# Blaizzy/mlx-audio

Measured on NVIDIA H100. Metric: audio-sec/sec Kokoro-82M TTS (128-phoneme utterance, 9.75 s), higher is better.
Workload: dtype bf16x2

## Files before the change

include/b200audio.h:

```cpp
#ifndef B200AUDIO_H
#define B200AUDIO_H

#include <stdint.h>

#ifdef __cplusplus
extern "C" {
#endif

#define B2A_OK 0
#define B2A_E_INVALID (-1)
#define B2A_E_CUDA (-2)
#define B2A_E_UNSUPPORTED (-3)

enum {
  B2A_ACT_NONE = 0,
  B2A_ACT_LRELU = 1,
  B2A_ACT_SNAKE = 2,
  B2A_ACT_ELU = 3,
  B2A_ACT_GELU = 4,
  B2A_ACT_GELU_TANH = 5,
  B2A_ACT_TANH = 6,
  B2A_ACT_SIGMOID = 7,
  B2A_ACT_SILU = 8,
  B2A_ACT_CLIP1 = 9
};

const char* b2a_last_error(void);
int32_t b2a_version(void);
int32_t b2a_device_sm_count(void);

typedef struct {
  const float* x; int64_t x_bs; int64_t x_ld;
  int32_t B, L, Cin;
  const float* w; const float* bias;
  float* y; int64_t y_bs; int64_t y_ld;
  int32_t Lout, Cout;
  int32_t K, stride, dilation, pad_left, groups, pad_mode;
  const float* pre_scale; const float* pre_shift;
  int32_t pre_act; float pre_p0; const float* pre_a; const float* pre_b;
  int32_t post_act; float post_p0;
  const float* post_cscale; int64_t post_cscale_bs;
  const float* res; int64_t res_bs; int64_t res_ld; int32_t res_div;
  float out_scale; int32_t accumulate;
  void* emit_hi; void* emit_lo; int64_t emit_ld;
  int32_t emit_act; float emit_p0; const float* emit_a; const float* emit_b;
} b2a_conv1d_t;

int32_t b2a_conv1d_cl(const b2a_conv1d_t* p, void* stream);
int32_t b2a_convtr1d_cl(const b2a_conv1d_t* p, void* stream);

enum {
  B2A_CONV_PATH_LINEAR_ROWS = 1,
  B2A_CONV_PATH_NARROW = 2,
  B2A_CONV_PATH_DENSE = 3,
  B2A_CONV_PATH_DW_TILED4 = 4,
  B2A_CONV_PATH_DW_TILED = 5,
  B2A_CONV_PATH_DW = 6,
  B2A_CONV_PATH_CONVTR_DENSE = 7,
  B2A_CONV_PATH_CONVTR_DW = 8
};
int32_t b2a_conv1d_cl_last_path(int32_t* out4);

int32_t b2a_kokoro_source_conv(const float* x, int32_t B, int32_t L, const float* w, const float* bias, float* y, int32_t Lout,
                               int32_t Cout, int32_t K, int32_t stride, int32_t pad_left, void* stream);

int32_t b2a_prep_bf16(const float* x, int64_t x_bs, int64_t x_ld, int32_t B, int32_t L, int32_t C, int32_t cpad,
                      const float* scale, const float* shift, int32_t act, float p0, const float* a, const float* b,
                      void* hi, void* lo, int32_t f16, void* stream);
int32_t b2a_conv1d_tc(const void* a_hi, const void* a_lo, int32_t f16, int32_t B, int32_t L, int32_t cin_pad, const void* w_bf16,
                      const void* w_lo,
                      int32_t taps, const int32_t* shifts_host, int32_t Cout, int32_t Lout, const float* bias,
                      int32_t post_act, float post_p0, const float* cscale, int64_t cscale_bs, const float* res,
                      int64_t res_bs, int64_t res_ld, int32_t res_div, float out_scale, int32_t accumulate, float* y,
                      int64_t y_bs, int64_t y_ld, int32_t up_stride, int32_t up_crop, void* emit_hi, void* emit_lo,
                      int64_t emit_ld, void* attn_ws, int32_t attn_heads, float attn_scale, void* stream);

typedef struct {
  int32_t T, layers, heads, hidden, inter, planes;
  const void* w[4];
  const float* bias[4];
  const float* ln_w[2];
  const float* ln_b[2];
  float eps, scale;
  float* h; void* h_hi; void* h_lo;
} b2a_albert_t;
int64_t b2a_albert_ws_bytes(int32_t T, int32_t heads, int32_t hidden, int32_t inter);
int32_t b2a_albert_encoder(const b2a_albert_t* a, void* ws, uint32_t* err, int64_t* timeline, void* stream);

int32_t b2a_conv1d_tc_debug(void* dbg8);

int32_t b2a_conv1d_tc_last_config(int32_t* out5);

int32_t b2a_copy2d(const float* src, int64_t src_ld, float* dst, int64_t dst_ld, int64_t rows, int32_t cols, void* stream);
int32_t b2a_gather_rows(const float* src, int64_t src_ld, const int64_t* idx, float* dst, int64_t dst_ld,
                        int64_t rows, int32_t cols, int64_t n_src_rows, const float* add, int64_t add_ld, int64_t add_period,
                        void* stream);
int32_t b2a_durations_to_index(const float* dur_f, const int64_t* dur_i, int32_t T, float speed, int64_t* pred_dur_out,
                               int64_t* idx_out, int64_t max_frames, int64_t* total_dev, void* stream);

int64_t b2a_adain_ws_bytes(int32_t B, int32_t L, int32_t C);
int32_t b2a_adain_coeffs(const float* x, int64_t x_bs, int64_t x_ld, int32_t B, int32_t L, int32_t C,
                         const float* gb, float eps, float* scale, float* shift, void* ws, void* stream);
int32_t b2a_channel_stats(const float* x, int64_t x_bs, int64_t x_ld, int32_t B, int32_t L, int32_t C, int64_t* const* dst,
                          const int64_t* dst_bs, int32_t n_dst, void* stream);
int32_t b2a_coeffs_from_stats(const int64_t* stats, int32_t B, int32_t L, int32_t C, const float* gb, float eps, float* scale, float* shift,
                              void* stream);
int32_t b2a_layernorm(const float* x, int64_t x_ld, const float* res, int64_t res_ld, float* y, int64_t y_ld,
                      int64_t rows, int32_t C, const float* w, const float* b, const float* ada, float eps,
                      int32_t rms, int32_t post_act, float post_p0, void* emit_hi, void* emit_lo, int64_t emit_ld, void* stream);

typedef struct {
  const float* q; const float* k; const float* v; float* o;
  int64_t q_bs, q_ld, k_bs, k_ld, v_bs, v_ld, o_bs, o_ld;
  int32_t B, Tq, Tk, H, Hkv, D;
  float scale; int32_t causal, q_offset, window;
  const int32_t* k_len;
  void* emit_hi; void* emit_lo; int64_t emit_ld;
  int32_t operands_ready;
} b2a_attn_t;
int32_t b2a_attention(const b2a_attn_t* p, void* stream);
int64_t b2a_attention_tc_ws_bytes(int32_t B, int32_t H, int32_t Tq, int32_t Tk);
int32_t b2a_attention_tc(const b2a_attn_t* p, void* ws, void* stream);
int32_t b2a_rope(float* x, int64_t x_bs, int64_t x_ld, int32_t B, int32_t T, int32_t H, int32_t D,
                 int32_t offset, float base, int32_t traditional, void* stream);

int32_t b2a_lstm_bidir(const float* xproj, const float* wh, float* out, int64_t out_ld, int32_t B, int32_t T, int32_t H, void* stream);

int32_t b2a_stft(const float* x, int64_t x_bs, int32_t B, int64_t n, const float* window, int32_t n_fft, int32_t hop,
                 int32_t pad_mode, int64_t frames, float* out_re, float* out_im, void* stream);
int32_t b2a_whisper_logmel(const float* x, int64_t x_bs, int32_t B, int64_t n, int64_t padding, const float* window,
                           const float* filters, int32_t n_mels, int64_t frames, float* out, float* gmax, void* stream);
int32_t b2a_istft(const float* re, const float* im, int32_t B, int32_t n_fft, int32_t T, int32_t hop, const float* window,
                  int32_t norm_sq, int32_t clamp_mode, int64_t trim, int64_t out_len, float* out, float* ws, void* stream);

int32_t b2a_resample_poly(const float* x, int64_t x_bs, int32_t B, int64_t n_in, const double* h, int32_t n_h, int32_t up,
                          int32_t down, int64_t n_pre_pad, int64_t n_pre_remove, float* out, int64_t n_out, void* stream);

int32_t b2a_kokoro_source(const float* f0, int32_t B, int32_t n_frames, int32_t n_down, const float* noise, const float* lin_w,
                          const float* lin_b, float* har, float* src_ws, double* ph_ws, void* stream);
int32_t b2a_kokoro_istft_head(const float* x, int64_t x_bs, int64_t x_ld, int32_t B, int32_t T, float* audio, void* stream);

#define B2A_CONVF_MAX_PROBLEMS 4
typedef struct {
  const float* x; const float* x1; const float* x2; int64_t x_bs, x_ld; float in_scale;
  int32_t B, L, Cin;
  int32_t pre_mode; const float* pre_scale; const float* pre_shift; const int64_t* pre_stats; const float* pre_gb; int64_t pre_gb_bs; float pre_eps;
  int32_t pre_act; float pre_p0; const float* pre_a; const float* pre_b;
  const void* w_hi; const void* w_lo; int32_t cin_pad, taps, N; int32_t shifts[32];
  int32_t Lout; const float* bias; int32_t post_act; float post_p0; const float* cscale; int64_t cscale_bs;
  const float* res; int64_t res_bs, res_ld; int32_t res_div; float out_scale; int32_t accumulate;
  float* y; int64_t y_bs, y_ld;
  int32_t up_stride, up_crop;
  int64_t* stats_out;
} b2a_convf_t;
int32_t b2a_conv1d_fused_debug(void* stamps );
int32_t b2a_conv1d_fused(const b2a_convf_t* problems, int32_t n_problems, int32_t planes, int32_t f16, void* ws, int64_t ws_bytes, void* stream);
int32_t b2a_conv1d_fused_fits(int32_t span, int32_t N, int32_t C, int32_t wplanes, int32_t planes);
int32_t b2a_conv1d_fused_last_config(int32_t* out10);

int32_t b2a_randn(float* out, int64_t n, uint64_t seed, uint64_t offset, void* stream);
int32_t b2a_randn_dev(float* out, int64_t n, uint64_t* state, void* stream);

int32_t b2a_whisper_greedy_step(const float* logits, int64_t logits_bs, const int64_t* tokens, int64_t tokens_bs,
                                int32_t B, int32_t cur_len, int32_t sample_begin, int32_t V, const float* suppress_mask,
                                const float* blank_mask, int32_t eot, int32_t no_timestamps, int32_t timestamp_begin,
                                int32_t max_initial_ts, int32_t without_timestamps, int64_t* next_out,
                                float* sum_logprobs, int32_t* not_done, float temperature, const float* u, void* stream);

int32_t b2a_sample_token(const float* logits, int64_t logits_bs, int32_t B, int32_t V, const float* suppress_mask,
                         uint8_t* seen, int64_t seen_bs, int32_t mark_seen, float repetition_penalty, float temperature,
                         int32_t top_k, float top_p, float min_p, const float* u, int64_t* out, int64_t out_stride,
                         float* filtered_out, uint8_t* finished, int32_t eos, void* stream);

int32_t b2a_gemv_bf16(const float* x, int64_t x_ld, int32_t M, int32_t K, const void* w_bf16, int64_t w_ld, int32_t N,
                      const float* bias, const float* norm_w, float norm_eps, int32_t mode, const float* res, int64_t res_ld,
                      float* y, int64_t y_ld, const void* prefetch, int64_t prefetch_bytes, void* stream);
int32_t b2a_qknorm_rope_cache(const float* qkv, int64_t qkv_bs, int64_t qkv_ss, int32_t B, int32_t S, int32_t Hq, int32_t Hkv,
                              int32_t D, const float* q_norm_w, const float* k_norm_w, float eps, const int32_t* pos3,
                              const int32_t* base_dev, int32_t base_host, int32_t sec_h, int32_t sec_w, float theta,
                              float* q_out, int64_t qo_bs, int64_t qo_ss, float* k_cache, float* v_cache, int64_t c_bs,
                              int64_t c_ss, int32_t smax, const int32_t* pos_shift, const int32_t* base_rows, const int32_t* slot,
                              void* stream);
int32_t b2a_attn_decode(const float* q, int64_t q_bs, int64_t q_ss, const float* k_cache, const float* v_cache, int64_t c_bs,
                        int64_t c_ss, float* out, int64_t o_bs, int64_t o_ss, int32_t B, int32_t S, int32_t Hq, int32_t Hkv,
                        int32_t D, float scale, const int32_t* base_dev, int32_t base_host, const int32_t* kv_start,
                        int32_t max_k, const int32_t* base_rows, const int32_t* slot, void* stream);
int32_t b2a_attn_prefill(const float* q, int64_t q_bs, int64_t q_ss, const float* k_cache, const float* v_cache, int64_t c_bs,
                         int64_t c_ss, float* out, int64_t o_bs, int64_t o_ss, int32_t B, int32_t S, int32_t Hq, int32_t Hkv,
                         int32_t D, float scale, const int32_t* base_dev, int32_t base_host, const int32_t* kv_start,
                         int32_t max_k, const int32_t* base_rows, const int32_t* slot, void* stream);
int32_t b2a_swiglu(const float* x, int64_t x_ld, int64_t rows, int32_t I, int32_t interleaved, float* y, int64_t y_ld, void* stream);
int32_t b2a_embed_sum(const int64_t* codes, int64_t codes_bs, int32_t B, int32_t G, int32_t dim, const float* const* tables_dev,
                      const int32_t* bins_dev, const float* text, int64_t text_bs, int64_t text_ss, int32_t n_text,
                      const float* pad, const int32_t* step_dev, int32_t step_sub, float* out, int64_t out_bs,
                      int32_t* err_flag_dev, int32_t* tidx, const uint8_t* finished, void* stream);
int32_t b2a_incr_i32(int32_t* p, int32_t v, void* stream);
int32_t b2a_slot_advance(int32_t* lengths, int32_t* frames, uint8_t* finished, const int32_t* cap, const int64_t* codes, int32_t G,
                         int64_t* out, int64_t out_bs, const float* u_tab, int64_t u_bs, float* u, int32_t B, void* stream);

int32_t b2a_rvq_decode(const int64_t* codes, int64_t codes_bs, int64_t codes_qs, int32_t B, int32_t nq, int64_t T,
                       const float* codebooks, int32_t bins, int32_t dim, float* out, int64_t out_ld, int32_t* err_flag_dev, void* stream);
int32_t b2a_rvq_encode(const float* x, int64_t x_ld, int64_t rows, int32_t dim, const float* codebooks, const double* c2, int32_t bins,
                       int32_t nq, int32_t mode, int64_t* codes, int64_t codes_row_stride, int64_t codes_level_stride, void* stream);
int32_t b2a_snac_from_codes(const int64_t* const* codes_host_ptrs, const int32_t* strides_host, int32_t n_levels,
                            const float* const* emb_host_ptrs, const float* const* w_host_ptrs, const float* const* bias_host_ptrs,
                            int32_t B, int64_t T, int32_t bins, int32_t cd, int32_t dim, float* out, int32_t* err_flag_dev, void* stream);

typedef struct {
  const float* w_in; const float* b_in;
  const float* cbn; const double* c2;
  const float* cb;
  const float* w_out; const float* b_out;
  int32_t cd; int32_t lat_off;
} b2a_dac_level_t;
int64_t b2a_dac_rvq_encode_smem_bytes(int32_t dim);
int32_t b2a_dac_rvq_encode(const float* z, int64_t z_ld, int32_t B, int64_t T, int32_t dim, const b2a_dac_level_t* levels_dev, int32_t n_levels,
                           int32_t bins, int32_t latent_channels, int64_t* codes, float* latents, float* z_q, double* loss_part, void* stream);
int32_t b2a_dac_from_codes(const int64_t* codes, int64_t codes_bs, int64_t codes_qs, int32_t B, int32_t n_levels, int64_t T,
                           const b2a_dac_level_t* levels_dev, int32_t bins, int32_t latent_channels, int32_t dim, float* out, float* z_p,
                           int32_t* err_flag_dev, void* stream);

int32_t b2a_aa_snakebeta(const float* x, int64_t x_bs, int64_t x_ld, int32_t B, int32_t L, int32_t C, const float* alpha, const float* inv_beta,
                         const float* f_up, const float* f_down, int32_t ratio, int32_t taps, float* y, int64_t y_bs, int64_t y_ld, void* hi,
                         void* lo, int32_t cpad, void* stream);

#define B2A_ROWOP_COPY 0
#define B2A_ROWOP_ADD 1
#define B2A_ROWOPS_MAX 32
typedef struct {
  const float* src; int64_t src_bs, src_ld;
  float* dst; int64_t dst_bs, dst_ld;
  int32_t B, rows, C, op;
} b2a_rowop_t;
int32_t b2a_stream_rows(const b2a_rowop_t* ops, int32_t n, void* stream);

int32_t b2a_conv1d_stream(const b2a_conv1d_t* p, float* hist, int64_t hist_bs, int32_t H, const int32_t* step_dev, int32_t fresh,
                          void* stream);
int32_t b2a_convtr1d_stream(const b2a_conv1d_t* p, float* tail, int64_t tail_bs, void* stream);
int32_t b2a_ring_rope_kv(float* qkv, int64_t qkv_bs, int64_t qkv_ld, int32_t B, int32_t T, int32_t H, int32_t D, float base,
                         float* k_ring, float* v_ring, int64_t ring_bs, int32_t cap, const int32_t* pos_dev, void* stream);
int32_t b2a_ring_attn(const float* q, int64_t q_bs, int64_t q_ld, const float* k_ring, const float* v_ring, int64_t ring_bs, int32_t cap,
                      float* out, int64_t o_bs, int64_t o_ld, int32_t B, int32_t T, int32_t H, int32_t D, float scale, int32_t window,
                      const int32_t* pos_dev, void* stream);
int32_t b2a_stream_advance(int32_t* ctr, int32_t dpos, void* stream);

int32_t b2a_spk_logmel(const float* x, int64_t x_bs, int32_t B, int64_t n, const float* window, const float* filters, int32_t n_mels,
                       int64_t frames, float* out, void* stream);
int32_t b2a_spk_reflect_pad(const float* x, int64_t x_bs, int64_t x_ld, int32_t B, int32_t T, int32_t C, int32_t pad, float* out_f32,
                            void* hi, void* lo, int32_t cpad, void* stream);
int64_t b2a_spk_res2net_smem_bytes(int32_t C, int32_t scale, int32_t K, int32_t pad, int32_t tile);
int32_t b2a_spk_res2net(const float* y, int64_t y_bs, int64_t y_ld, float* z, int64_t z_bs, int64_t z_ld, const float* w, const float* bias,
                        int32_t B, int32_t T, int32_t C, int32_t scale, int32_t K, int32_t dilation, int32_t tile, void* stream);
int32_t b2a_spk_channel_stats(const float* x, int64_t x_bs, int64_t x_ld, int32_t B, int32_t T, int32_t C, int32_t with_std, float eps,
                              float* out, int64_t o_bs, void* stream);
int32_t b2a_spk_se_gate(const float* mean, int64_t m_bs, int32_t B, int32_t C, int32_t S, const float* w1, const float* b1, const float* w2,
                        const float* b2, float* gate, void* stream);
int32_t b2a_spk_se_apply(const float* y, int64_t y_bs, int64_t y_ld, const float* gate, const float* res, int64_t r_bs, int64_t r_ld,
                         float* out, int64_t o_bs, int64_t o_ld, int32_t B, int32_t T, int32_t C, void* stream);
int32_t b2a_spk_gemv(const float* x, int64_t x_bs, int32_t B, int32_t K, const float* w, int64_t w_ld, int32_t N, const float* bias,
                     int32_t act, float* y, int64_t y_bs, void* stream);
int32_t b2a_spk_asp_act(float* h, int64_t h_bs, int64_t h_ld, const float* cb, int32_t B, int32_t T, int32_t A, void* stream);
int32_t b2a_spk_asp_pool(const float* logits, int64_t l_bs, int64_t l_ld, const float* x, int64_t x_bs, int64_t x_ld, int32_t B, int32_t T,
                         int32_t C, float eps, float* pooled, int64_t p_bs, void* stream);

int32_t b2a_vocos_dwnorm(const float* x, int64_t x_bs, int64_t x_ld, int32_t B, int32_t L, int32_t C, const float* dw_w, const float* dw_b,
                         int32_t K, const float* w, const float* b, const float* ada, int64_t ada_bs, float eps, float* y, int64_t y_bs,
                         int64_t y_ld, void* hi, void* lo, void* stream);
int32_t b2a_vocos_istft_head(const float* h, int64_t h_bs, int64_t h_ld, int32_t B, int32_t T, int32_t n_fft, int32_t hop, const float* window,
                             float* out, int64_t out_bs, void* stream);
int32_t b2a_vocos_logmel(const float* x, int64_t x_bs, int32_t B, int64_t n, const float* window, const float* filters, int32_t n_mels,
                         int64_t frames, float* out, void* stream);

int32_t b2a_encodec_lstm(const float* xproj, const float* wh, const float* skip, float* out, int32_t R, int32_t T, int32_t H, uint32_t* err,
                         void* stream);
int32_t b2a_encodec_pad(const float* x, int64_t x_bs, int64_t x_ld, int32_t B, int32_t T, int32_t C, int32_t pad_left, int32_t pad_right,
                        int32_t reflect, const float* scale, const float* shift, int32_t elu, const float* res, int64_t res_bs, int64_t res_ld,
                        float* y, int64_t y_bs, int64_t y_ld, void* stream);
int64_t b2a_encodec_gn_ws_bytes(int32_t B);
int32_t b2a_encodec_gn_coeffs(const float* x, int64_t x_bs, int64_t x_ld, int32_t B, int32_t T, int32_t C, const float* gamma,
                              const float* beta, float eps, float* scale, float* shift, void* ws, void* stream);
int32_t b2a_encodec_normalize(const float* x, int64_t x_bs, int64_t x_ld, int32_t R, int32_t L, int32_t C, const uint8_t* mask,
                              int64_t mask_bs, float* y, float* scale, void* stream);
int32_t b2a_encodec_ola(const float* frames, int32_t N, int32_t B, int32_t L, int32_t C, const float* scale, int32_t stride, int32_t Tout,
                        float* out, void* stream);

int32_t b2a_lm_sample_mlx(const float* logits, int64_t logits_bs, int32_t B, int32_t V, float temperature, double top_p, const float* u,
                          int64_t u_bs, const int32_t* step_dev, int64_t* out, int64_t* hist, int64_t hist_bs, uint8_t* finished,
                          int32_t stop0, int32_t stop1, void* stream);
int32_t b2a_soprano_upsample(const float* x, int64_t x_bs, int64_t x_ld, int32_t B, int32_t L, int32_t H, int32_t up, float* y, int64_t y_bs,
                             int64_t y_ld, void* hi, void* lo, int32_t cpad, void* stream);
int32_t b2a_soprano_store_rows(const float* src, int64_t src_bs, int32_t B, int32_t H, float* dst, int64_t dst_bs, int64_t dst_ld,
                               const int32_t* idx_dev, int32_t add, int32_t cap, void* stream);

#ifdef __cplusplus
}
#endif
#endif
```

mlx_audio_b200/_lib.py:

```python
from __future__ import annotations

import ctypes as C
import os

_HERE = os.path.dirname(os.path.abspath(__file__))
LIB_PATH = os.path.join(_HERE, "libb200audio.so")

c_f = C.c_void_p
i32, i64, f32 = C.c_int32, C.c_int64, C.c_float


class Conv1dParams(C.Structure):
    _fields_ = [
        ("x", C.c_void_p), ("x_bs", i64), ("x_ld", i64),
        ("B", i32), ("L", i32), ("Cin", i32),
        ("w", C.c_void_p), ("bias", C.c_void_p),
        ("y", C.c_void_p), ("y_bs", i64), ("y_ld", i64),
        ("Lout", i32), ("Cout", i32),
        ("K", i32), ("stride", i32), ("dilation", i32), ("pad_left", i32), ("groups", i32), ("pad_mode", i32),
        ("pre_scale", C.c_void_p), ("pre_shift", C.c_void_p),
        ("pre_act", i32), ("pre_p0", f32), ("pre_a", C.c_void_p), ("pre_b", C.c_void_p),
        ("post_act", i32), ("post_p0", f32),
        ("post_cscale", C.c_void_p), ("post_cscale_bs", i64),
        ("res", C.c_void_p), ("res_bs", i64), ("res_ld", i64), ("res_div", i32),
        ("out_scale", f32), ("accumulate", i32),
        ("emit_hi", C.c_void_p), ("emit_lo", C.c_void_p), ("emit_ld", i64),
        ("emit_act", i32), ("emit_p0", f32), ("emit_a", C.c_void_p), ("emit_b", C.c_void_p),
    ]


class AttnParams(C.Structure):
    _fields_ = [
        ("q", C.c_void_p), ("k", C.c_void_p), ("v", C.c_void_p), ("o", C.c_void_p),
        ("q_bs", i64), ("q_ld", i64), ("k_bs", i64), ("k_ld", i64), ("v_bs", i64), ("v_ld", i64), ("o_bs", i64), ("o_ld", i64),
        ("B", i32), ("Tq", i32), ("Tk", i32), ("H", i32), ("Hkv", i32), ("D", i32),
        ("scale", f32), ("causal", i32), ("q_offset", i32), ("window", i32),
        ("k_len", C.c_void_p),
        ("emit_hi", C.c_void_p), ("emit_lo", C.c_void_p), ("emit_ld", i64), ("operands_ready", i32),
    ]


class ConvFParams(C.Structure):
    _fields_ = [
        ("x", C.c_void_p), ("x1", C.c_void_p), ("x2", C.c_void_p), ("x_bs", i64), ("x_ld", i64), ("in_scale", f32),
        ("B", i32), ("L", i32), ("Cin", i32),
        ("pre_mode", i32), ("pre_scale", C.c_void_p), ("pre_shift", C.c_void_p), ("pre_stats", C.c_void_p), ("pre_gb", C.c_void_p),
        ("pre_gb_bs", i64), ("pre_eps", f32),
        ("pre_act", i32), ("pre_p0", f32), ("pre_a", C.c_void_p), ("pre_b", C.c_void_p),
        ("w_hi", C.c_void_p), ("w_lo", C.c_void_p), ("cin_pad", i32), ("taps", i32), ("N", i32), ("shifts", i32 * 32),
        ("Lout", i32), ("bias", C.c_void_p), ("post_act", i32), ("post_p0", f32), ("cscale", C.c_void_p), ("cscale_bs", i64),
        ("res", C.c_void_p), ("res_bs", i64), ("res_ld", i64), ("res_div", i32), ("out_scale", f32), ("accumulate", i32),
        ("y", C.c_void_p), ("y_bs", i64), ("y_ld", i64),
        ("up_stride", i32), ("up_crop", i32),
        ("stats_out", C.c_void_p),
    ]


class AlbertParams(C.Structure):
    _fields_ = [("T", i32), ("layers", i32), ("heads", i32), ("hidden", i32), ("inter", i32), ("planes", i32),
                ("w", C.c_void_p * 4), ("bias", C.c_void_p * 4), ("ln_w", C.c_void_p * 2), ("ln_b", C.c_void_p * 2),
                ("eps", f32), ("scale", f32), ("h", C.c_void_p), ("h_hi", C.c_void_p), ("h_lo", C.c_void_p)]


class RowOp(C.Structure):
    _fields_ = [("src", C.c_void_p), ("src_bs", i64), ("src_ld", i64), ("dst", C.c_void_p), ("dst_bs", i64), ("dst_ld", i64),
                ("B", i32), ("rows", i32), ("C", i32), ("op", i32)]


class DacLevel(C.Structure):
    _fields_ = [("w_in", C.c_void_p), ("b_in", C.c_void_p), ("cbn", C.c_void_p), ("c2", C.c_void_p), ("cb", C.c_void_p),
                ("w_out", C.c_void_p), ("b_out", C.c_void_p), ("cd", i32), ("lat_off", i32)]


ROWOPS_MAX = 32


PROTOTYPES = {
    "b2a_last_error": (C.c_char_p, []),
    "b2a_version": (i32, []),
    "b2a_device_sm_count": (i32, []),
    "b2a_conv1d_cl": (i32, [C.POINTER(Conv1dParams), C.c_void_p]),
    "b2a_convtr1d_cl": (i32, [C.POINTER(Conv1dParams), C.c_void_p]),
    "b2a_conv1d_cl_last_path": (i32, [C.POINTER(i32)]),
    "b2a_kokoro_source_conv": (i32, [c_f, i32, i32, c_f, c_f, c_f, i32, i32, i32, i32, i32, C.c_void_p]),
    "b2a_prep_bf16": (i32, [c_f, i64, i64, i32, i32, i32, i32, c_f, c_f, i32, f32, c_f, c_f, c_f, c_f, i32, C.c_void_p]),
    "b2a_conv1d_tc": (i32, [c_f, c_f, i32, i32, i32, i32, c_f, c_f, i32, C.POINTER(i32), i32, i32, c_f, i32, f32, c_f, i64, c_f, i64, i64, i32, f32, i32,
                            c_f, i64, i64, i32, i32, c_f, c_f, i64, c_f, i32, f32, C.c_void_p]),
    "b2a_conv1d_tc_debug": (i32, [c_f]),
    "b2a_conv1d_tc_last_config": (i32, [C.POINTER(i32)]),
    "b2a_conv1d_fused_debug": (i32, [c_f]),
    "b2a_conv1d_fused_last_config": (i32, [C.POINTER(i32)]),
    "b2a_conv1d_fused": (i32, [C.POINTER(ConvFParams), i32, i32, i32, c_f, i64, C.c_void_p]),
    "b2a_conv1d_fused_fits": (i32, [i32, i32, i32, i32, i32]),
    "b2a_copy2d": (i32, [c_f, i64, c_f, i64, i64, i32, C.c_void_p]),
    "b2a_gather_rows": (i32, [c_f, i64, c_f, c_f, i64, i64, i32, i64, c_f, i64, i64, C.c_void_p]),
    "b2a_durations_to_index": (i32, [c_f, c_f, i32, f32, c_f, c_f, i64, c_f, C.c_void_p]),
    "b2a_adain_ws_bytes": (i64, [i32, i32, i32]),
    "b2a_adain_coeffs": (i32, [c_f, i64, i64, i32, i32, i32, c_f, f32, c_f, c_f, c_f, C.c_void_p]),
    "b2a_channel_stats": (i32, [c_f, i64, i64, i32, i32, i32, C.POINTER(C.c_void_p), C.POINTER(i64), i32, C.c_void_p]),
    "b2a_coeffs_from_stats": (i32, [c_f, i32, i32, i32, c_f, f32, c_f, c_f, C.c_void_p]),
    "b2a_layernorm": (i32, [c_f, i64, c_f, i64, c_f, i64, i64, i32, c_f, c_f, c_f, f32, i32, i32, f32, c_f, c_f, i64, C.c_void_p]),
    "b2a_attention": (i32, [C.POINTER(AttnParams), C.c_void_p]),
    "b2a_attention_tc_ws_bytes": (i64, [i32, i32, i32, i32]),
    "b2a_attention_tc": (i32, [C.POINTER(AttnParams), C.c_void_p, C.c_void_p]),
    "b2a_albert_ws_bytes": (i64, [i32, i32, i32, i32]),
    "b2a_albert_encoder": (i32, [C.POINTER(AlbertParams), C.c_void_p, C.c_void_p, C.c_void_p, C.c_void_p]),
    "b2a_rope": (i32, [c_f, i64, i64, i32, i32, i32, i32, i32, f32, i32, C.c_void_p]),
    "b2a_lstm_bidir": (i32, [c_f, c_f, c_f, i64, i32, i32, i32, C.c_void_p]),
    "b2a_stft": (i32, [c_f, i64, i32, i64, c_f, i32, i32, i32, i64, c_f, c_f, C.c_void_p]),
    "b2a_whisper_logmel": (i32, [c_f, i64, i32, i64, i64, c_f, c_f, i32, i64, c_f, c_f, C.c_void_p]),
    "b2a_istft": (i32, [c_f, c_f, i32, i32, i32, i32, c_f, i32, i32, i64, i64, c_f, c_f, C.c_void_p]),
    "b2a_resample_poly": (i32, [c_f, i64, i32, i64, c_f, i32, i32, i32, i64, i64, c_f, i64, C.c_void_p]),
    "b2a_kokoro_source": (i32, [c_f, i32, i32, i32, c_f, c_f, c_f, c_f, c_f, c_f, C.c_void_p]),
    "b2a_kokoro_istft_head": (i32, [c_f, i64, i64, i32, i32, c_f, C.c_void_p]),
    "b2a_randn": (i32, [c_f, i64, C.c_uint64, C.c_uint64, C.c_void_p]),
    "b2a_randn_dev": (i32, [c_f, i64, c_f, C.c_void_p]),
    "b2a_whisper_greedy_step": (i32, [c_f, i64, c_f, i64, i32, i32, i32, i32, c_f, c_f, i32, i32, i32, i32, i32, c_f, c_f, c_f, f32, c_f, C.c_void_p]),
    "b2a_sample_token": (i32, [c_f, i64, i32, i32, c_f, c_f, i64, i32, f32, f32, i32, f32, f32, c_f, c_f, i64, c_f, c_f, i32, C.c_void_p]),
    "b2a_gemv_bf16": (i32, [c_f, i64, i32, i32, c_f, i64, i32, c_f, c_f, f32, i32, c_f, i64, c_f, i64, c_f, i64, C.c_void_p]),
    "b2a_qknorm_rope_cache": (i32, [c_f, i64, i64, i32, i32, i32, i32, i32, c_f, c_f, f32, c_f, c_f, i32, i32, i32, f32, c_f, i64, i64,
                                    c_f, c_f, i64, i64, i32, c_f, c_f, c_f, C.c_void_p]),
    "b2a_attn_decode": (i32, [c_f, i64, i64, c_f, c_f, i64, i64, c_f, i64, i64, i32, i32, i32, i32, i32, f32, c_f, i32, c_f, i32, c_f, c_f,
                              C.c_void_p]),
    "b2a_attn_prefill": (i32, [c_f, i64, i64, c_f, c_f, i64, i64, c_f, i64, i64, i32, i32, i32, i32, i32, f32, c_f, i32, c_f, i32, c_f, c_f,
                               C.c_void_p]),
    "b2a_swiglu": (i32, [c_f, i64, i64, i32, i32, c_f, i64, C.c_void_p]),
    "b2a_embed_sum": (i32, [c_f, i64, i32, i32, i32, c_f, c_f, c_f, i64, i64, i32, c_f, c_f, i32, c_f, i64, c_f, c_f, c_f, C.c_void_p]),
    "b2a_incr_i32": (i32, [c_f, i32, C.c_void_p]),
    "b2a_slot_advance": (i32, [c_f, c_f, c_f, c_f, c_f, i32, c_f, i64, c_f, i64, c_f, i32, C.c_void_p]),
    "b2a_rvq_decode": (i32, [c_f, i64, i64, i32, i32, i64, c_f, i32, i32, c_f, i64, c_f, C.c_void_p]),
    "b2a_rvq_encode": (i32, [c_f, i64, i64, i32, c_f, c_f, i32, i32, i32, c_f, i64, i64, C.c_void_p]),
    "b2a_snac_from_codes": (i32, [C.POINTER(C.c_void_p), C.POINTER(i32), i32, C.POINTER(C.c_void_p), C.POINTER(C.c_void_p),
                                  C.POINTER(C.c_void_p), i32, i64, i32, i32, i32, c_f, c_f, C.c_void_p]),
    "b2a_dac_rvq_encode_smem_bytes": (i64, [i32]),
    "b2a_dac_rvq_encode": (i32, [c_f, i64, i32, i64, i32, c_f, i32, i32, i32, c_f, c_f, c_f, c_f, C.c_void_p]),
    "b2a_dac_from_codes": (i32, [c_f, i64, i64, i32, i32, i64, c_f, i32, i32, i32, c_f, c_f, c_f, C.c_void_p]),
    "b2a_aa_snakebeta": (i32, [c_f, i64, i64, i32, i32, i32, c_f, c_f, c_f, c_f, i32, i32, c_f, i64, i64, c_f, c_f, i32, C.c_void_p]),
    "b2a_stream_rows": (i32, [C.POINTER(RowOp), i32, C.c_void_p]),
    "b2a_conv1d_stream": (i32, [C.POINTER(Conv1dParams), c_f, i64, i32, c_f, i32, C.c_void_p]),
    "b2a_convtr1d_stream": (i32, [C.POINTER(Conv1dParams), c_f, i64, C.c_void_p]),
    "b2a_ring_rope_kv": (i32, [c_f, i64, i64, i32, i32, i32, i32, f32, c_f, c_f, i64, i32, c_f, C.c_void_p]),
    "b2a_ring_attn": (i32, [c_f, i64, i64, c_f, c_f, i64, i32, c_f, i64, i64, i32, i32, i32, i32, f32, i32, c_f, C.c_void_p]),
    "b2a_stream_advance": (i32, [c_f, i32, C.c_void_p]),
    "b2a_spk_logmel": (i32, [c_f, i64, i32, i64, c_f, c_f, i32, i64, c_f, C.c_void_p]),
    "b2a_spk_reflect_pad": (i32, [c_f, i64, i64, i32, i32, i32, i32, c_f, c_f, c_f, i32, C.c_void_p]),
    "b2a_spk_res2net_smem_bytes": (i64, [i32, i32, i32, i32, i32]),
    "b2a_spk_res2net": (i32, [c_f, i64, i64, c_f, i64, i64, c_f, c_f, i32, i32, i32, i32, i32, i32, i32, C.c_void_p]),
    "b2a_spk_channel_stats": (i32, [c_f, i64, i64, i32, i32, i32, i32, f32, c_f, i64, C.c_void_p]),
    "b2a_spk_se_gate": (i32, [c_f, i64, i32, i32, i32, c_f, c_f, c_f, c_f, c_f, C.c_void_p]),
    "b2a_spk_se_apply": (i32, [c_f, i64, i64, c_f, c_f, i64, i64, c_f, i64, i64, i32, i32, i32, C.c_void_p]),
    "b2a_spk_gemv": (i32, [c_f, i64, i32, i32, c_f, i64, i32, c_f, i32, c_f, i64, C.c_void_p]),
    "b2a_spk_asp_act": (i32, [c_f, i64, i64, c_f, i32, i32, i32, C.c_void_p]),
    "b2a_spk_asp_pool": (i32, [c_f, i64, i64, c_f, i64, i64, i32, i32, i32, f32, c_f, i64, C.c_void_p]),
    "b2a_vocos_dwnorm": (i32, [c_f, i64, i64, i32, i32, i32, c_f, c_f, i32, c_f, c_f, c_f, i64, f32, c_f, i64, i64, c_f, c_f, C.c_void_p]),
    "b2a_vocos_istft_head": (i32, [c_f, i64, i64, i32, i32, i32, i32, c_f, c_f, i64, C.c_void_p]),
    "b2a_vocos_logmel": (i32, [c_f, i64, i32, i64, c_f, c_f, i32, i64, c_f, C.c_void_p]),
    "b2a_encodec_lstm": (i32, [c_f, c_f, c_f, c_f, i32, i32, i32, c_f, C.c_void_p]),
    "b2a_encodec_pad": (i32, [c_f, i64, i64, i32, i32, i32, i32, i32, i32, c_f, c_f, i32, c_f, i64, i64, c_f, i64, i64, C.c_void_p]),
    "b2a_encodec_gn_ws_bytes": (i64, [i32]),
    "b2a_encodec_gn_coeffs": (i32, [c_f, i64, i64, i32, i32, i32, c_f, c_f, f32, c_f, c_f, c_f, C.c_void_p]),
    "b2a_encodec_normalize": (i32, [c_f, i64, i64, i32, i32, i32, c_f, i64, c_f, c_f, C.c_void_p]),
    "b2a_encodec_ola": (i32, [c_f, i32, i32, i32, i32, c_f, i32, i32, c_f, C.c_void_p]),
    "b2a_lm_sample_mlx": (i32, [c_f, i64, i32, i32, f32, C.c_double, c_f, i64, c_f, c_f, c_f, i64, c_f, i32, i32, C.c_void_p]),
    "b2a_soprano_upsample": (i32, [c_f, i64, i64, i32, i32, i32, i32, c_f, i64, i64, c_f, c_f, i32, C.c_void_p]),
    "b2a_soprano_store_rows": (i32, [c_f, i64, i32, i32, c_f, i64, i64, c_f, i32, i32, C.c_void_p]),
}

E_INVALID, E_CUDA, E_UNSUPPORTED = -1, -2, -3


def load() -> C.CDLL:
    if not os.path.exists(LIB_PATH):
        raise ImportError(
            f"{LIB_PATH} is missing: build it with `python -m mlx_audio_b200.build` "
            "(there is no CPU or PyTorch fallback for the hot path)")
    lib = C.CDLL(LIB_PATH)
    for name, (res, args) in PROTOTYPES.items():
        fn = getattr(lib, name)
        fn.restype = res
        fn.argtypes = args
    return lib


_LIB = None


def lib() -> C.CDLL:
    global _LIB
    if _LIB is None:
        _LIB = load()
    return _LIB


def check(rc: int) -> None:
    if rc == 0:
        return
    msg = lib().b2a_last_error().decode("utf-8", "replace")
    if rc == E_INVALID:
        raise ValueError(msg)
    if rc == E_UNSUPPORTED:
        raise NotImplementedError(msg)
    raise RuntimeError(msg)
```

mlx_audio_b200/csrc/albert.cu:

```cuda
#include "common.cuh"
#include "tc_common.cuh"
#include "tc_epilogue.cuh"
#include "attn_tc_tile.cuh"
#include "layernorm_row.cuh"

using namespace tc;

namespace {

constexpr int THREADS = 288;
constexpr int SLOTS = 6;
constexpr int SLOT_BYTES = 32768;
constexpr int PLANE = 64 * 128;
constexpr int OFF_Q = SLOTS * SLOT_BYTES;
constexpr int OFF_BAR = OFF_Q + 2 * PLANE;
constexpr int SMEM_BYTES = OFF_BAR + (2 * SLOTS + 2) * 8 + 16 + 1024;
constexpr int STAGES = 7;
constexpr long long TIMEOUT_NS = 10000000000LL;

struct AlbertMaps {
  CUtensorMap a_hi[4], a_lo[4], w[4];
  CUtensorMap qh, ql, kh, kl, vh, vl;
};

struct AlbertParams {
  int T, layers, planes, mb, H, hs, inter, nkt;
  int N[4], K[4];
  const float* bias[4];
  const float *ln_w[2], *ln_b[2]; float eps;
  float qmul;
  float *h, *t, *u;
  __nv_bfloat16 *hp_hi, *hp_lo, *ap_hi, *ap_lo, *fp_hi, *fp_lo;
  __nv_bfloat16 *cp_hi, *cp_lo;
  AttnOperands attn;
  unsigned* bar; unsigned* err;
  long long* tl;
};

__device__ __forceinline__ int gemm_of_stage(int s) { return s == 0 ? 0 : s == 2 ? 1 : s == 4 ? 2 : s == 5 ? 3 : -1; }

__device__ __forceinline__ long long globaltimer() {
  long long t;
  asm volatile("mov.u64 %0, %globaltimer;" : "=l"(t));
  return t;
}

__device__ bool grid_wait(const AlbertParams& p, unsigned target) {
  long long t0 = 0;
  for (int it = 0;; it++) {
    unsigned v;
    asm volatile("ld.acquire.gpu.global.u32 %0, [%1];" : "=r"(v) : "l"(p.bar) : "memory");
    if ((int)(v - target) >= 0) return true;
    if ((it & 63) == 63) {
      if (*(volatile unsigned*)p.err) return false;
      const long long now = globaltimer();
      if (!t0) t0 = now;
      else if (now - t0 > TIMEOUT_NS) { atomicExch(p.err, 1u); return false; }
    }
    __nanosleep(64);
  }
}

__device__ __forceinline__ void grid_arrive(unsigned* bar) {
  asm volatile("red.release.gpu.global.add.u32 [%0], 1;" ::"l"(bar) : "memory");
}

__device__ __forceinline__ void fence_proxy_async_global() { asm volatile("fence.proxy.async.global;" ::: "memory"); }

template <bool TL>
__global__ void __launch_bounds__(THREADS, 1) albert_kernel(const __grid_constant__ AlbertMaps maps, const AlbertParams p) {
  extern __shared__ __align__(1024) uint8_t smem_raw[];
  uint8_t* smem = (uint8_t*)(((uintptr_t)smem_raw + 1023) & ~(uintptr_t)1023);
  uint64_t* full = (uint64_t*)(smem + OFF_BAR);
  uint64_t* empty = full + SLOTS;
  uint64_t* q_full = empty + SLOTS;
  uint64_t* q_empty = q_full + 1;
  const int warp = threadIdx.x >> 5, lane = threadIdx.x & 31;
  const int bid = blockIdx.x, grid = gridDim.x;
  const int total = p.layers * STAGES;

  if (warp == 8 && lane == 0) {
    for (int g = 0; g < 4; g++) {
      asm volatile("prefetch.tensormap [%0];" ::"l"(&maps.a_hi[g]) : "memory");
      asm volatile("prefetch.tensormap [%0];" ::"l"(&maps.w[g]) : "memory");
    }
    for (int s = 0; s < SLOTS; s++) { mbar_init(full + s, 1); mbar_init(empty + s, 2); }
    mbar_init(q_full, 1); mbar_init(q_empty, 2);
    asm volatile("fence.mbarrier_init.release.cluster;" ::: "memory");
    asm volatile("fence.proxy.async.shared::cta;" ::: "memory");
  }
  __syncthreads();

  if (warp == 8) {
    if (lane != 0) return;
    uint32_t g = 0, qn = 0;
    for (int k = 0; k < total; k++) {
      const int stage = k % STAGES, gi = gemm_of_stage(stage);
      if (stage == 1) {
        const int units = p.H * p.mb;
        if (bid >= units) continue;
        grid_wait(p, (unsigned)k * grid);
        fence_proxy_async_global();
        for (int u = bid; u < units; u += grid) {
          const int head = u / p.mb, q0 = (u % p.mb) * 64;
          mbar_wait(q_empty, (qn & 1) ^ 1);
          mbar_expect_tx(q_full, 2 * PLANE);
          tma_load_3d(smem + OFF_Q, &maps.qh, q_full, 0, q0, head);
          tma_load_3d(smem + OFF_Q + PLANE, &maps.ql, q_full, 0, q0, head);
          qn++;
          for (int t = 0; t < p.nkt; t++, g++) {
            const int s = g % SLOTS;
            uint8_t* st = smem + (size_t)s * SLOT_BYTES;
            mbar_wait(empty + s, ((g / SLOTS) & 1) ^ 1);
            mbar_expect_tx(full + s, 4 * PLANE);
            tma_load_3d(st, &maps.kh, full + s, 0, t * 64, head);
            tma_load_3d(st + PLANE, &maps.kl, full + s, 0, t * 64, head);
            tma_load_3d(st + 2 * PLANE, &maps.vh, full + s, t * 64, 0, head);
            tma_load_3d(st + 3 * PLANE, &maps.vl, full + s, t * 64, 0, head);
          }
        }
        continue;
      }
      if (gi < 0) continue;
      const int units = p.mb * (p.N[gi] / 64), kc = p.K[gi] / 64;
      const uint32_t bytes = (uint32_t)(PLANE * p.planes + PLANE);
      bool waited = k == 0;
      for (int u = bid; u < units; u += grid) {
        const int m0 = (u % p.mb) * 64, n0 = (u / p.mb) * 64;
        int pre = 0;
        if (!waited) {
          pre = kc < SLOTS ? kc : SLOTS;
          for (int c = 0; c < pre; c++) {
            const uint32_t gc = g + c;
            const int s = gc % SLOTS;
            mbar_wait(empty + s, ((gc / SLOTS) & 1) ^ 1);
            mbar_expect_tx(full + s, bytes);
            tma_load_2d(smem + (size_t)s * SLOT_BYTES + 2 * PLANE, &maps.w[gi], full + s, c * 64, n0);
          }
          grid_wait(p, (unsigned)k * grid);
          fence_proxy_async_global();
          waited = true;
          for (int c = 0; c < pre; c++) {
            const int s = (g + c) % SLOTS;
            uint8_t* st = smem + (size_t)s * SLOT_BYTES;
            tma_load_2d(st, &maps.a_hi[gi], full + s, c * 64, m0);
            if (p.planes == 2) tma_load_2d(st + PLANE, &maps.a_lo[gi], full + s, c * 64, m0);
          }
        }
        for (int c = pre; c < kc; c++) {
          const uint32_t gc = g + c;
          const int s = gc % SLOTS;
          uint8_t* st = smem + (size_t)s * SLOT_BYTES;
          mbar_wait(empty + s, ((gc / SLOTS) & 1) ^ 1);
          mbar_expect_tx(full + s, bytes);
          tma_load_2d(st + 2 * PLANE, &maps.w[gi], full + s, c * 64, n0);
          tma_load_2d(st, &maps.a_hi[gi], full + s, c * 64, m0);
          if (p.planes == 2) tma_load_2d(st + PLANE, &maps.a_lo[gi], full + s, c * 64, m0);
        }
        g += kc;
      }
    }
    return;
  }

  const int ct = threadIdx.x, wg = warp >> 2, w4 = warp & 3;
  const uint32_t sb = smem_u32(smem);
  uint32_t g = 0, qn = 0;
  for (int k = 0; k < total; k++) {
    const int stage = k % STAGES, gi = gemm_of_stage(stage);
    if (k > 0) {
      if (ct == 0) grid_wait(p, (unsigned)k * grid);
      bar_sync(1, 256);
    }
    if constexpr (TL) { if (ct == 0) p.tl[((int64_t)k * grid + bid) * 2] = globaltimer(); }
    if (gi >= 0) {
      const int units = p.mb * (p.N[gi] / 64), kc = p.K[gi] / 64, N = p.N[gi];
      const float* bias = p.bias[gi];
      for (int u = bid; u < units; u += grid) {
        const int m0 = (u % p.mb) * 64, n0 = (u / p.mb) * 64;
        float acc[16];
        int prev = -1;
        for (int c = 0; c < kc; c++, g++) {
          const int s = g % SLOTS;
          mbar_wait(full + s, (g / SLOTS) & 1);
          const uint32_t st = sb + s * SLOT_BYTES;
          const uint64_t ad = gmma_desc_sw128(st), wd = gmma_desc_sw128(st + 2 * PLANE + wg * 32 * 128);
          wgmma_fence();
          wgmma_chunk<1, false>(acc, ad, wd, c != 0);
          if (p.planes == 2) wgmma_chunk<1, false>(acc, gmma_desc_sw128(st + PLANE), wd, 1u);
          wgmma_commit();
          wgmma_wait<1>();
          wgmma_fence_regs<16>(acc);
          if (prev >= 0 && (ct & 127) == 0) mbar_arrive(empty + prev);
          prev = s;
        }
        wgmma_wait<0>();
        wgmma_fence_regs<16>(acc);
        if ((ct & 127) == 0) mbar_arrive(empty + prev);
#pragma unroll
        for (int j = 0; j < 4; j++) {
          const int n = n0 + wg * 32 + 8 * j + 2 * (lane & 3);
          const float b0 = __ldg(bias + n), b1 = __ldg(bias + n + 1);
          EmitCol e0{}, e1{};
          if (gi == 0) { e0 = emit_col_attn(p.attn, 0, p.T, p.hs, p.qmul, n); e1 = emit_col_attn(p.attn, 0, p.T, p.hs, p.qmul, n + 1); }
#pragma unroll
          for (int hh = 0; hh < 2; hh++) {
            const int row = m0 + 16 * w4 + (lane >> 2) + 8 * hh;
            const float a0 = acc[4 * j + 2 * hh], a1 = acc[4 * j + 2 * hh + 1];
            if (row >= p.T) {
              if (gi == 0 && e0.step == 1 && row < p.attn.tkp) { e0.hi[row] = 0; e0.lo[row] = 0; e1.hi[row] = 0; e1.lo[row] = 0; }
              continue;
            }
            const int64_t o = (int64_t)row * N + n;
            if (gi == 0) {
              emit_store(e0, row, epilogue_value(a0, b0, 0, 0.f, 1.f, 0.f));
              emit_store(e1, row, epilogue_value(a1, b1, 0, 0.f, 1.f, 0.f));
            } else if (gi == 2) {
              const float y0 = epilogue_value(a0, b0, B2A_ACT_GELU, 0.f, 1.f, 0.f), y1 = epilogue_value(a1, b1, B2A_ACT_GELU, 0.f, 1.f, 0.f);
              __nv_bfloat162 h2, l2;
              split16(y0, h2.x, l2.x);
              split16(y1, h2.y, l2.y);
              *reinterpret_cast<__nv_bfloat162*>(p.fp_hi + o) = h2;
              if (p.planes == 2) *reinterpret_cast<__nv_bfloat162*>(p.fp_lo + o) = l2;
            } else {
              const float* res = gi == 1 ? p.h : p.t;
              float* out = gi == 1 ? p.t : p.u;
              const float2 r = *reinterpret_cast<const float2*>(res + o);
              *reinterpret_cast<float2*>(out + o) = make_float2(epilogue_value(a0, b0, 0, 0.f, 1.f, r.x), epilogue_value(a1, b1, 0, 0.f, 1.f, r.y));
            }
          }
        }
      }
    } else if (stage == 1) {
      const int units = p.H * p.mb;
      for (int u = bid; u < units; u += grid, qn++) {
        const int head = u / p.mb, q0 = (u % p.mb) * 64;
        float o[32], m[2] = {-INFINITY, -INFINITY}, l[2] = {0.f, 0.f};
#pragma unroll
        for (int j = 0; j < 32; j++) o[j] = 0.f;
        const int kmax[2] = {p.T - 1, p.T - 1}, kmin[2] = {0, 0};
        const uint64_t dqh = gmma_desc_sw128(sb + OFF_Q), dql = gmma_desc_sw128(sb + OFF_Q + PLANE);
        mbar_wait(q_full, qn & 1);
        for (int t = 0; t < p.nkt; t++, g++) {
          const int s = g % SLOTS;
          const uint32_t st = sb + s * SLOT_BYTES;
          mbar_wait(full + s, (g / SLOTS) & 1);
          if (wg == 0)
            attn_tc_tile(o, m, l, dqh, dql, gmma_desc_sw128(st), gmma_desc_sw128(st + PLANE), gmma_desc_sw128(st + 2 * PLANE),
                         gmma_desc_sw128(st + 3 * PLANE), t * 64, kmax, kmin, lane);
          if ((ct & 127) == 0) mbar_arrive(empty + s);
        }
        if ((ct & 127) == 0) mbar_arrive(q_empty);
        if (wg == 0) {
          float inv[2];
          attn_tc_row_inv(l, inv);
#pragma unroll
          for (int hh = 0; hh < 2; hh++) {
            const int q = q0 + w4 * 16 + (lane >> 2) + 8 * hh;
            if (q < p.T) {
              const int64_t e = (int64_t)q * p.hs + head * 64 + 2 * (lane & 3);
#pragma unroll
              for (int j = 0; j < 8; j++) {
                __nv_bfloat162 eh, el;
                split16(o[4 * j + 2 * hh] * inv[hh], eh.x, el.x);
                split16(o[4 * j + 2 * hh + 1] * inv[hh], eh.y, el.y);
                *reinterpret_cast<__nv_bfloat162*>(p.cp_hi + e + 8 * j) = eh;
                if (p.planes == 2) *reinterpret_cast<__nv_bfloat162*>(p.cp_lo + e + 8 * j) = el;
              }
            }
          }
        }
      }
    } else {
      const int which = stage == 3 ? 0 : 1;
      const float* x = which ? p.u : p.t;
      float* y = which ? p.h : p.t;
      __nv_bfloat16* eh = which ? p.hp_hi : p.ap_hi;
      __nv_bfloat16* el = p.planes == 2 ? (which ? p.hp_lo : p.ap_lo) : nullptr;
      for (int row = bid * 8 + warp; row < p.T; row += grid * 8) {
        const int64_t o = (int64_t)row * p.hs;
        layernorm_row_vec<8>(x + o, nullptr, y + o, p.hs, p.ln_w[which], p.ln_b[which], nullptr, p.eps, 0, 0, 0.f, eh + o,
                             el ? el + o : nullptr, lane);
      }
    }
    if constexpr (TL) { if (ct == 0) p.tl[((int64_t)k * grid + bid) * 2 + 1] = globaltimer(); }
    if (k + 1 < total) {
      fence_proxy_async_global();
      bar_sync(1, 256);
      if (ct == 0) { __threadfence(); grid_arrive(p.bar); }
    }
  }
}

struct WsLayout { int64_t t, u, cp_hi, cp_lo, ap_hi, ap_lo, fp_hi, fp_lo, attn, total; };
WsLayout ws_layout(int64_t T, int64_t H, int64_t hs, int64_t inter) {
  auto up = [](int64_t x) { return (x + 255) / 256 * 256; };
  WsLayout w;
  int64_t o = 256;
  w.t = o; o += up(T * hs * 4);
  w.u = o; o += up(T * hs * 4);
  w.cp_hi = o; o += up(T * hs * 2);
  w.cp_lo = o; o += up(T * hs * 2);
  w.ap_hi = o; o += up(T * hs * 2);
  w.ap_lo = o; o += up(T * hs * 2);
  w.fp_hi = o; o += up(T * inter * 2);
  w.fp_lo = o; o += up(T * inter * 2);
  w.attn = o; o += b2a_attention_tc_ws_bytes(1, (int32_t)H, (int32_t)T, (int32_t)T);
  w.total = o;
  return w;
}

}

extern "C" int64_t b2a_albert_ws_bytes(int32_t T, int32_t heads, int32_t hidden, int32_t inter) {
  return ws_layout(T, heads, hidden, inter).total;
}

extern "C" int32_t b2a_albert_encoder(const b2a_albert_t* a, void* ws, uint32_t* err, int64_t* timeline, void* stream) {
  B2A_CHECK_ARG(a && ws && err && a->h && a->h_hi && (a->planes == 1 || (a->planes == 2 && a->h_lo)), "null pointer");
  for (int i = 0; i < 4; i++) B2A_CHECK_ARG(a->w[i] && a->bias[i], "null weight or bias");
  for (int i = 0; i < 2; i++) B2A_CHECK_ARG(a->ln_w[i] && a->ln_b[i], "null LayerNorm parameter");
  B2A_CHECK_ARG(a->T >= 64 && a->T <= 512 && a->layers > 0 && a->heads > 0 && a->hidden == 64 * a->heads && a->hidden <= 1024 &&
                a->inter % 64 == 0 && a->inter > 0, "shape: 64 <= T <= 512, hidden = 64 * heads <= 1024, inter a multiple of 64");
  const int T = a->T, H = a->heads, hs = a->hidden, inter = a->inter;
  uint8_t* base = (uint8_t*)ws;
  B2A_CHECK_ARG(((uintptr_t)base & 255) == 0, "workspace must be 256-byte aligned");
  const WsLayout L = ws_layout(T, H, hs, inter);
  cudaStream_t st = (cudaStream_t)stream;

  AlbertParams p{};
  p.T = T; p.layers = a->layers; p.planes = a->planes; p.mb = cdiv(T, 64); p.H = H; p.hs = hs; p.inter = inter; p.nkt = cdiv(T, 64);
  const int N[4] = {3 * hs, hs, inter, hs}, K[4] = {hs, hs, hs, inter};
  for (int i = 0; i < 4; i++) { p.N[i] = N[i]; p.K[i] = K[i]; p.bias[i] = a->bias[i]; }
  for (int i = 0; i < 2; i++) { p.ln_w[i] = a->ln_w[i]; p.ln_b[i] = a->ln_b[i]; }
  p.eps = a->eps;
  p.qmul = a->scale * 1.4426950408889634f;
  p.h = a->h; p.t = (float*)(base + L.t); p.u = (float*)(base + L.u);
  p.hp_hi = (__nv_bfloat16*)a->h_hi; p.hp_lo = (__nv_bfloat16*)a->h_lo;
  p.cp_hi = (__nv_bfloat16*)(base + L.cp_hi); p.cp_lo = (__nv_bfloat16*)(base + L.cp_lo);
  p.ap_hi = (__nv_bfloat16*)(base + L.ap_hi); p.ap_lo = (__nv_bfloat16*)(base + L.ap_lo);
  p.fp_hi = (__nv_bfloat16*)(base + L.fp_hi); p.fp_lo = (__nv_bfloat16*)(base + L.fp_lo);
  p.attn = attn_operands(base + L.attn, H, T, T);
  p.bar = (unsigned*)base; p.err = err;
  p.tl = (long long*)timeline;

  AlbertMaps m;
  const void* a_hi[4] = {p.hp_hi, p.cp_hi, p.ap_hi, p.fp_hi};
  const void* a_lo[4] = {p.hp_lo, p.cp_lo, p.ap_lo, p.fp_lo};
  const uint32_t box[3] = {64, 64, 1};
  int e = 0;
  for (int i = 0; i < 4 && !e; i++) {
    const uint64_t ad[2] = {(uint64_t)K[i], (uint64_t)T}, as[1] = {(uint64_t)K[i] * 2};
    const uint64_t wd[2] = {(uint64_t)K[i], (uint64_t)N[i]};
    e = b2a_tmap16(&m.a_hi[i], a_hi[i], 2, ad, as, box, false);
    if (!e) e = b2a_tmap16(&m.a_lo[i], a->planes == 2 ? a_lo[i] : a_hi[i], 2, ad, as, box, false);
    if (!e) e = b2a_tmap16(&m.w[i], a->w[i], 2, wd, as, box, false);
  }
  const uint64_t qd[3] = {64, (uint64_t)T, (uint64_t)H}, qs[2] = {128, (uint64_t)T * 128};
  const uint64_t vd[3] = {(uint64_t)p.attn.tkp, 64, (uint64_t)H}, vs[2] = {(uint64_t)p.attn.tkp * 2, (uint64_t)p.attn.tkp * 128};
  if (!e) e = b2a_tmap16(&m.qh, p.attn.qh, 3, qd, qs, box, true);
  if (!e) e = b2a_tmap16(&m.ql, p.attn.ql, 3, qd, qs, box, true);
  if (!e) e = b2a_tmap16(&m.kh, p.attn.kh, 3, qd, qs, box, true);
  if (!e) e = b2a_tmap16(&m.kl, p.attn.kl, 3, qd, qs, box, true);
  if (!e) e = b2a_tmap16(&m.vh, p.attn.vh, 3, vd, vs, box, true);
  if (!e) e = b2a_tmap16(&m.vl, p.attn.vl, 3, vd, vs, box, true);
  if (e) { b2a_set_error("b2a_albert_encoder: cuTensorMapEncodeTiled failed (%d)", e); return B2A_E_CUDA; }

  void (*kern)(const AlbertMaps, const AlbertParams) = timeline ? albert_kernel<true> : albert_kernel<false>;
  B2A_SMEM_OPTIN(kern, SMEM_BYTES);
  const int nsm = b2a_device_sm_count();
  int per_sm = 0;
  if (cudaOccupancyMaxActiveBlocksPerMultiprocessor(&per_sm, kern, THREADS, SMEM_BYTES) != cudaSuccess || per_sm < 1 || nsm < 1) {
    b2a_set_error("b2a_albert_encoder: the kernel cannot be resident (%s)", cudaGetErrorString(cudaGetLastError()));
    return B2A_E_CUDA;
  }
  if (cudaMemsetAsync(p.bar, 0, 4, st) != cudaSuccess) { b2a_set_error("b2a_albert_encoder: %s", cudaGetErrorString(cudaGetLastError())); return B2A_E_CUDA; }
  cudaLaunchConfig_t cfg = {};
  cfg.gridDim = dim3(nsm); cfg.blockDim = dim3(THREADS); cfg.dynamicSmemBytes = SMEM_BYTES; cfg.stream = st;
  cudaLaunchAttribute at[1];
  at[0].id = cudaLaunchAttributeCooperative;
  at[0].val.cooperative = 1;
  cfg.attrs = at; cfg.numAttrs = 1;
  if (cudaLaunchKernelEx(&cfg, kern, m, p) != cudaSuccess) {
    b2a_set_error("b2a_albert_encoder: %s", cudaGetErrorString(cudaGetLastError()));
    return B2A_E_CUDA;
  }
  return B2A_OK;
}
```

mlx_audio_b200/csrc/conv_fused.cu:

```cuda
#include "common.cuh"
#include "tc_common.cuh"
#include <stdlib.h>

using namespace tc;

namespace {

constexpr int TM = 128;
constexpr int TK = 64;

constexpr int MAXG = B2A_CONVF_MAX_PROBLEMS;
constexpr int NWORK = 8;
constexpr int NSUB = NWORK / 4;
constexpr int WG_PROD = 2;
constexpr int W_PROD = WG_PROD * 4;
constexpr int W_WORK0 = 12;
constexpr int THREADS = (W_WORK0 + NWORK) * 32;
constexpr int REG_LAUNCH = 96;
constexpr int REG_MMA = 96, REG_PROD = 32, REG_WORK = 128;
static_assert(THREADS % 128 == 0 && W_WORK0 % 4 == 0, "roles must sit on warpgroup boundaries");
static_assert(2 * REG_MMA + REG_PROD + 2 * REG_WORK <= 5 * REG_LAUNCH, "the re-allocated registers must fit in the launch allocation");

template <int R> __device__ __forceinline__ void set_regs() {
  if constexpr (R < REG_LAUNCH) asm volatile("setmaxnreg.dec.sync.aligned.u32 %0;" ::"n"(R));
  else if constexpr (R > REG_LAUNCH) asm volatile("setmaxnreg.inc.sync.aligned.u32 %0;" ::"n"(R));
}
constexpr int RSTRIDE = NWORK * 32 / 16;
constexpr int SACC = 4 * 2 * 128 * 4;
constexpr int CT_MAX = 1280;
constexpr int CTAB = 2 * CT_MAX * 4;

struct FProb {
  const float* x; const float* x1; const float* x2; int64_t x_bs, x_ld; float in_scale;
  int B, L, Cin, cin_pad;
  int pre_mode;
  const float* pre_scale; const float* pre_shift;
  const long long* pre_stats; const float* pre_gb; int64_t pre_gb_bs; float pre_eps, pre_invL;
  int pre_act; float pre_p0; const float* pre_a; const float* pre_b;
  int taps, wplanes, BN, ntn, ntm, Ntot, R, shift_min, ksplit, kper;
  int shift[32];
  int Lout, Mrows, up_s, up_crop, C;
  const float* bias; int post_act; float post_p0; const float* cscale; int64_t cscale_bs;
  const float* res; int64_t res_bs, res_ld; int res_div; float out_scale; int accumulate;
  float* y; int64_t y_bs, y_ld;
  long long* stats_out;
  float* ws; int* counters;
  int tile_begin;
};

struct FParams {
  int G, ntiles, planes, f16, wst, w_stage, a_plane, acc_ld;
  unsigned long long* dbg;
  int dbg_flags;
  FProb pr[MAXG];
};
constexpr size_t DYN_SMEM_MAX = (size_t)227 * 1024 - ((sizeof(FParams) + 1023) & ~(size_t)1023);

struct TileRef { int g, b, mt, nt, ks; };

__device__ __forceinline__ TileRef decode_tile(const FParams& p, int tile) {
  int g = 0;
#pragma unroll
  for (int i = 1; i < MAXG; i++) if (i < p.G && tile >= p.pr[i].tile_begin) g = i;
  int local = tile - p.pr[g].tile_begin;
  const FProb& P = p.pr[g];
  TileRef t;
  t.g = g;
  t.ks = local % P.ksplit; local /= P.ksplit;
  t.nt = local % P.ntn; local /= P.ntn;
  t.mt = local % P.ntm; t.b = local / P.ntm;
  return t;
}

template <typename T16> __device__ __forceinline__ void split16x2(float a, float b, uint32_t& hi, uint32_t& lo);
template <> __device__ __forceinline__ void split16x2<__nv_bfloat16>(float a, float b, uint32_t& hi, uint32_t& lo) {
  const __nv_bfloat162 h = __floats2bfloat162_rn(a, b);
  const __nv_bfloat162 l = __floats2bfloat162_rn(a - __low2float(h), b - __high2float(h));
  hi = *reinterpret_cast<const uint32_t*>(&h); lo = *reinterpret_cast<const uint32_t*>(&l);
}
template <> __device__ __forceinline__ void split16x2<__half>(float a, float b, uint32_t& hi, uint32_t& lo) {
  const __half2 h = __floats2half2_rn(a, b);
  const __half2 l = __floats2half2_rn(a - __low2float(h), b - __high2float(h));
  hi = *reinterpret_cast<const uint32_t*>(&h); lo = *reinterpret_cast<const uint32_t*>(&l);
}

__device__ __noinline__ float act_slow(float v, int act, float p0) { return b2a_act(v, act, p0, 1.f, 1.f); }
__device__ __noinline__ float act_slow2(float v, int act, float p0, float a, float b) { return b2a_act(v, act, p0, a, b); }

#define TIMED_WAIT(p, acc, stmt) do { if (DBG && (p).dbg) { const long long t0_ = clock64(); stmt; acc += (unsigned long long)(clock64() - t0_); } else { stmt; } } while (0)
__device__ __forceinline__ void stamp(const FParams& p, int slot) {
  if (p.dbg) { unsigned long long t; asm volatile("mov.u64 %0, %%globaltimer;" : "=l"(t)); p.dbg[(size_t)blockIdx.x * 32 + slot] = t; }
}

template <typename T16, int ACT>
__device__ __forceinline__ void convert_store(float4 v, bool valid, const float sc[4], const float sh[4], const float aa[4], const float bb[4],
                                              const bool chok[4], int act, float p0, uint8_t* hi, uint8_t* lo, int r, int c4, bool do_store = true) {
  const float t[4] = {v.x, v.y, v.z, v.w};
  float u[4];
#pragma unroll
  for (int q = 0; q < 4; q++) {
    const bool ok = valid && chok[q];
    float w = fmaf(t[q], sc[q], sh[q]);
    if constexpr (ACT == B2A_ACT_SNAKE) { const float s = b2a_sin_fast(aa[q] * w); w = fmaf(bb[q], s * s, w); }
    else if constexpr (ACT == B2A_ACT_LRELU) w = w > 0.f ? w : w * p0;
    else if constexpr (ACT == B2A_ACT_ELU) w = w > 0.f ? w : expm1f(w);
    else if constexpr (ACT == 0) { }
    else if (ok && act) w = act_slow2(w, act, p0, aa[q], bb[q]);
    u[q] = ok ? w : 0.f;
  }
  uint2 h, l;
  split16x2<T16>(u[0], u[1], h.x, l.x);
  split16x2<T16>(u[2], u[3], h.y, l.y);
  const uint32_t off = (uint32_t)r * 128u + ((((uint32_t)c4 >> 1) ^ ((uint32_t)r & 7u)) << 4) + (((uint32_t)c4 & 1u) << 3);
  if (do_store) {
    *reinterpret_cast<uint2*>(hi + off) = h;
    if (lo) *reinterpret_cast<uint2*>(lo + off) = l;
  } else if (h.x == 0x12345678u && l.y == 0x9abcdef0u) {
    hi[0] = 1;
  }
}

template <typename T16, int ACT, int NADD, int U>
__device__ __forceinline__ void convert_chunk(const float* __restrict__ xb, const float* __restrict__ xb1, const float* __restrict__ xb2, int64_t x_ld,
                                              int L, int lbase, int ch, int c4, int r0, int R, bool anych, const float sc[4], const float sh[4],
                                              const float aa[4], const float bb[4], const bool chok[4], int act, float p0, uint8_t* hi, uint8_t* lo,
                                              int flags = 0) {
  for (int r = r0; r < R; r += RSTRIDE * U) {
    float4 v[U], w1[NADD > 0 ? U : 1], w2[NADD > 1 ? U : 1];
    bool ok[U];
#pragma unroll
    for (int u = 0; u < U; u++) {
      const int rr = r + u * RSTRIDE;
      const int l = lbase + rr;
      ok[u] = rr < R && l >= 0 && l < L && anych;
      const int64_t off = ok[u] ? (int64_t)l * x_ld + ch : 0;
      if (flags & 1) v[u] = make_float4((float)rr, 1.f, 2.f, 3.f); else
      v[u] = __ldg(reinterpret_cast<const float4*>(xb + off));
      if constexpr (NADD > 0) w1[u] = __ldg(reinterpret_cast<const float4*>(xb1 + off));
      if constexpr (NADD > 1) w2[u] = __ldg(reinterpret_cast<const float4*>(xb2 + off));
    }
#pragma unroll
    for (int u = 0; u < U; u++) {
      const int rr = r + u * RSTRIDE;
      if constexpr (NADD > 0) { v[u].x += w1[u].x; v[u].y += w1[u].y; v[u].z += w1[u].z; v[u].w += w1[u].w; }
      if constexpr (NADD > 1) { v[u].x += w2[u].x; v[u].y += w2[u].y; v[u].z += w2[u].z; v[u].w += w2[u].w; }
      if (rr < R) convert_store<T16, ACT>(v[u], ok[u], sc, sh, aa, bb, chok, act, p0, hi, lo, rr, c4, !(flags & 2));
    }
  }
}

__device__ __forceinline__ void stats_coeffs(const FProb& P, int b, int c, float& sc, float& sh) {
  const long long* w = P.pre_stats + ((int64_t)b * P.Cin + c) * (2 * B2A_NBIN);
  const double invL = 1.0 / (double)P.L;
  const double mean = repro_value(w) * invL;
  double var = repro_value(w + B2A_NBIN) * invL - mean * mean;
  if (var < 0) var = 0;
  const double rstd = 1.0 / sqrt(var + (double)P.pre_eps);
  double g_ = 1.0, be = 0.0;
  if (P.pre_gb) { g_ = 1.0 + (double)__ldg(P.pre_gb + (int64_t)b * P.pre_gb_bs + c); be = (double)__ldg(P.pre_gb + (int64_t)b * P.pre_gb_bs + P.Cin + c); }
  const double s_ = g_ * rstd;
  sc = (float)s_ * P.in_scale;
  sh = (float)(be - s_ * mean);
}

struct MmaCtl { int kc0, kc1, taps, nb, two_w; };
__device__ __forceinline__ MmaCtl mma_ctl(const FProb& P, const TileRef& t) {
  const int kchunks = P.cin_pad / TK;
  const int kc0 = t.ks * P.kper;
  MmaCtl c;
  c.kc0 = __shfl_sync(0xffffffffu, kc0, 0);
  c.kc1 = __shfl_sync(0xffffffffu, min(kchunks, kc0 + P.kper), 0);
  c.taps = __shfl_sync(0xffffffffu, P.taps, 0);
  c.nb = __shfl_sync(0xffffffffu, P.BN >> 5, 0);
  c.two_w = __shfl_sync(0xffffffffu, P.wplanes == 2, 0);
  return c;
}

enum { MW_FULL, MW_AFULL, MW_TEMPTY, MW_WGMMA, MW_N };
#define MMA_TIMED(slot, stmt) do { if constexpr (DBG) { const long long t0_ = clock64(); stmt; if (leader) mwait[slot] += (unsigned long long)(clock64() - t0_); } else { stmt; } } while (0)
template <int NB, bool F16, bool DBG>
__device__ __forceinline__ void mma_tile(const FParams& p, const FProb& P, const MmaCtl& c, bool two_a, float* acc, uint32_t a0, uint32_t w0,
                                         uint64_t* full, uint64_t* empty, uint64_t* a_full, uint64_t* a_empty, uint64_t* tfull, uint64_t* tempty,
                                         float* acct, uint32_t lt, uint32_t& s, uint32_t& ph, uint32_t& cg, unsigned long long* mwait) {
  const int wg = threadIdx.x >> 7;
  const bool leader = (threadIdx.x & 127) == 0;
  const int kc0 = c.kc0, kc1 = c.kc1;
  const uint32_t wb = (uint32_t)NB * 32u * 128u, a_plane = (uint32_t)p.a_plane, a_buf = a_plane * (two_a ? 2u : 1u);
  const bool two_w = c.two_w != 0;
  const int taps = c.taps, smin = P.shift_min;
  int pend_s = -1, pend_a = -1;
  uint32_t accum = 0;
  for (int kc = kc0; kc < kc1; kc++, cg++) {
    const uint32_t ab = cg & 1;
    MMA_TIMED(MW_AFULL, mbar_wait(a_full + ab, (cg >> 1) & 1));
    const uint32_t abase = a0 + ab * a_buf + (uint32_t)wg * 64u * 128u;
    for (int tap = 0; tap < taps; tap++) {
      MMA_TIMED(MW_FULL, mbar_wait(full + s, ph));
      const uint32_t wa = w0 + s * (uint32_t)p.w_stage;
      const uint32_t aa = abase + (uint32_t)(P.shift[tap] - smin) * 128u;
      const uint64_t wd = gmma_desc_sw128(wa), ad = gmma_desc_sw128(aa);
      wgmma_fence();
      wgmma_chunk<NB, F16>(acc, ad, wd, accum);
      accum = 1;
      if (two_a) wgmma_chunk<NB, F16>(acc, gmma_desc_sw128(aa + a_plane), wd, 1u);
      if (two_w) wgmma_chunk<NB, F16>(acc, ad, gmma_desc_sw128(wa + wb), 1u);
      wgmma_commit();
      MMA_TIMED(MW_WGMMA, wgmma_wait<1>());
      wgmma_fence_regs<NB * 16>(acc);
      if (leader) {
        if (pend_s >= 0) mbar_arrive(empty + pend_s);
        if (pend_a >= 0) mbar_arrive(a_empty + pend_a);
      }
      pend_s = (int)s;
      pend_a = tap == taps - 1 ? (int)ab : -1;
      if (++s == (uint32_t)p.wst) { s = 0; ph ^= 1; }
    }
  }
  MMA_TIMED(MW_WGMMA, wgmma_wait<0>());
  wgmma_fence_regs<NB * 16>(acc);
  if (leader) {
    if (pend_s >= 0) mbar_arrive(empty + pend_s);
    if (pend_a >= 0) mbar_arrive(a_empty + pend_a);
  }
  MMA_TIMED(MW_TEMPTY, mbar_wait(tempty, (lt & 1) ^ 1));
  store_acc<NB>(acc, acct, p.acc_ld, wg * 64);
  __syncwarp();
  if ((threadIdx.x & 31) == 0) mbar_arrive(tfull);
}

struct SmemLayout {
  int a_buf;
  uint8_t* wbase;
  float *acct, *sacc, *ctab;
  uint64_t *full, *empty, *tfull, *tempty, *a_full, *a_empty;
  int* flag_slot;
  __device__ __forceinline__ SmemLayout(uint8_t* smem, const FParams& p) {
    a_buf = p.a_plane * p.planes;
    wbase = smem + (size_t)2 * a_buf;
    acct = reinterpret_cast<float*>(wbase + (size_t)p.wst * p.w_stage);
    sacc = acct + TM * p.acc_ld;
    ctab = reinterpret_cast<float*>(reinterpret_cast<uint8_t*>(sacc) + SACC);
    full = reinterpret_cast<uint64_t*>(reinterpret_cast<uint8_t*>(ctab) + CTAB);
    empty = full + p.wst;
    tfull = empty + p.wst;
    tempty = tfull + 1;
    a_full = tempty + 1;
    a_empty = a_full + 2;
    flag_slot = reinterpret_cast<int*>(a_empty + 2);
  }
};

template <bool DBG>
__global__ void __launch_bounds__(THREADS, 1)
conv_fused_kernel(const __grid_constant__ FParams gp, const __grid_constant__ CUtensorMap mw0, const __grid_constant__ CUtensorMap mw1,
                  const __grid_constant__ CUtensorMap mw2, const __grid_constant__ CUtensorMap mw3,
                  const __grid_constant__ CUtensorMap ml0, const __grid_constant__ CUtensorMap ml1,
                  const __grid_constant__ CUtensorMap ml2, const __grid_constant__ CUtensorMap ml3) {
  extern __shared__ __align__(1024) uint8_t smem_raw[];
  uint8_t* smem = (uint8_t*)(((uintptr_t)smem_raw + 1023) & ~(uintptr_t)1023);
  const int warp = threadIdx.x >> 5, lane = threadIdx.x & 31;
  __shared__ __align__(16) FParams sparams;
  __shared__ unsigned long long mwait_all[DBG ? 2 * MW_N : 1];
  {
    const uint32_t* src = reinterpret_cast<const uint32_t*>(&gp);
    uint32_t* dst = reinterpret_cast<uint32_t*>(&sparams);
    for (int i = threadIdx.x; i < (int)(sizeof(FParams) / 4); i += THREADS) dst[i] = src[i];
    if (DBG && threadIdx.x < 2 * MW_N) mwait_all[threadIdx.x] = 0;
  }
  __syncthreads();
  const FParams& p = sparams;
  if (threadIdx.x == 0) if (DBG) stamp(p, 0);

  if (warp == W_PROD && lane == 0) {
    const SmemLayout sl(smem, p);
    for (int s = 0; s < p.wst; s++) { mbar_init(sl.full + s, 1); mbar_init(sl.empty + s, 2); }
    mbar_init(sl.tfull, 8); mbar_init(sl.tempty, NWORK);
    mbar_init(sl.a_full, NWORK); mbar_init(sl.a_full + 1, NWORK); mbar_init(sl.a_empty, 2); mbar_init(sl.a_empty + 1, 2);
    asm volatile("fence.mbarrier_init.release.cluster;" ::: "memory");
    asm volatile("fence.proxy.async.shared::cta;" ::: "memory");
  }
  __syncthreads();
  if (threadIdx.x == 0) if (DBG) stamp(p, 1);
  pdl_launch_dependents();

  const int wgi = __shfl_sync(0xffffffffu, (int)(threadIdx.x >> 7), 0);
  if (wgi == WG_PROD) {
    set_regs<REG_PROD>();
    if (warp == W_PROD && lane == 0) {
      const SmemLayout sl(smem, p);
      uint8_t* const wbase = sl.wbase;
      uint64_t* const full = sl.full;
      uint64_t* const empty = sl.empty;
      const CUtensorMap* mws[MAXG] = {&mw0, &mw1, &mw2, &mw3};
      const CUtensorMap* mls[MAXG] = {&ml0, &ml1, &ml2, &ml3};
      for (int g = 0; g < p.G; g++) {
        asm volatile("prefetch.tensormap [%0];" ::"l"(mws[g]) : "memory");
        if (p.pr[g].wplanes == 2) asm volatile("prefetch.tensormap [%0];" ::"l"(mls[g]) : "memory");
      }
      int s = 0; uint32_t ph = 0;
      unsigned long long w_pempty = 0;
      const long long pt0 = DBG ? clock64() : 0;
      for (int tile = blockIdx.x; tile < p.ntiles; tile += gridDim.x) {
        const TileRef t = decode_tile(p, tile);
        const FProb& P = p.pr[t.g];
        const int n0 = t.nt * P.BN;
        const int kchunks = P.cin_pad / TK;
        const int kc0 = t.ks * P.kper, kc1 = min(kchunks, kc0 + P.kper);
        const uint32_t wb = (uint32_t)P.BN * 128u;
        for (int kc = kc0; kc < kc1; kc++) {
          for (int tap = 0; tap < P.taps; tap++) {
            TIMED_WAIT(p, w_pempty, mbar_wait(empty + s, ph ^ 1));
            uint8_t* st = wbase + (size_t)s * p.w_stage;
            mbar_expect_tx(full + s, wb * (uint32_t)P.wplanes);
            tma_load_2d(st, mws[t.g], full + s, kc * TK, tap * P.Ntot + n0);
            if (P.wplanes == 2) tma_load_2d(st + wb, mls[t.g], full + s, kc * TK, tap * P.Ntot + n0);
            if (++s == p.wst) { s = 0; ph ^= 1; }
          }
        }
      }
      if (DBG && p.dbg) { p.dbg[(size_t)blockIdx.x * 32 + 21] = (unsigned long long)(clock64() - pt0); p.dbg[(size_t)blockIdx.x * 32 + 22] = w_pempty; }
    }
  } else if (wgi < WG_PROD) {
    set_regs<REG_MMA>();
    const SmemLayout sl(smem, p);
    uint64_t *const full = sl.full, *const empty = sl.empty, *const a_full = sl.a_full, *const a_empty = sl.a_empty;
    uint64_t *const tfull = sl.tfull, *const tempty = sl.tempty;
    float* const acct = sl.acct;
    const uint32_t a0 = smem_u32(smem), w0 = smem_u32(sl.wbase);
    const bool f16 = gp.f16 != 0, two_a = gp.planes == 2;
    uint32_t s = 0, ph = 0, lt = 0, cg = 0;
    float acc[4 * 16];
#pragma unroll
    for (int i = 0; i < 4 * 16; i++) acc[i] = 0.f;
    unsigned long long* const mwait = mwait_all + (DBG ? wgi * MW_N : 0);
    for (int tile = blockIdx.x; tile < gp.ntiles; tile += gridDim.x, lt++) {
      const TileRef t = decode_tile(p, tile);
      const FProb& P = p.pr[t.g];
      const MmaCtl c = mma_ctl(P, t);
#define B2A_MMA_TILE(NB) (f16 ? mma_tile<NB, true, DBG>(p, P, c, two_a, acc, a0, w0, full, empty, a_full, a_empty, tfull, tempty, acct, lt, s, ph, cg, mwait) \
                              : mma_tile<NB, false, DBG>(p, P, c, two_a, acc, a0, w0, full, empty, a_full, a_empty, tfull, tempty, acct, lt, s, ph, cg, mwait))
      switch (c.nb) {
        case 1: B2A_MMA_TILE(1); break;
        case 2: B2A_MMA_TILE(2); break;
        case 3: B2A_MMA_TILE(3); break;
        default: B2A_MMA_TILE(4); break;
      }
#undef B2A_MMA_TILE
    }
  } else {
    set_regs<REG_WORK>();
    const SmemLayout sl(smem, p);
    const int a_buf = sl.a_buf;
    float *const acct = sl.acct, *const sacc = sl.sacc, *const ctab = sl.ctab;
    uint64_t *const a_full = sl.a_full, *const a_empty = sl.a_empty, *const tfull = sl.tfull, *const tempty = sl.tempty;
    int* const flag_slot = sl.flag_slot;
    pdl_wait();
    if (warp == W_WORK0 && lane == 0) if (DBG) stamp(p, 3);
    const int ww = warp - W_WORK0;
    const int wt = ww * 32 + lane;
    const int c4 = wt & 15;
    const int r0 = wt >> 4;
    const int quarter = ww & 3, sub = ww >> 2;
    const int et = wt;
    uint32_t cg = 0;
    int cur_key = -1;
    unsigned long long w_aempty = 0, w_tfull = 0;

    auto convert_tile = [&](const int tile) {
      {
        const TileRef t = decode_tile(p, tile);
        const FProb& P = p.pr[t.g];
        const int l0 = t.mt * TM, n0 = t.nt * P.BN, b = t.b;
        if (!P.up_s && P.ksplit == 1) {
          const int prow = l0 + quarter * 32 + lane;
          if (prow < P.Lout) {
            if (P.res) {
              const float* q = P.res + (int64_t)b * P.res_bs + (int64_t)(P.res_div == 2 ? (prow >> 1) : prow) * P.res_ld + n0;
              for (int c = sub * 32; c < P.BN; c += NSUB * 32) asm volatile("prefetch.global.L2 [%0];" ::"l"(q + c));
            }
            if (P.accumulate) {
              const float* q = P.y + (int64_t)b * P.y_bs + (int64_t)prow * P.y_ld + n0;
              for (int c = sub * 32; c < P.BN; c += NSUB * 32) asm volatile("prefetch.global.L2 [%0];" ::"l"(q + c));
            }
          }
        }
      }
      const TileRef t = decode_tile(p, tile);
      const FProb& P = p.pr[t.g];
      const int kchunks = P.cin_pad / TK;
      const int kc0 = t.ks * P.kper, kc1 = min(kchunks, kc0 + P.kper);
      const int lbase = t.mt * TM + P.shift_min;
      const float* xb = P.x + (int64_t)t.b * P.x_bs;
      const float* xb1 = P.x1 ? P.x1 + (int64_t)t.b * P.x_bs : nullptr;
      const float* xb2 = P.x2 ? P.x2 + (int64_t)t.b * P.x_bs : nullptr;
      const int R = P.R;
      const bool tabled = P.pre_mode != 0 && P.Cin <= CT_MAX;
      const int key = (t.g << 16) | t.b;
      if (tabled && key != cur_key) {
        bar_sync(3, NWORK * 32);
        for (int c = wt; c < P.Cin; c += NWORK * 32) {
          float sc_ = P.in_scale, sh_ = 0.f;
          if (P.pre_mode == 1) { sc_ = __ldg(P.pre_scale + (int64_t)t.b * P.Cin + c) * P.in_scale; sh_ = __ldg(P.pre_shift + (int64_t)t.b * P.Cin + c); }
          else stats_coeffs(P, t.b, c, sc_, sh_);
          ctab[c] = sc_; ctab[CT_MAX + c] = sh_;
        }
        bar_sync(3, NWORK * 32);
        cur_key = key;
      }
      for (int kc = kc0; kc < kc1; kc++, cg++) {
        const uint32_t ab = cg & 1;
        const int ch = kc * TK + c4 * 4;
        float sc[4], sh[4], aa[4], bb[4];
        bool chok[4];
#pragma unroll
        for (int q = 0; q < 4; q++) {
          const int c = ch + q;
          chok[q] = c < P.Cin;
          sc[q] = P.in_scale; sh[q] = 0.f; aa[q] = 1.f; bb[q] = 1.f;
          if (chok[q]) {
            if (tabled) { sc[q] = ctab[c]; sh[q] = ctab[CT_MAX + c]; }
            else if (P.pre_mode == 1) { sc[q] = __ldg(P.pre_scale + (int64_t)t.b * P.Cin + c) * P.in_scale; sh[q] = __ldg(P.pre_shift + (int64_t)t.b * P.Cin + c); }
            else if (P.pre_mode == 2) stats_coeffs(P, t.b, c, sc[q], sh[q]);
            if (P.pre_a) aa[q] = __ldg(P.pre_a + c);
            if (P.pre_b) bb[q] = __ldg(P.pre_b + c);
          }
        }
        const bool anych = ch < P.Cin;
        TIMED_WAIT(p, w_aempty, mbar_wait(a_empty + ab, ((cg >> 1) & 1) ^ 1));
        uint8_t* hi = smem + (size_t)ab * a_buf;
        uint8_t* lo = p.planes == 2 ? hi + p.a_plane : nullptr;
#define B2A_CONVERT(T, A, N, UU) convert_chunk<T, A, N, UU>(xb, xb1, xb2, P.x_ld, P.L, lbase, chs, c4, r0, R, anych, sc, sh, aa, bb, chok, P.pre_act, P.pre_p0, hi, lo, (DBG ? p.dbg_flags : 0))
        const int chs = anych ? ch : 0;
        if ((DBG ? p.dbg_flags : 0) & 16) { }
        else if (p.f16) { if (xb1 == nullptr && P.pre_act == 0) B2A_CONVERT(__half, 0, 0, 5); else if (xb2) B2A_CONVERT(__half, -1, 2, 2);
                     else if (xb1) B2A_CONVERT(__half, -1, 1, 3); else B2A_CONVERT(__half, -1, 0, 3); }
        else if (xb2) B2A_CONVERT(__nv_bfloat16, -1, 2, 2);
        else if (xb1) B2A_CONVERT(__nv_bfloat16, -1, 1, 3);
        else if (P.pre_act == 0) B2A_CONVERT(__nv_bfloat16, 0, 0, 5);
        else if (P.pre_act == B2A_ACT_SNAKE) B2A_CONVERT(__nv_bfloat16, B2A_ACT_SNAKE, 0, 5);
        else if (P.pre_act == B2A_ACT_LRELU) B2A_CONVERT(__nv_bfloat16, B2A_ACT_LRELU, 0, 5);
        else if (P.pre_act == B2A_ACT_ELU) B2A_CONVERT(__nv_bfloat16, B2A_ACT_ELU, 0, 3);
        else B2A_CONVERT(__nv_bfloat16, -1, 0, 3);
#undef B2A_CONVERT
        if (!((DBG ? p.dbg_flags : 0) & 4)) asm volatile("fence.proxy.async.shared::cta;" ::: "memory");
        __syncwarp();
        if (lane == 0) mbar_arrive(a_full + ab);
        if (warp == W_WORK0 && lane == 0) { if (cg == 0) if (DBG) stamp(p, 6); if (DBG) stamp(p, 7); }
      }
    };

    auto epilogue_tile = [&](const int tile, const uint32_t lt) {
      const TileRef t = decode_tile(p, tile);
      const FProb& P = p.pr[t.g];
      const int mul = P.up_s ? P.up_s : 1;
      const int l0 = t.mt * TM, n0 = t.nt * P.BN, b = t.b;
      const bool do_stats = P.stats_out != nullptr;
      TIMED_WAIT(p, w_tfull, mbar_wait(tfull, lt & 1));
      if (et == 0 && lt == 0) if (DBG) stamp(p, 8);
      const int mrow0 = l0 + quarter * 32;
      float* tq = acct + (size_t)(quarter * 32) * p.acc_ld;
      const int ALD = p.acc_ld;
      bool last_split = !((DBG ? p.dbg_flags : 0) & 32);
      if (P.ksplit > 1) {
        const int tid = ((b * P.ntm + t.mt) * P.ntn + t.nt);
        float* mine = P.ws + ((int64_t)tid * P.ksplit + t.ks) * (TM * P.BN) + (int64_t)(quarter * 32) * P.BN;
        for (int c0 = sub * 32; c0 < P.BN; c0 += NSUB * 32) {
          const float* stage = tq + c0;
#pragma unroll 8
          for (int i = 0; i < 32; i++) mine[(int64_t)i * P.BN + c0 + lane] = stage[i * ALD + lane];
        }
        __threadfence();
        bar_sync(2, NWORK * 32);
        if (et == 0) {
          const int prev = atomicAdd(P.counters + tid, 1);
          const int last = prev == P.ksplit - 1;
          if (last) P.counters[tid] = 0;
          *flag_slot = last;
        }
        bar_sync(2, NWORK * 32);
        last_split = *flag_slot != 0;
        if (last_split) __threadfence();
        if (et == 0 && lt == 0) if (DBG) stamp(p, 9);
      }
      if (last_split) {
        for (int c0 = sub * 32; c0 < P.BN; c0 += NSUB * 32) {
          float* stage = tq + c0;
          if (P.ksplit > 1) {
            const int tid = ((b * P.ntm + t.mt) * P.ntn + t.nt);
            const float* base = P.ws + (int64_t)tid * P.ksplit * (TM * P.BN) + (int64_t)(quarter * 32) * P.BN + c0 + lane;
            for (int i0 = 0; i0 < 32; i0 += 8) {
              float acc[8];
#pragma unroll
              for (int i = 0; i < 8; i++) acc[i] = 0.f;
              for (int s = 0; s < P.ksplit; s++) {
                const float* q = base + (int64_t)s * (TM * P.BN) + (int64_t)i0 * P.BN;
#pragma unroll
                for (int i = 0; i < 8; i++) acc[i] += __ldcg(q + (int64_t)i * P.BN);
              }
#pragma unroll
              for (int i = 0; i < 8; i++) stage[(i0 + i) * ALD + lane] = acc[i];
            }
            __syncwarp();
          }
          const int rsub = lane >> 3, c4 = (lane & 7) * 4;
          const int n = n0 + c0 + c4;
          const int ph = P.up_s ? n / P.C : 0;
          const int co = n - ph * P.C;
          float st1[4] = {0.f, 0.f, 0.f, 0.f}, st2[4] = {0.f, 0.f, 0.f, 0.f};
          if (mrow0 < P.Mrows) {
            const int add = P.up_s ? ph - P.up_crop : 0;
            float bias[4], cso[4];
#pragma unroll
            for (int q = 0; q < 4; q++) {
              bias[q] = P.bias ? __ldg(P.bias + co + q) : 0.f;
              cso[q] = (P.cscale ? __ldg(P.cscale + (int64_t)b * P.cscale_bs + co + q) : 1.f) * P.out_scale;
            }
            float* ycol = P.y + (int64_t)b * P.y_bs + co;
            const float* rcol = P.res ? P.res + (int64_t)b * P.res_bs + co : nullptr;
            const int row0 = mrow0 * mul + add;
            const int mvalid = min(32, P.Mrows - mrow0);
            int i_lo = 0, i_hi = mvalid;
            if (row0 < 0) i_lo = (-row0 + mul - 1) / mul;
            if (row0 + (mvalid - 1) * mul >= P.Lout) i_hi = P.Lout > row0 ? (P.Lout - row0 + mul - 1) / mul : 0;
            const bool half_res = P.res_div == 2;
            const float osc = P.out_scale;
            float4 rr[8];
            bool okr[8];
#pragma unroll
            for (int i = 0; i < 8; i++) {
              const int ti = 4 * i + rsub;
              const int row = row0 + ti * mul;
              okr[i] = ti >= i_lo && ti < i_hi;
              rr[i] = make_float4(0.f, 0.f, 0.f, 0.f);
              if (okr[i]) {
                if (rcol) rr[i] = __ldg(reinterpret_cast<const float4*>(rcol + (int64_t)(half_res ? (row >> 1) : row) * P.res_ld));
              }
            }
            if (P.accumulate) {
#pragma unroll
              for (int i = 0; i < 8; i++) {
                if (okr[i]) {
                  const float4 o = *reinterpret_cast<const float4*>(ycol + (int64_t)(row0 + (4 * i + rsub) * mul) * P.y_ld);
                  rr[i].x = fmaf(rr[i].x, osc, o.x); rr[i].y = fmaf(rr[i].y, osc, o.y); rr[i].z = fmaf(rr[i].z, osc, o.z); rr[i].w = fmaf(rr[i].w, osc, o.w);
                }
              }
            } else {
#pragma unroll
              for (int i = 0; i < 8; i++) { rr[i].x *= osc; rr[i].y *= osc; rr[i].z *= osc; rr[i].w *= osc; }
            }
#pragma unroll
            for (int i = 0; i < 8; i++) {
              const int ti = 4 * i + rsub;
              if (okr[i]) {
                const float4 sp = *reinterpret_cast<const float4*>(stage + ti * ALD + c4);
                float a[4] = {sp.x + bias[0], sp.y + bias[1], sp.z + bias[2], sp.w + bias[3]};
                if (P.post_act) {
#pragma unroll
                  for (int q = 0; q < 4; q++) a[q] = act_slow(a[q], P.post_act, P.post_p0);
                }
                float4 v;
                v.x = fmaf(a[0], cso[0], rr[i].x); v.y = fmaf(a[1], cso[1], rr[i].y); v.z = fmaf(a[2], cso[2], rr[i].z); v.w = fmaf(a[3], cso[3], rr[i].w);
                *reinterpret_cast<float4*>(ycol + (int64_t)(row0 + ti * mul) * P.y_ld) = v;
                st1[0] += v.x; st1[1] += v.y; st1[2] += v.z; st1[3] += v.w;
                st2[0] = fmaf(v.x, v.x, st2[0]); st2[1] = fmaf(v.y, v.y, st2[1]); st2[2] = fmaf(v.z, v.z, st2[2]); st2[3] = fmaf(v.w, v.w, st2[3]);
              }
            }
            __syncwarp();
          }
          if (do_stats) {
#pragma unroll
            for (int q = 0; q < 4; q++) {
              st1[q] += __shfl_xor_sync(0xffffffffu, st1[q], 8); st1[q] += __shfl_xor_sync(0xffffffffu, st1[q], 16);
              st2[q] += __shfl_xor_sync(0xffffffffu, st2[q], 8); st2[q] += __shfl_xor_sync(0xffffffffu, st2[q], 16);
            }
            if (rsub == 0) {
#pragma unroll
              for (int q = 0; q < 4; q++) { sacc[(quarter * 2 + 0) * 128 + c0 + c4 + q] = st1[q]; sacc[(quarter * 2 + 1) * 128 + c0 + c4 + q] = st2[q]; }
            }
          }
        }
      }
      __syncwarp();
      if (et == 0) { if (lt == 0) if (DBG) stamp(p, 10); if (DBG) stamp(p, 11); }
      if (lane == 0) mbar_arrive(tempty);
      if (do_stats) {
        bar_sync(1, NWORK * 32);
        if (last_split) {
          const int co0 = P.up_s ? (n0 % P.C) : n0;
          for (int i = et; i < 2 * P.BN; i += NWORK * 32) {
            const int which = i >= P.BN, col = i - which * P.BN;
            const float v = ((sacc[(0 * 2 + which) * 128 + col] + sacc[(1 * 2 + which) * 128 + col]) + sacc[(2 * 2 + which) * 128 + col]) +
                            sacc[(3 * 2 + which) * 128 + col];
            repro_add(P.stats_out + (((int64_t)b * P.C + co0 + col) * 2 + which) * B2A_NBIN, v);
          }
        }
        bar_sync(1, NWORK * 32);
      }
    };

    int prev = -1;
    uint32_t nt_done = 0;
    long long cyc_c = 0, cyc_e = 0;
    for (int tile = blockIdx.x; tile < p.ntiles; tile += gridDim.x) {
      const long long c0_ = DBG ? clock64() : 0;
      convert_tile(tile);
      const long long c1_ = DBG ? clock64() : 0;
      if (prev >= 0) { epilogue_tile(prev, nt_done); nt_done++; }
      if (DBG) { cyc_c += c1_ - c0_; cyc_e += clock64() - c1_; }
      prev = tile;
    }
    { const long long c1_ = DBG ? clock64() : 0; if (prev >= 0) epilogue_tile(prev, nt_done); if (DBG) cyc_e += clock64() - c1_; }
    if (DBG && p.dbg && warp == W_WORK0 && lane == 0) { p.dbg[(size_t)blockIdx.x * 32 + 24] = (unsigned long long)cyc_c; p.dbg[(size_t)blockIdx.x * 32 + 25] = (unsigned long long)cyc_e; }
    if (DBG && p.dbg && warp == W_WORK0 && lane == 0) { p.dbg[(size_t)blockIdx.x * 32 + 19] = w_aempty; p.dbg[(size_t)blockIdx.x * 32 + 20] = w_tfull; }
  }
  if (threadIdx.x == 0) if (DBG) stamp(p, 12);
  __syncthreads();
  if (threadIdx.x == 0) if (DBG) stamp(p, 13);
  if (DBG && p.dbg && threadIdx.x < MW_N)
    p.dbg[(size_t)blockIdx.x * 32 + 26 + threadIdx.x] = mwait_all[threadIdx.x] + mwait_all[MW_N + threadIdx.x];
}

unsigned long long* g_fdbg = nullptr;
thread_local int32_t g_last_cfg[2 + 2 * MAXG] = {};

int n_tile(int N, int C) {
  for (int c = 128; c >= 32; c -= 32) if (N % c == 0 && C % c == 0) return c;
  return 0;
}
int a_rows(int span) { return (TM + span + 7) / 8 * 8; }
int acc_tile_ld(int bn) { return bn + 8; }
int gemm_rows(const b2a_convf_t& q) {
  if (q.up_stride <= 0) return q.Lout;
  const int tail = cdiv(q.Lout + q.up_crop, q.up_stride);
  return q.L + q.taps - 1 > tail ? q.L + q.taps - 1 : tail;
}
int weight_stages(int a_plane, int planes, int acc_ld, int w_stage, size_t* smem) {
  const size_t fixed = (size_t)2 * a_plane * planes + (size_t)TM * acc_ld * 4 + SACC + CTAB + 1024  + 512 ;
  int wst = fixed < DYN_SMEM_MAX ? (int)((DYN_SMEM_MAX - fixed) / w_stage) : 0;
  if (wst > 8) wst = 8;
  if (smem) *smem = fixed + (size_t)wst * w_stage;
  return wst;
}

}

extern "C" int32_t b2a_conv1d_fused_debug(void* buf) { g_fdbg = (unsigned long long*)buf; return B2A_OK; }

extern "C" int32_t b2a_conv1d_fused_last_config(int32_t* out10) {
  B2A_CHECK_ARG(out10, "null pointer");
  for (int i = 0; i < 2 + 2 * MAXG; i++) out10[i] = g_last_cfg[i];
  return B2A_OK;
}

extern "C" int32_t b2a_conv1d_fused_fits(int32_t span, int32_t N, int32_t C, int32_t wplanes, int32_t planes) {
  if (span < 0 || span > 64 || N <= 0 || C <= 0 || N % C || (wplanes != 1 && wplanes != 2) || (planes != 1 && planes != 2)) return 0;
  const int bn = n_tile(N, C);
  return bn && weight_stages(a_rows(span) * 128, planes, acc_tile_ld(bn), bn * 128 * wplanes, nullptr) >= 2;
}

extern "C" int32_t b2a_conv1d_fused(const b2a_convf_t* pr, int32_t n, int32_t planes, int32_t f16, void* ws, int64_t ws_bytes, void* stream) {
  B2A_CHECK_ARG(pr && n >= 1 && n <= MAXG && (planes == 1 || planes == 2), "1..4 problems, planes 1 or 2");
  static const int nsm = [] { const int n = b2a_device_sm_count(); return n > 0 ? n : 132; }();
  FParams p;
  p.G = n; p.planes = planes; p.f16 = f16 ? 1 : 0; p.dbg = g_fdbg;
  { static int flags = -1; if (flags < 0) { const char* e = getenv("B2A_FUSED_DBGFLAGS"); flags = e ? atoi(e) : 0; } p.dbg_flags = flags; }
  int order[MAXG];
  double cost[MAXG];
  for (int i = 0; i < n; i++) { order[i] = i; cost[i] = (double)pr[i].taps * pr[i].cin_pad; }
  for (int i = 0; i < n; i++) for (int j = i + 1; j < n; j++) if (cost[order[j]] > cost[order[i]]) { int t = order[i]; order[i] = order[j]; order[j] = t; }
  int maxR = 0, maxBN = 0, maxWst = 0, tiles_total = 0;
  int64_t base_tiles = 0, sum_base = 0, cnt_used = 0, ws_used = 0;
  for (int gi = 0; gi < n; gi++) {
    const b2a_convf_t& q = pr[gi];
    if (q.N <= 0 || q.N % 32) continue;
    const int bn = n_tile(q.N, q.up_stride > 0 ? q.N / q.up_stride : q.N);
    if (!bn) continue;
    sum_base += (int64_t)cdiv(gemm_rows(q), TM) * (q.N / bn) * q.B;
  }
  for (int gi = 0; gi < n; gi++) {
    const b2a_convf_t& q = pr[order[gi]];
    B2A_CHECK_ARG(q.x && q.w_hi && q.y && q.B > 0 && q.L > 0 && q.Lout > 0 && q.Cin > 0 && q.taps > 0 && q.taps <= 32 && q.cin_pad % 64 == 0 && q.cin_pad >= q.Cin,
                  "bad pointers / shape");
    B2A_CHECK_ARG(q.N % 32 == 0 && q.y_ld % 4 == 0 && (q.res == nullptr || q.res_ld % 4 == 0) && (q.res_div == 1 || q.res_div == 2), "N % 32, row strides % 4, res_div 1|2");
    B2A_CHECK_ARG(((uintptr_t)q.y & 15) == 0 && q.y_bs % 4 == 0 && (q.res == nullptr || (((uintptr_t)q.res & 15) == 0 && q.res_bs % 4 == 0)), "y / res must be 16-byte aligned");
    B2A_CHECK_ARG(q.x_ld % 4 == 0 && q.x_bs % 4 == 0 && ((uintptr_t)q.x & 15) == 0 && q.x_ld >= ((q.Cin + 3) & ~3), "x must be 16-byte aligned with row stride % 4 == 0 and >= ceil4(Cin)");
    B2A_CHECK_ARG((q.x1 == nullptr || ((uintptr_t)q.x1 & 15) == 0) && (q.x2 == nullptr || ((uintptr_t)q.x2 & 15) == 0), "x1 / x2 alignment");
    B2A_CHECK_ARG(q.up_stride >= 0 && (q.up_stride == 0 || (q.N % q.up_stride == 0 && (q.N / q.up_stride) % 32 == 0)), "transposed mode: N = up_stride * C, C % 32 == 0");
    B2A_CHECK_ARG(q.pre_mode >= 0 && q.pre_mode <= 2 && (q.pre_mode != 1 || (q.pre_scale && q.pre_shift)) && (q.pre_mode != 2 || q.pre_stats), "prologue mode / pointers");
    FProb& P = p.pr[gi];
    P.x = q.x; P.x1 = q.x1; P.x2 = q.x2; P.x_bs = q.x_bs; P.x_ld = q.x_ld; P.in_scale = q.in_scale;
    P.B = q.B; P.L = q.L; P.Cin = q.Cin; P.cin_pad = q.cin_pad;
    P.pre_mode = q.pre_mode; P.pre_scale = q.pre_scale; P.pre_shift = q.pre_shift; P.pre_stats = (const long long*)q.pre_stats; P.pre_gb = q.pre_gb;
    P.pre_gb_bs = q.pre_gb_bs; P.pre_eps = q.pre_eps; P.pre_invL = 1.0f / (float)q.L;
    P.pre_act = q.pre_act; P.pre_p0 = q.pre_p0; P.pre_a = q.pre_a; P.pre_b = q.pre_b;
    P.taps = q.taps; P.wplanes = q.w_lo ? 2 : 1; P.Ntot = q.N;
    int smin = q.shifts[0], smax = q.shifts[0];
    for (int i = 0; i < q.taps; i++) { P.shift[i] = q.shifts[i]; smin = q.shifts[i] < smin ? q.shifts[i] : smin; smax = q.shifts[i] > smax ? q.shifts[i] : smax; }
    if (smax - smin > 64) { b2a_set_error("b2a_conv1d_fused: taps span %d rows (> 64)", smax - smin); return B2A_E_UNSUPPORTED; }
    P.shift_min = smin; P.R = a_rows(smax - smin);
    P.up_s = q.up_stride; P.up_crop = q.up_crop; P.C = q.up_stride ? q.N / q.up_stride : q.N;
    P.Lout = q.Lout; P.Mrows = gemm_rows(q);
    P.ntm = cdiv(P.Mrows, TM);
    P.BN = n_tile(q.N, P.C); P.ntn = q.N / P.BN;
    base_tiles = (int64_t)P.ntm * P.ntn * q.B;
    const int kchunks = q.cin_pad / TK;
    P.ksplit = 1;
    if (sum_base * 2 <= nsm && kchunks >= 4 && ws) {
      int ks = (int)(nsm / sum_base);
      if (ks > 8) ks = 8;
      if (ks > kchunks / 2) ks = kchunks / 2;
      if (ks >= 2) P.ksplit = ks;
    }
    P.kper = cdiv(kchunks, P.ksplit);
    P.ksplit = cdiv(kchunks, P.kper);
    P.bias = q.bias; P.post_act = q.post_act; P.post_p0 = q.post_p0; P.cscale = q.cscale; P.cscale_bs = q.cscale_bs;
    P.res = q.res; P.res_bs = q.res_bs; P.res_ld = q.res_ld; P.res_div = q.res_div; P.out_scale = q.out_scale; P.accumulate = q.accumulate;
    P.y = q.y; P.y_bs = q.y_bs; P.y_ld = q.y_ld; P.stats_out = (long long*)q.stats_out;
    P.ws = nullptr; P.counters = nullptr;
    if (P.ksplit > 1) {
      const int64_t bytes = base_tiles * P.ksplit * (TM * P.BN) * 4;
      if (4096 + ws_used + bytes > ws_bytes || cnt_used + base_tiles > 1024) { P.ksplit = 1; P.kper = kchunks; }
      else {
        P.counters = (int*)ws + cnt_used; P.ws = (float*)((uint8_t*)ws + 4096 + ws_used);
        cnt_used += base_tiles; ws_used += bytes;
      }
    }
    P.tile_begin = tiles_total;
    tiles_total += (int)(base_tiles * P.ksplit);
    maxR = P.R > maxR ? P.R : maxR; maxBN = P.BN > maxBN ? P.BN : maxBN;
    const int wsz = P.BN * 128 * P.wplanes;
    maxWst = wsz > maxWst ? wsz : maxWst;
  }
  p.ntiles = tiles_total;
  p.a_plane = maxR * 128;
  p.w_stage = maxWst;
  p.acc_ld = acc_tile_ld(maxBN);
  size_t smem = 0;
  const int wst = weight_stages(p.a_plane, planes, p.acc_ld, p.w_stage, &smem);
  if (wst < 2) { b2a_set_error("b2a_conv1d_fused: shared memory cannot hold two weight stages (R %d, BN %d)", maxR, maxBN); return B2A_E_UNSUPPORTED; }
  p.wst = wst;

  CUtensorMap mw[MAXG], ml[MAXG];
  for (int gi = 0; gi < MAXG; gi++) {
    const b2a_convf_t& q = pr[order[gi < n ? gi : 0]];
    const FProb& P = p.pr[gi < n ? gi : 0];
    const uint64_t wdims[2] = {(uint64_t)q.cin_pad, (uint64_t)q.taps * q.N}, wstr[1] = {(uint64_t)q.cin_pad * 2};
    const uint32_t wbox[2] = {TK, (uint32_t)P.BN};
    int e = b2a_tmap16(&mw[gi], q.w_hi, 2, wdims, wstr, wbox, p.f16);
    if (!e) e = b2a_tmap16(&ml[gi], q.w_lo ? q.w_lo : q.w_hi, 2, wdims, wstr, wbox, p.f16);
    if (e) { b2a_set_error("b2a_conv1d_fused: cuTensorMapEncodeTiled failed (%d)", e); return B2A_E_CUDA; }
  }
  const bool dbg = p.dbg != nullptr || p.dbg_flags != 0;
  const auto kern = dbg ? conv_fused_kernel<true> : conv_fused_kernel<false>;
  B2A_SMEM_OPTIN(kern, DYN_SMEM_MAX);
  const int grid = tiles_total < nsm ? tiles_total : nsm;
  cudaError_t err = b2a_launch_pdl(kern, dim3(grid), dim3(THREADS), smem, (cudaStream_t)stream, p, mw[0], mw[1], mw[2], mw[3], ml[0], ml[1],
                                   ml[2], ml[3]);
  if (err != cudaSuccess) { b2a_set_error("b2a_conv1d_fused: launch failed: %s", cudaGetErrorString(err)); return B2A_E_CUDA; }
  B2A_CHECK_LAUNCH();
  for (int i = 0; i < 2 + 2 * MAXG; i++) g_last_cfg[i] = 0;
  g_last_cfg[0] = n; g_last_cfg[1] = grid;
  for (int gi = 0; gi < n; gi++) { g_last_cfg[2 + 2 * order[gi]] = p.pr[gi].BN; g_last_cfg[3 + 2 * order[gi]] = p.pr[gi].ksplit; }
  return B2A_OK;
}
```

mlx_audio_b200/ops.py:

```python
from __future__ import annotations

import ctypes as C
import math
import contextlib
import os
from dataclasses import dataclass
from typing import Optional

import torch

from . import _lib
from ._lib import AttnParams, Conv1dParams, ConvFParams

ACT = {"none": 0, "lrelu": 1, "snake": 2, "elu": 3, "gelu": 4, "gelu_tanh": 5, "tanh": 6, "sigmoid": 7,
       "silu": 8, "clip1": 9}

LAUNCHES = [0]


PROFILE = None
PROFILE_TAGS = None
TAG = [None]
PROFILE_EXTERNAL = False

# ... 307 lines not shown

def conv1d_cl_last_path() -> dict:
    out = (C.c_int32 * 4)()
    _lib.check(_lib.lib().b2a_conv1d_cl_last_path(out))
    return {"kernel": CL_PATHS.get(out[0]), "variant": (out[1], out[2], out[3])}


def conv1d_tc_last_config() -> dict:
    out = (C.c_int32 * 5)()
    _lib.check(_lib.lib().b2a_conv1d_tc_last_config(out))
    return {"BN": out[0], "grid": (out[1], out[2], out[3]), "stages": out[4]}


def conv1d_fused_last_config() -> dict:
    out = (C.c_int32 * 10)()
    _lib.check(_lib.lib().b2a_conv1d_fused_last_config(out))
    n = out[0]
    return {"grid": out[1], "BN": [out[2 + 2 * i] for i in range(n)], "ksplit": [out[3 + 2 * i] for i in range(n)]}


FUSED = [os.environ.get("B2A_FUSED", "1") != "0"]
FUSED_DISPATCH = [os.environ.get("B2A_FUSED_DISPATCH", "0") == "1"]


@contextlib.contextmanager
def fused_dispatch(on: bool = True):
    old = FUSED_DISPATCH[0]
    FUSED_DISPATCH[0] = bool(on) and FUSED[0]
    try:
        yield
    finally:
        FUSED_DISPATCH[0] = old
FUSED_WS_BYTES = 16 << 20
_FUSED_WS = {}


@dataclass
class PreStats:
    stats: torch.Tensor
    gb: Optional[torch.Tensor] = None
    eps: float = 1e-5
    act: int = 0
    p0: float = 0.0
    a: Optional[torch.Tensor] = None
    b: Optional[torch.Tensor] = None


STAT_BINS, STAT_BIN0, STAT_BIN_BITS = 4, -100, 40


def new_stats(B: int, Cc: int, device) -> torch.Tensor:
    return torch.zeros(B, Cc, 2, STAT_BINS, device=device, dtype=torch.int64)


def stats_value(stats: torch.Tensor) -> torch.Tensor:
    w = torch.tensor([2.0 ** (STAT_BIN0 + STAT_BIN_BITS * k) for k in range(STAT_BINS)], dtype=torch.float64, device=stats.device)
    t = torch.zeros(stats.shape[:-1], dtype=torch.float64, device=stats.device)
    for k in range(STAT_BINS - 1, -1, -1):
        t = t + stats[..., k].double() * w[k]
    return t


def _al16(t: Optional[torch.Tensor]) -> bool:
    return t is None or (t.data_ptr() % 16 == 0 and t.stride(1) % 4 == 0 and t.stride(0) % 4 == 0)


def fused_eligible(x, cw: "ConvW", stride: int = 1, dilation: int = 1, transpose: bool = False, pad_mode: int = 0, out=None, res=None) -> bool:
    if not FUSED[0] or TC_MODE[0] == "off" or cw.w_tc is None or pad_mode != 0 or cw.cout % 32 != 0 or cw.groups != 1 or isinstance(x, Planes):
        return False
    if x.dtype != torch.float32 or x.dim() != 3 or x.stride(2) != 1 or x.stride(1) % 4 or x.stride(0) % 4 or x.data_ptr() % 16:
        return False
    if x.stride(1) < -(-x.shape[2] // 4) * 4 or not _al16(out) or not _al16(res):
        return False
    if transpose:
        if not (dilation == 1 and cw.K % stride == 0 and cw.K // stride <= 32 and cw.cin * (cw.K // stride) >= TC_MIN_K):
            return False
        span, n_total = cw.K // stride - 1, stride * cw.cout
    else:
        if not (stride == 1 and cw.K <= 32 and cw.cin * cw.K >= TC_MIN_K):
            return False
        span, n_total = (cw.K - 1) * dilation, cw.cout
    return bool(_lib.lib().b2a_conv1d_fused_fits(span, n_total, cw.cout, 1 if cw.w_tc_lo is None else 2, 2 if TC_MODE[0] == "x2" else 1))


class FusedProblem:

    def __init__(self, x, cw: "ConvW", *, stride=1, dilation=1, pad_left=0, lout=None, pre=None, x_add=(), in_scale=1.0, post_act=0, post_p0=0.0,
                 cscale=None, res=None, res_div=1, out_scale=1.0, out=None, accumulate=False, transpose=False, stats_out=None):
        _chk3(x, "conv_fused x")
        B, L, cin = x.shape
        if cin != cw.cin:
            raise ValueError(f"conv_fused: input has {cin} channels, weight expects {cw.cin}")
        if lout is None:
            lout = (L - 1) * stride + cw.K - 2 * pad_left if transpose else (L + 2 * pad_left - dilation * (cw.K - 1) - 1) + 1
        if out is None:
            out = torch.empty(B, lout, cw.cout, device=x.device, dtype=torch.float32)
        else:
            _chk3(out, "conv_fused out")
            if out.shape != (B, lout, cw.cout):
                raise ValueError(f"conv_fused: out has shape {tuple(out.shape)}, expected {(B, lout, cw.cout)}")
        p = ConvFParams()
        p.x, p.x_bs, p.x_ld, p.in_scale = x.data_ptr(), x.stride(0), x.stride(1), float(in_scale)
        keep = [x, out, cw]
        for i, xa in enumerate(x_add):
            if xa.shape != x.shape or xa.stride() != x.stride() or xa.dtype != torch.float32:
                raise ValueError("conv_fused: x_add tensors must have x's shape and strides")
            setattr(p, "x1" if i == 0 else "x2", xa.data_ptr())
            keep.append(xa)
        p.B, p.L, p.Cin = B, L, cin
        if isinstance(pre, PreStats):
            if pre.stats.dtype != torch.int64 or tuple(pre.stats.shape) != (B, cin, 2, STAT_BINS) or not pre.stats.is_contiguous():
                raise ValueError("conv_fused: stats must be a contiguous int64 [B, Cin, 2, 4] tensor (ops.new_stats)")
            p.pre_mode, p.pre_stats, p.pre_eps = 2, pre.stats.data_ptr(), float(pre.eps)
            if pre.gb is not None:
                if pre.gb.shape[-1] != 2 * cin or pre.gb.stride(-1) != 1:
                    raise ValueError("conv_fused: gb must be [B, 2*Cin] rows (gamma | beta)")
                p.pre_gb, p.pre_gb_bs = pre.gb.data_ptr(), (pre.gb.stride(0) if pre.gb.dim() == 2 and pre.gb.shape[0] == B and B > 1 else 0)
            keep += [pre.stats, pre.gb]
        elif pre is not None and pre.scale is not None:
            p.pre_mode, p.pre_scale, p.pre_shift = 1, pre.scale.data_ptr(), pre.shift.data_ptr()
            keep += [pre.scale, pre.shift]
        if pre is not None:
            p.pre_act, p.pre_p0, p.pre_a, p.pre_b = pre.act, float(pre.p0), _p(pre.a), _p(pre.b)
            keep += [pre.a, pre.b]
        if transpose:
            taps, n_total = cw.K // stride, stride * cw.cout
            w_tc, w_lo = _tc_transposed_weights(cw, stride)
            shifts = [-j for j in range(taps)]
            p.up_stride, p.up_crop = stride, pad_left
        else:
            taps, n_total, w_tc, w_lo = cw.K, cw.cout, cw.w_tc, cw.w_tc_lo
            shifts = [k * dilation - pad_left for k in range(taps)]
        p.w_hi, p.w_lo, p.cin_pad, p.taps, p.N = w_tc.data_ptr(), _p(w_lo), cw.cin_pad, taps, n_total
        for i, sft in enumerate(shifts):
            p.shifts[i] = sft
        p.Lout, p.bias, p.post_act, p.post_p0 = lout, _p(cw.bias), post_act, float(post_p0)
        if cscale is not None:
            p.cscale, p.cscale_bs = cscale.data_ptr(), (cscale.stride(0) if cscale.dim() == 2 else 0)
            keep.append(cscale)
        if res is not None:
            _chk3(res, "conv_fused res")
            p.res, p.res_bs, p.res_ld = res.data_ptr(), (res.stride(0) if res.shape[0] == B else 0), res.stride(1)
            keep.append(res)
        p.res_div, p.out_scale, p.accumulate = res_div, float(out_scale), int(accumulate)
        p.y, p.y_bs, p.y_ld = out.data_ptr(), out.stride(0), out.stride(1)
        if stats_out is not None:
            if stats_out.dtype != torch.int64 or tuple(stats_out.shape) != (B, cw.cout, 2, STAT_BINS) or not stats_out.is_contiguous():
                raise ValueError("conv_fused: stats_out must be a contiguous int64 [B, Cout, 2, 4] tensor (ops.new_stats)")
            p.stats_out = stats_out.data_ptr()
            keep.append(stats_out)
        self.p, self.out, self.keep, self.f16 = p, out, keep, cw.f16


def conv_fused(problems) -> list:
    if isinstance(problems, FusedProblem):
        problems = [problems]
    n = len(problems)
    if not 1 <= n <= 4:
        raise ValueError("conv_fused: 1..4 problems per launch")
    f16 = problems[0].f16
    if any(pr.f16 != f16 for pr in problems):
        raise ValueError("conv_fused: all problems of a launch must use the same 16-bit operand type")
    arr = (ConvFParams * n)(*[pr.p for pr in problems])
    dev = problems[0].out.device
    key = (dev, torch.cuda.current_stream().cuda_stream)
    ws = _FUSED_WS.get(key)
    if ws is None:
        ws = _FUSED_WS[key] = torch.zeros(FUSED_WS_BYTES, device=dev, dtype=torch.uint8)
    if PROFILE_TAGS is not None:
        TAG[0] = "fused " + " + ".join(f"[{q.B}x{q.L}x{q.Cin}->{q.N} k{q.taps}{' up' + str(q.up_stride) if q.up_stride else ''}]" for q in (pr.p for pr in problems))
    _call("conv_tc", _lib.lib().b2a_conv1d_fused, 1, arr, n, 2 if TC_MODE[0] == "x2" else 1, int(f16), ws.data_ptr(), ws.numel(), _stream())
    return [pr.out for pr in problems]


def linear(x, cw: ConvW, *, planes=False, qkv_heads=0, qkv_scale=0.0, **kw):
    if planes or qkv_heads:
        if isinstance(x, torch.Tensor) and x.dim() != 3:
            raise ValueError("linear: planes= / qkv_heads= need a 3-D operand")
        B, L, _ = x.shape
        if not emit_tc_eligible(cw, L):
            raise ValueError("linear: planes= / qkv_heads= need a tensor-core layer (ops.emit_tc_eligible)")
        for k in ("out", "res"):
            t = kw.get(k)
            if t is not None and t.dim() == 2:
                kw[k] = t[None]
        out, pre, res = kw.pop("out", None), kw.pop("pre", None), kw.pop("res", None)
        post_act, post_p0, cscale, out_scale = kw.pop("post_act", 0), kw.pop("post_p0", 0.0), kw.pop("cscale", None), kw.pop("out_scale", 1.0)
        if kw:
            raise TypeError(f"linear: unsupported arguments with planes= / qkv_heads=: {sorted(kw)}")
        if isinstance(x, Planes) and (pre is not None or x.C != cw.cin or x.hi.shape[2] != cw.cin_pad or x.hi.dtype != torch.bfloat16):
            raise ValueError("linear: a Planes operand needs matching channels and dtype and takes no prologue")
        if out is None:
            out = torch.empty(B, L, cw.cout, device=cw.w.device, dtype=torch.float32)
        em = at = None
        if qkv_heads:
            if cw.cout != 3 * 64 * qkv_heads:
                raise ValueError(f"linear: qkv_heads={qkv_heads} needs Cout = {3 * 64 * qkv_heads}, got {cw.cout}")
            at = AttnPlanes(torch.empty(_lib.lib().b2a_attention_tc_ws_bytes(B, qkv_heads, L, L), device=out.device, dtype=torch.uint8),
                            B, L, qkv_heads)
        else:
            em = _new_planes(B, L, cw.cout, out.device)
        y = _conv1d_tc(x, cw, 1, 0, L, pre, post_act, post_p0, cscale, res, 1, out_scale, out, False, emit=em, attn=at, attn_scale=qkv_scale)
        return y, (at if qkv_heads else em)
    if isinstance(x, torch.Tensor) and x.dim() == 2:
        o = kw.get("out")
        if o is not None and o.dim() == 2:
            kw["out"] = o[None]
        r = kw.get("res")
        if r is not None and r.dim() == 2:
            kw["res"] = r[None]
        return conv1d(x[None], cw, **kw)[0]
    return conv1d(x, cw, **kw)


def copy2d(src: torch.Tensor, dst: torch.Tensor) -> None:
    rows, cols = src.shape
    assert dst.shape == src.shape and src.stride(1) == 1 and dst.stride(1) == 1
    _call("other", _lib.lib().b2a_copy2d, 1, src.data_ptr(), src.stride(0), dst.data_ptr(), dst.stride(0), rows, cols, _stream())


def stream_rows(entries) -> None:
    entries = [e for e in entries if e[0].numel()]
    if len(entries) > _lib.ROWOPS_MAX:
        raise ValueError(f"stream_rows: at most {_lib.ROWOPS_MAX} entries per launch, got {len(entries)}")
    if not entries:
        return
    arr = (_lib.RowOp * len(entries))()
    for i, (src, dst, add) in enumerate(entries):
        _chk3(src, "stream_rows src")
        _chk3(dst, "stream_rows dst")
        if src.shape != dst.shape:
            raise ValueError(f"stream_rows: source {tuple(src.shape)} and destination {tuple(dst.shape)} differ")
        B, rows, Cc = src.shape
        arr[i] = _lib.RowOp(src.data_ptr(), src.stride(0), src.stride(1), dst.data_ptr(), dst.stride(0), dst.stride(1), B, rows, Cc, int(bool(add)))
    _call("other", _lib.lib().b2a_stream_rows, 1, arr, len(entries), _stream())


def _stream_conv_params(x, cw: ConvW, B: int, L: int, lout: int, out, stride: int, dilation: int, pad_mode: int, pre: Optional[Pre],
                        post_act: int, res, res_div: int) -> Conv1dParams:
    p = Conv1dParams()
    if L:
        _chk3(x, "stream conv x")
        p.x, p.x_bs, p.x_ld = x.data_ptr(), x.stride(0), x.stride(1)
    p.B, p.L, p.Cin = B, L, cw.cin
    p.w, p.bias = cw.w.data_ptr(), _p(cw.bias)
    if lout:
        p.y, p.y_bs, p.y_ld = out.data_ptr(), out.stride(0), out.stride(1)
    p.Lout, p.Cout = lout, cw.cout
    p.K, p.stride, p.dilation, p.groups, p.pad_mode = cw.K, stride, dilation, cw.groups, pad_mode
    if pre is not None:
        if pre.scale is not None or pre.shift is not None or pre.a is not None or pre.b is not None:
            raise ValueError("stream conv: the prologue is an activation only")
        p.pre_act, p.pre_p0 = pre.act, pre.p0
    p.post_act = post_act
    if res is not None:
        _chk3(res, "stream conv res")
        p.res, p.res_bs, p.res_ld = res.data_ptr(), res.stride(0), res.stride(1)
    p.res_div, p.out_scale = res_div, 1.0
    return p


def conv1d_stream(x: Optional[torch.Tensor], cw: ConvW, hist: torch.Tensor, H: int, step: torch.Tensor, *, B=None, stride=1, dilation=1,
                  pad_mode=0, fresh=False, pre: Optional[Pre] = None, post_act=0, res=None, res_div=1, out=None) -> torch.Tensor:
    L = 0 if x is None else x.shape[1]
    B = x.shape[0] if x is not None else B
    keff = (cw.K - 1) * dilation + 1
    lout = (H + L - keff) // stride + 1 if H + L >= keff else 0
    if hist.dtype != torch.float32 or not hist.is_contiguous() or hist.shape != (2, B, max(keff - 1, 1), cw.cin):
        raise ValueError(f"conv1d_stream: history buffer must be float32 [2, {B}, {max(keff - 1, 1)}, {cw.cin}], got {tuple(hist.shape)}")
    if out is None:
        out = torch.empty(B, lout, cw.cout, device=hist.device, dtype=torch.float32)
    p = _stream_conv_params(x, cw, B, L, lout, out, stride, dilation, pad_mode, pre, post_act, res, res_div)
    _call("conv", _lib.lib().b2a_conv1d_stream, 1, C.byref(p), hist.data_ptr(), hist.stride(1), H, step.data_ptr(), int(fresh), _stream())
    return out


def convtr1d_stream(x: torch.Tensor, cw: ConvW, tail: torch.Tensor, *, stride: int, pre: Optional[Pre] = None, out=None) -> torch.Tensor:
    _chk3(x, "convtr1d_stream x")
    B, L, _ = x.shape
    if not tail.is_contiguous() or tail.shape != (B, cw.K - stride, cw.cout):
        raise ValueError(f"convtr1d_stream: tail must be contiguous [{B}, {cw.K - stride}, {cw.cout}], got {tuple(tail.shape)}")
    if out is None:
        out = torch.empty(B, L * stride, cw.cout, device=x.device, dtype=torch.float32)
    p = _stream_conv_params(x, cw, B, L, L * stride, out, stride, 1, 0, pre, 0, None, 1)
    _call("conv", _lib.lib().b2a_convtr1d_stream, 1, C.byref(p), tail.data_ptr(), tail.stride(0), _stream())
    return out


def ring_rope_kv(qkv: torch.Tensor, n_heads: int, k_ring: torch.Tensor, v_ring: torch.Tensor, pos: torch.Tensor, *, base: float) -> None:
    _chk3(qkv, "ring_rope_kv qkv")
    B, T, w = qkv.shape
    D = w // (3 * n_heads)
    _call("rope", _lib.lib().b2a_ring_rope_kv, 1, qkv.data_ptr(), qkv.stride(0), qkv.stride(1), B, T, n_heads, D, base, k_ring.data_ptr(),
          v_ring.data_ptr(), k_ring.stride(0), k_ring.shape[1], pos.data_ptr(), _stream())


def ring_attn(q: torch.Tensor, k_ring: torch.Tensor, v_ring: torch.Tensor, pos: torch.Tensor, *, n_heads: int, scale: float, window: int,
              out=None) -> torch.Tensor:
    _chk3(q, "ring_attn q")
    B, T, hd = q.shape
    if out is None:
        out = torch.empty(B, T, hd, device=q.device, dtype=torch.float32)
    _call("attention", _lib.lib().b2a_ring_attn, 1, q.data_ptr(), q.stride(0), q.stride(1), k_ring.data_ptr(), v_ring.data_ptr(), k_ring.stride(0),
          k_ring.shape[1], out.data_ptr(), out.stride(0), out.stride(1), B, T, n_heads, hd // n_heads, scale, window, pos.data_ptr(), _stream())
    return out


def stream_advance(ctr: torch.Tensor, dpos: int) -> None:
    assert ctr.dtype == torch.int32 and ctr.numel() >= 2
    _call("other", _lib.lib().b2a_stream_advance, 1, ctr.data_ptr(), dpos, _stream())


def gather_rows(src: torch.Tensor, idx: torch.Tensor, out: Optional[torch.Tensor] = None, add: Optional[torch.Tensor] = None) -> torch.Tensor:
    assert src.dim() == 2 and src.stride(1) == 1 and idx.dtype == torch.int64 and idx.is_contiguous()
    rows, cols = idx.shape[0], src.shape[1]
    if out is None:
        out = torch.empty(rows, cols, device=src.device, dtype=torch.float32)
    a, a_ld, a_per = (None, 0, 0) if add is None else (add.data_ptr(), add.stride(0), add.shape[0])
    _call("other", _lib.lib().b2a_gather_rows, 1, src.data_ptr(), src.stride(0), idx.data_ptr(), out.data_ptr(), out.stride(0),
          rows, cols, src.shape[0], a, a_ld, a_per, _stream())
    return out


def whisper_greedy_step(logits: torch.Tensor, tokens: torch.Tensor, cur_len: int, sample_begin: int, *, suppress_mask, blank_mask,
                        eot: int, no_timestamps: int, timestamp_begin: int, max_initial_ts: int, without_timestamps: bool,
# ... 797 lines not shown
```

mlx_audio_b200/tts/models/kokoro/kokoro.py:

```python
from __future__ import annotations

import functools
import math
import time
import weakref
from dataclasses import dataclass
from numbers import Number
from typing import Dict, Optional

import torch

from .... import ops
from ....ops import ACT, ConvW, Pre
from ..base import BaseModelArgs, GenerationResult, check_array_shape


def _fused_layers(fn):
    @functools.wraps(fn)
    def wrapped(*a, **k):
        with ops.fused_dispatch(True):
            return fn(*a, **k)
    return wrapped


# ... 146 lines not shown
                blk[lst].append((a.contiguous(), (1.0 / a).contiguous()))
        return blk

    def _prepare(self, P, strict):
        cfg, dev = self.config, self.device
        W = {}
        ada = _AdaSlots()
        f = lambda t: t.float().to(dev).contiguous()
        B = "bert."
        W["word_emb"] = f(P[B + "embeddings.word_embeddings.weight"])
        W["pos_type"] = f(P[B + "embeddings.position_embeddings.weight"].float()
                          + P[B + "embeddings.token_type_embeddings.weight"][0].float()[None])
        W["emb_ln"] = (f(P[B + "embeddings.LayerNorm.weight"]), f(P[B + "embeddings.LayerNorm.bias"]))
        W["map_in"] = self._lin(P, B + "encoder.embedding_hidden_mapping_in")
        L = B + "encoder.albert_layer_groups.0.albert_layers.0."
        wqkv = torch.cat([P[L + f"attention.{n}.weight"].float() for n in ("query", "key", "value")], 0)
        bqkv = torch.cat([P[L + f"attention.{n}.bias"].float() for n in ("query", "key", "value")], 0)
        W["qkv"] = ops.pack_linear(wqkv, bqkv, dev)
        W["attn_out"] = self._lin(P, L + "attention.dense")
        W["attn_ln"] = (f(P[L + "attention.LayerNorm.weight"]), f(P[L + "attention.LayerNorm.bias"]))
        W["ffn"] = self._lin(P, L + "ffn")
        W["ffn_out"] = self._lin(P, L + "ffn_output")
        W["full_ln"] = (f(P[L + "full_layer_layer_norm.weight"]), f(P[L + "full_layer_layer_norm.bias"]))
        W["bert_encoder"] = self._lin(P, "bert_encoder")
        W["dur_lstms"] = []
        for i in range(cfg.n_layer):
            W["dur_lstms"].append(self._lstm(P, f"predictor.text_encoder.lstms.{2 * i}"))
            ada.add(f"adaln.{i}", P[f"predictor.text_encoder.lstms.{2 * i + 1}.fc.weight"], P[f"predictor.text_encoder.lstms.{2 * i + 1}.fc.bias"])
        W["pred_lstm"] = self._lstm(P, "predictor.lstm")
        dpad = -cfg.max_dur % 32
        dw, db = P["predictor.duration_proj.linear_layer.weight"].float(), P["predictor.duration_proj.linear_layer.bias"].float()
        W["dur_proj"] = ops.pack_linear(torch.cat([dw, dw.new_zeros(dpad, dw.shape[1])], 0), torch.cat([db, db.new_zeros(dpad)], 0), dev)
        W["dur_sum"] = ops.pack_linear(torch.cat([torch.ones(1, cfg.max_dur), torch.zeros(1, dpad)], 1), None, dev)
        W["shared"] = self._lstm(P, "predictor.shared")
        for name in ("F0", "N"):
            W[name] = [self._resblk1d(P, f"predictor.{name}.0", ada), self._resblk1d(P, f"predictor.{name}.1", ada, True),
                       self._resblk1d(P, f"predictor.{name}.2", ada)]
            W[name + "_proj"] = ops.pack_conv(P[f"predictor.{name}_proj.weight"].float(), P[f"predictor.{name}_proj.bias"], 1, dev)
        W["te_emb"] = f(P["text_encoder.embedding.weight"])
        W["te_cnn"] = [(self._cw(P, f"text_encoder.cnn.{i}.0"), f(P[f"text_encoder.cnn.{i}.1.weight"]), f(P[f"text_encoder.cnn.{i}.1.bias"]))
                       for i in range(cfg.n_layer)]
        W["te_lstm"] = self._lstm(P, "text_encoder.lstm")
        W["encode"] = self._resblk1d(P, "decoder.encode", ada)
        W["decode"] = [self._resblk1d(P, f"decoder.decode.{i}", ada, (f"decoder.decode.{i}.pool.weight_v") in P) for i in range(4)]
        W["F0_conv"] = self._cw(P, "decoder.F0_conv")
        W["N_conv"] = self._cw(P, "decoder.N_conv")
        W["asr_res"] = self._cw(P, "decoder.asr_res.0")
        ist = cfg.istftnet
        G = "decoder.generator"
        W["src_lin"] = (f(P[G + ".m_source.l_linear.weight"]).reshape(-1), f(P[G + ".m_source.l_linear.bias"]).reshape(-1))
        rates, ks, rk, rd = ist["upsample_rates"], ist["upsample_kernel_sizes"], ist["resblock_kernel_sizes"], ist["resblock_dilation_sizes"]
        W["ups"], W["noise_convs"], W["noise_res"], W["resblocks"] = [], [], [], []
        for i in range(len(rates)):
            W["ups"].append(self._cw(P, f"{G}.ups.{i}", transpose_layout=True))
            W["noise_convs"].append(ops.pack_conv(P[f"{G}.noise_convs.{i}.weight"].float(), P[f"{G}.noise_convs.{i}.bias"], 1, dev))
            W["noise_res"].append(self._resblock1(P, f"{G}.noise_res.{i}", ada, 7 if i + 1 < len(rates) else 11, (1, 3, 5)))
            for j in range(len(rk)):
                W["resblocks"].append(self._resblock1(P, f"{G}.resblocks.{i * len(rk) + j}", ada, rk[j], tuple(rd[j])))
        wp = fold_weight_norm(P[G + ".conv_post.weight_v"], P[G + ".conv_post.weight_g"])
        bp = P[G + ".conv_post.bias"].float()
        n_post = wp.shape[0]
        if n_post % 32:
            padn = -(-n_post // 32) * 32 - n_post
            wp = torch.cat([wp, torch.zeros(padn, *wp.shape[1:], dtype=wp.dtype)], 0)
            bp = torch.cat([bp, torch.zeros(padn, dtype=bp.dtype)], 0)
        W["conv_post"] = ops.pack_conv(wp, bp, 1, self.device)
        W["n_post"] = n_post
        W["ada_all"] = ops.pack_linear(torch.cat(ada.ws, 0), torch.cat(ada.bs, 0), dev)
        self._ada_slices = ada.slices
        self._ada_pred = [k for k in ada.slices if k.startswith("adaln.") or k.startswith("predictor.")]
        self._w = W

    def _tap(self, name, t):
        if self.tap is not None:
            self.tap[name] = t.detach().clone()

    def _gb(self, name):
        off, n = self._ada_slices[name]
        src = self._gb_pred if name in self._pred_set else self._gb_dec
        return src[:, off:off + n]

    def _lstm_run(self, x2d, lw, out=None):
        xproj = ops.linear(x2d, lw[0])
        return ops.lstm_bidir(xproj[None], lw[1], out=None if out is None else out[None])[0]

    def _adain_resblk1d(self, x, blk, out=None):
        s1, h1 = ops.adain_coeffs(x, self._gb(blk["name"] + ".norm1").contiguous())
        pre1 = Pre(s1, h1, ACT["lrelu"], 0.2)
        L = x.shape[1]
        if blk["up"]:
            r = ops.conv1d(x, blk["pool"], stride=2, pad_left=1, lout=2 * L, pre=pre1, transpose=True)
            r = ops.conv1d(r, blk["conv1"], pad_left=1)
        else:
            r = ops.conv1d(x, blk["conv1"], pad_left=1, pre=pre1)
        s2, h2 = ops.adain_coeffs(r, self._gb(blk["name"] + ".norm2").contiguous())
        sc = ops.conv1d(x, blk["sc"]) if "sc" in blk else x
        return ops.conv1d(r, blk["conv2"], pad_left=1, pre=Pre(s2, h2, ACT["lrelu"], 0.2), res=sc,
                          res_div=2 if blk["up"] else 1, out_scale=1.0 / math.sqrt(2.0), out=out)

    def _adain_resblock1(self, x, blk, out=None, out_scale=1.0, accumulate=False, defer_last=False):
        k = blk["k"]
        for j, d in enumerate(blk["dils"]):
            s1, h1 = ops.adain_coeffs(x, self._gb(f"{blk['name']}.adain1.{j}").contiguous())
            a, ia = blk["a1"][j]
            xt = ops.conv1d(x, blk["c1"][j], dilation=d, pad_left=(k * d - d) // 2, pre=Pre(s1, h1, ACT["snake"], 0.0, a, ia))
            s2, h2 = ops.adain_coeffs(xt, self._gb(f"{blk['name']}.adain2.{j}").contiguous())
            a, ia = blk["a2"][j]
            last = j == len(blk["dils"]) - 1
            if last and defer_last:
                def final(xt=xt, s2=s2, h2=h2, a=a, ia=ia, x=x, j=j):
                    return ops.conv1d(xt, blk["c2"][j], pad_left=(k - 1) // 2, pre=Pre(s2, h2, ACT["snake"], 0.0, a, ia), res=x,
                                      out=out, out_scale=out_scale, accumulate=accumulate)
                return final
            if last:
                x = ops.conv1d(xt, blk["c2"][j], pad_left=(k - 1) // 2, pre=Pre(s2, h2, ACT["snake"], 0.0, a, ia), res=x,
                               out=out, out_scale=out_scale, accumulate=accumulate)
            else:
                x = ops.conv1d(xt, blk["c2"][j], pad_left=(k - 1) // 2, pre=Pre(s2, h2, ACT["snake"], 0.0, a, ia), res=x)
        return x


    def _stats(self, C: int) -> torch.Tensor:
        if self._stats_pool is not None:
            t = self._stats_pool.pop(0)
            assert t.shape[1] == C
            return t
        n = 2 * ops.STAT_BINS * C
        off = self._arena_off
        self._arena_off += n
        assert self._arena_off <= self._arena.numel()
        return self._arena[off:off + n].view(1, C, 2, ops.STAT_BINS)

    def _resblk1d_group(self, xs, sxs, blks, outs=None, sos=None):
        n = len(blks)
        outs = outs or [None] * n
        sos = sos or [None] * n
        up = blks[0]["up"]
        L = xs[0].shape[1]
        lrelu = ACT["lrelu"]
        s1 = [self._stats(b["conv1"].cout) for b in blks]
        first = []
        if up:
            rs = []
            for x, sx, b in zip(xs, sxs, blks):
                sc, sh = ops.coeffs_from_stats(sx, L, self._gb(b["name"] + ".norm1"))
                cpad = -(-x.shape[2] // 4) * 4
                r = torch.empty(1, 2 * L, cpad, device=x.device, dtype=torch.float32)[:, :, :x.shape[2]]
                rs.append(ops.conv1d(x, b["pool"], stride=2, pad_left=1, lout=2 * L, pre=Pre(sc, sh, lrelu, 0.2), transpose=True, out=r))
            first = [ops.FusedProblem(r, b["conv1"], pad_left=1, stats_out=st) for r, b, st in zip(rs, blks, s1)]
        else:
            first = [ops.FusedProblem(x, b["conv1"], pad_left=1, pre=ops.PreStats(sx, self._gb(b["name"] + ".norm1"), 1e-5, lrelu, 0.2), stats_out=st)
                     for x, sx, b, st in zip(xs, sxs, blks, s1)]
        shortcut = [ops.FusedProblem(x, b["sc"]) for x, b in zip(xs, blks) if "sc" in b]
        res = ops.conv_fused(first + shortcut) if len(first) + len(shortcut) <= 4 else ops.conv_fused(first) + ops.conv_fused(shortcut)
        r1 = res[:n]
        scs = res[n:] if shortcut else xs
        second = [ops.FusedProblem(r, b["conv2"], pad_left=1, pre=ops.PreStats(st, self._gb(b["name"] + ".norm2"), 1e-5, lrelu, 0.2), res=sc,
                                   res_div=2 if up else 1, out_scale=1.0 / math.sqrt(2.0), out=o, stats_out=so)
                  for r, b, st, sc, o, so in zip(r1, blks, s1, scs, outs, sos)]
        return ops.conv_fused(second)

    def _resblock1_group(self, xs, sxs, blks, outs=None):
        n = len(blks)
        outs = outs or [None] * n
        cur, scur = list(xs), list(sxs)
        for j in range(3):
            last = j == 2
            st1 = [self._stats(b["c1"][j].cout) for b in blks]
            c1 = [ops.FusedProblem(x, b["c1"][j], dilation=b["dils"][j], pad_left=(b["k"] * b["dils"][j] - b["dils"][j]) // 2,
                                   pre=ops.PreStats(sx, self._gb(f"{b['name']}.adain1.{j}"), 1e-5, ACT["snake"], 0.0, *b["a1"][j]), stats_out=st)
                  for x, sx, b, st in zip(cur, scur, blks, st1)]
            xt = ops.conv_fused(c1)
            snew = [None if last else self._stats(b["c2"][j].cout) for b in blks]
            c2 = [ops.FusedProblem(t, b["c2"][j], pad_left=(b["k"] - 1) // 2,
                                   pre=ops.PreStats(st, self._gb(f"{b['name']}.adain2.{j}"), 1e-5, ACT["snake"], 0.0, *b["a2"][j]), res=x,
                                   out=outs[i] if last else None, stats_out=sn)
                  for i, (t, st, x, b, sn) in enumerate(zip(xt, st1, cur, blks, snew))]
            cur, scur = ops.conv_fused(c2), snew
        return cur

    @torch.no_grad()
    def _acoustic_side_fused(self, st, F: int, noise=None, f0n_override=None):
        W, cfg, dev = self._w, self.config, self.device
        self._bind(st)
        hd = cfg.hidden_dim
        par = self.concurrent
        X, t_en = st["X"], st["t_en"]
        idx = st["idx"][:F]
        self._arena = torch.zeros(1 << 19, device=dev, dtype=torch.int64)
        self._arena_off = 0
        en = ops.gather_rows(X, idx)
        xs = self._lstm_run(en, W["shared"])[None]
        sxs = self._stats(xs.shape[2])
        ops.channel_stats(xs, sxs)
        F0N = torch.empty(2, 2 * F, 1, device=dev, dtype=torch.float32)
        hcur, scur = [xs, xs], [sxs, sxs]
        for bi in range(3):
            blks = [W["F0"][bi], W["N"][bi]]
            sos = [self._stats(b["conv2"].cout) for b in blks] if bi < 2 else None
            hcur = self._resblk1d_group(hcur, scur, blks, sos=sos)
            scur = sos
        ops.conv1d(hcur[0], W["F0_proj"], out=F0N[0:1])
        ops.conv1d(hcur[1], W["N_proj"], out=F0N[1:2])
        if f0n_override is not None:
            F0N[0, :, 0].copy_(torch.as_tensor(f0n_override[0]).to(device=dev, dtype=torch.float32).reshape(-1))
            F0N[1, :, 0].copy_(torch.as_tensor(f0n_override[1]).to(device=dev, dtype=torch.float32).reshape(-1))
        f0_curve, n_curve = F0N[0:1], F0N[1:2]
        self._tap("en", en)
        self._tap("F0", f0_curve)
        self._tap("N", n_curve)
        ist = cfg.istftnet
        rates, ks = ist["upsample_rates"], ist["upsample_kernel_sizes"]
        nk = len(ist["resblock_kernel_sizes"])
        n_har = 120 * F + 1
        xsrcs = []
        for i in range(len(rates)):
            sf0 = math.prod(rates[i + 1:]) if i + 1 < len(rates) else 1
            Li = (n_har + 2 * ((sf0 + 1) // 2) - (2 * sf0 - 1) - 1) // sf0 + 1 if sf0 > 1 else n_har
            xsrcs.append(torch.empty(1, Li, W["noise_convs"][i].cout, device=dev, dtype=torch.float32))
        src_stats = [self._stats(W["noise_convs"][i].cout) for i in range(len(rates))]
        src_arena = [[self._stats(W["noise_convs"][i].cout) for _ in range(5)] for i in range(len(rates))]

        def source_branch():
            har = ops.kokoro_source(f0_curve.reshape(1, 2 * F), noise, *W["src_lin"])
            self._tap("har", har)
            ts = []
            for i in range(len(rates)):
                if i + 1 < len(rates):
                    sf0 = math.prod(rates[i + 1:])
                    t = ops.kokoro_source_conv(har, W["noise_convs"][i], stride=sf0, pad_left=(sf0 + 1) // 2)
                else:
                    t = ops.kokoro_source_conv(har, W["noise_convs"][i])
                ops.channel_stats(t, src_stats[i])
                ts.append(t)
            pool, self._stats_pool = self._stats_pool, [s for group in zip(*src_arena) for s in group]
            try:
                self._resblock1_group(ts, src_stats, W["noise_res"], outs=xsrcs)
            finally:
                self._stats_pool = pool

        if par:
            side_src = ops.fork(dev, 1)
            with torch.cuda.stream(side_src[0]):
                source_branch()
        b514 = torch.empty(1, F, hd + 4, device=dev, dtype=torch.float32)[:, :, :hd + 2]
        ops.gather_rows(t_en, idx, out=b514[0, :, :hd])
        ops.conv1d(f0_curve, W["F0_conv"], stride=2, pad_left=1, out=b514[:, :, hd:hd + 1])
        ops.conv1d(n_curve, W["N_conv"], stride=2, pad_left=1, out=b514[:, :, hd + 1:hd + 2])
        bufs = [torch.empty(1, F, 1024 + 64 + 4, device=dev, dtype=torch.float32)[:, :, :1024 + 64 + 2] for _ in range(2)]
        ops.conv1d(b514[:, :, :hd], W["asr_res"], out=bufs[0][:, :, 1024:1088])
        ops.copy2d(b514[0, :, hd:], bufs[0][0, :, 1088:])
        ops.copy2d(bufs[0][0, :, 1024:], bufs[1][0, :, 1024:])
        s514 = self._stats(hd + 2)
        ops.channel_stats(b514, s514)
        nblk = len(W["decode"])
        sbuf = [self._stats(1024 + 64 + 2) for _ in range(nblk)]
        ops.channel_stats(bufs[0][:, :, 1024:], [sb[:, 1024:] for sb in sbuf])
        self._resblk1d_group([b514], [s514], [W["encode"]], outs=[bufs[0][:, :, :1024]], sos=[sbuf[0][:, :1024]])
        self._tap("dec_encode", bufs[0][:, :, :1024])
        cur = 0
        x = None
        for i, blk in enumerate(W["decode"]):
            if blk["up"]:
                x = self._resblk1d_group([bufs[cur]], [sbuf[i]], [blk])[0]
            else:
                self._resblk1d_group([bufs[cur]], [sbuf[i]], [blk], outs=[bufs[1 - cur][:, :, :1024]], sos=[sbuf[i + 1][:, :1024]])
                cur = 1 - cur
        self._tap("dec_out", x)
        if par:
            ops.join(dev, side_src)
        else:
            source_branch()
        x_add, in_scale = (), 1.0
        for i, (u, kk) in enumerate(zip(rates, ks)):
            last = i == len(rates) - 1
            xsrc = xsrcs[i]
            L = x.shape[1]
            lout = (L - 1) * u + kk - 2 * ((kk - u) // 2)
            cout = W["ups"][i].cout
            sy = self._stats(cout)
            pre = Pre(act=ACT["lrelu"], p0=0.1)
            if last:
                y = torch.empty(1, lout + 1, cout, device=dev, dtype=torch.float32)
                ops.copy2d(xsrc[0, :1], y[0, :1])
                ops.channel_stats(y[:, :1], sy)
                ops.conv_fused(ops.FusedProblem(x, W["ups"][i], stride=u, pad_left=(kk - u) // 2, pre=pre, transpose=True, res=xsrc[:, 1:],
                                                out=y[:, 1:], x_add=x_add, in_scale=in_scale, stats_out=sy))
            else:
                y = ops.conv_fused(ops.FusedProblem(x, W["ups"][i], stride=u, pad_left=(kk - u) // 2, pre=pre, transpose=True, res=xsrc,
                                                    x_add=x_add, in_scale=in_scale, stats_out=sy))[0]
            blks = [W["resblocks"][i * nk + j] for j in range(nk)]
            outs = self._resblock1_group([y] * nk, [sy] * nk, blks)
            x, x_add, in_scale = outs[0], tuple(outs[1:]), 1.0 / nk
            if self.tap is not None:
                self._tap(f"gen_stage{i}", sum(outs) / nk)
        xpost = ops.conv_fused(ops.FusedProblem(x, W["conv_post"], pad_left=3, pre=Pre(act=ACT["lrelu"], p0=0.01), x_add=x_add,
                                                in_scale=in_scale))[0][:, :, :W["n_post"]]
        self._tap("xpost", xpost)
        return ops.kokoro_istft_head(xpost)[0]

    @torch.no_grad()
    @_fused_layers
    def _text_side(self, ids, ref_s, speed: float = 1.0, pred_dur=None):
        W, cfg, dev = self._w, self.config, self.device
        T = ids.shape[0]
        s_dec, s_pred = ref_s[:, :128].contiguous(), ref_s[:, 128:].contiguous()
        st = {"T": T}
        st["gb_pred"] = ops.linear(s_pred, W["ada_all"])
        st["gb_dec"] = ops.linear(s_dec, W["ada_all"])
        self._bind(st)
        hd = cfg.hidden_dim
        par = self.concurrent
        t_en = torch.empty(T, hd, device=dev, dtype=torch.float32)

        def text_branch():
            te = ops.gather_rows(W["te_emb"], ids)[None]
            k = cfg.text_encoder_kernel_size
            for cw, lw, lb in W["te_cnn"]:
                te = ops.conv1d(te, cw, pad_left=(k - 1) // 2)
                te = ops.layernorm(te, lw, lb, eps=1e-5, post_act=ACT["lrelu"], post_p0=0.2)
            self._lstm_run(te[0], W["te_lstm"], out=t_en)

        e = ops.gather_rows(W["word_emb"], ids)
        nh = cfg.plbert["num_attention_heads"]
        hs = cfg.plbert["hidden_size"]
        scale = 1.0 / math.sqrt(hs // nh)
        if self._albert_planes(T):
            _, ep = ops.layernorm(e, *W["emb_ln"], eps=1e-12, res=W["pos_type"][:T], planes=True)
            h, hp = ops.linear(ep, W["map_in"], planes=True)
            ops.albert_encoder(h, hp, cfg.plbert["num_hidden_layers"], W["qkv"], W["attn_out"], W["ffn"], W["ffn_out"], W["attn_ln"],
                               W["full_ln"], heads=nh, scale=scale, eps=1e-12)
            h = h[0]
        else:
            with ops.fused_dispatch(False):
                e = ops.layernorm(e, *W["emb_ln"], eps=1e-12, res=W["pos_type"][:T])
                h = ops.linear(e, W["map_in"])
                for _ in range(cfg.plbert["num_hidden_layers"]):
                    qkv = ops.linear(h, W["qkv"])[None]
                    ctx = ops.attention(qkv[:, :, :hs], qkv[:, :, hs:2 * hs], qkv[:, :, 2 * hs:], n_heads=nh, scale=scale)[0]
                    a = ops.linear(ctx, W["attn_out"], res=h)
                    a = ops.layernorm(a, *W["attn_ln"], eps=1e-12)
                    f1 = ops.linear(a, W["ffn"], post_act=ACT["gelu"])
                    f2 = ops.linear(f1, W["ffn_out"], res=a)
                    h = ops.layernorm(f2, *W["full_ln"], eps=1e-12)
        self._tap("bert", h)
        if par:
            side_text = ops.fork(dev, 1)
            with torch.cuda.stream(side_text[0]):
                text_branch()
        stl = cfg.style_dim
        X = torch.empty(T, hd + stl, device=dev, dtype=torch.float32)
        ops.linear(h, W["bert_encoder"], out=X[:, :hd])
        ops.copy2d(s_pred.expand(T, stl), X[:, hd:])
        for i in range(cfg.n_layer):
            o = self._lstm_run(X, W["dur_lstms"][i])
            ops.layernorm(o, eps=1e-5, ada=self._gb(f"adaln.{i}").reshape(-1).contiguous(), out=X[:, :hd])
        xl = self._lstm_run(X, W["pred_lstm"])
        dsig = ops.linear(xl, W["dur_proj"], post_act=ACT["sigmoid"])
        dsum = ops.linear(dsig, W["dur_sum"]).reshape(-1).contiguous()
        self._tap("d", X)
        self._tap("dur", dsum)
        max_frames = 100 * T
        if pred_dur is not None:
            pred, idx, total = ops.durations_to_index(pred_dur, max_frames)
        else:
            pred, idx, total = ops.durations_to_index(dsum, max_frames, float(speed))
        if par:
            ops.join(dev, side_text)
        else:
            text_branch()
        self._tap("t_en", t_en)
        st.update(X=X, t_en=t_en, pred=pred, idx=idx, total=total)
        return st

    def _albert_planes(self, T: int) -> bool:
        W, pb = self._w, self.config.plbert
        return (64 <= T <= 512 and ops.ATTN_MODE[0] == "tc" and pb["hidden_size"] == 64 * pb["num_attention_heads"]
                and pb["hidden_size"] % 64 == 0 and W["map_in"].cin % 64 == 0
                and all(ops.emit_tc_eligible(W[k], T) and W[k].w_tc_lo is None for k in ("map_in", "qkv", "attn_out", "ffn", "ffn_out")))

    def _bind(self, st):
        self._pred_set = set(self._ada_pred)
        self._gb_pred, self._gb_dec = st["gb_pred"], st["gb_dec"]

    @torch.no_grad()
    @_fused_layers
    def _acoustic_side(self, st, F: int, noise=None, f0n_override=None):
        if ops.FUSED[0] and ops.TC_MODE[0] != "off":
            return self._acoustic_side_fused(st, F, noise, f0n_override)
        W, cfg, dev = self._w, self.config, self.device
        self._bind(st)
        hd = cfg.hidden_dim
        par = self.concurrent
        X, t_en = st["X"], st["t_en"]
        idx = st["idx"][:F]
        en = ops.gather_rows(X, idx)
        xs = self._lstm_run(en, W["shared"])[None]
        F0N = torch.empty(2, 2 * F, 1, device=dev, dtype=torch.float32)

        def head(n_i, name):
            hcur = xs
            for blk in W[name]:
                hcur = self._adain_resblk1d(hcur, blk)
            ops.conv1d(hcur, W[name + "_proj"], out=F0N[n_i:n_i + 1])

        if par:
            side = ops.fork(dev, 1)
            with torch.cuda.stream(side[0]):
                head(1, "N")
            head(0, "F0")
            ops.join(dev, side)
        else:
            head(0, "F0")
            head(1, "N")
        if f0n_override is not None:
            F0N[0, :, 0].copy_(torch.as_tensor(f0n_override[0]).to(device=dev, dtype=torch.float32).reshape(-1))
            F0N[1, :, 0].copy_(torch.as_tensor(f0n_override[1]).to(device=dev, dtype=torch.float32).reshape(-1))
        f0_curve, n_curve = F0N[0:1], F0N[1:2]
        self._tap("en", en)
        self._tap("F0", f0_curve)
        self._tap("N", n_curve)
        ist = cfg.istftnet
        rates, ks = ist["upsample_rates"], ist["upsample_kernel_sizes"]
        nk = len(ist["resblock_kernel_sizes"])
        n_har = 120 * F + 1
        xsrcs, Lh = [], n_har
        for i in range(len(rates)):
            sf0 = math.prod(rates[i + 1:]) if i + 1 < len(rates) else 1
            Li = (n_har + 2 * ((sf0 + 1) // 2) - (2 * sf0 - 1) - 1) // sf0 + 1 if sf0 > 1 else n_har
            xsrcs.append(torch.empty(1, Li, W["noise_convs"][i].cout, device=dev, dtype=torch.float32))
        del Lh

        def source_branch():
            har = ops.kokoro_source(f0_curve.reshape(1, 2 * F), noise, *W["src_lin"])
            self._tap("har", har)
            for i in range(len(rates)):
                if i + 1 < len(rates):
                    sf0 = math.prod(rates[i + 1:])
                    t = ops.conv1d(har, W["noise_convs"][i], stride=sf0, pad_left=(sf0 + 1) // 2)
                else:
                    t = ops.conv1d(har, W["noise_convs"][i])
                self._adain_resblock1(t, W["noise_res"][i], out=xsrcs[i])

        if par:
            side_src = ops.fork(dev, 1)
# ... 228 lines not shown
```

Before: 1832.

## Chain dependent fused conv stages in one persistent launch with grid barriers

After: 1824, median of 6. Within noise of the previous version (-0.4%).

```diff
diff --git a/include/b200audio.h b/include/b200audio.h
--- a/include/b200audio.h
+++ b/include/b200audio.h
@@ -154,7 +154,9 @@
   int64_t* stats_out;
 } b2a_convf_t;
 int32_t b2a_conv1d_fused_debug(void* stamps );
-int32_t b2a_conv1d_fused(const b2a_convf_t* problems, int32_t n_problems, int32_t planes, int32_t f16, void* ws, int64_t ws_bytes, void* stream);
+#define B2A_CONVF_MAX_STAGES 4
+int32_t b2a_conv1d_fused(const b2a_convf_t* problems, const int32_t* counts, int32_t n_stages, int32_t planes, int32_t f16, void* ws,
+                         int64_t ws_bytes, uint32_t* bar, uint32_t* err, int32_t grid, void* stream);
 int32_t b2a_conv1d_fused_fits(int32_t span, int32_t N, int32_t C, int32_t wplanes, int32_t planes);
 int32_t b2a_conv1d_fused_last_config(int32_t* out10);
 
diff --git a/mlx_audio_b200/_lib.py b/mlx_audio_b200/_lib.py
--- a/mlx_audio_b200/_lib.py
+++ b/mlx_audio_b200/_lib.py
@@ -90,7 +90,7 @@
     "b2a_conv1d_tc_last_config": (i32, [C.POINTER(i32)]),
     "b2a_conv1d_fused_debug": (i32, [c_f]),
     "b2a_conv1d_fused_last_config": (i32, [C.POINTER(i32)]),
-    "b2a_conv1d_fused": (i32, [C.POINTER(ConvFParams), i32, i32, i32, c_f, i64, C.c_void_p]),
+    "b2a_conv1d_fused": (i32, [C.POINTER(ConvFParams), C.POINTER(i32), i32, i32, i32, c_f, i64, c_f, c_f, i32, C.c_void_p]),
     "b2a_conv1d_fused_fits": (i32, [i32, i32, i32, i32, i32]),
     "b2a_copy2d": (i32, [c_f, i64, c_f, i64, i64, i32, C.c_void_p]),
     "b2a_gather_rows": (i32, [c_f, i64, c_f, c_f, i64, i64, i32, i64, c_f, i64, i64, C.c_void_p]),
diff --git a/mlx_audio_b200/csrc/albert.cu b/mlx_audio_b200/csrc/albert.cu
--- a/mlx_audio_b200/csrc/albert.cu
+++ b/mlx_audio_b200/csrc/albert.cu
@@ -3,6 +3,7 @@
 #include "tc_epilogue.cuh"
 #include "attn_tc_tile.cuh"
 #include "layernorm_row.cuh"
+#include "grid_barrier.cuh"
 
 using namespace tc;
 
@@ -16,7 +17,6 @@
 constexpr int OFF_BAR = OFF_Q + 2 * PLANE;
 constexpr int SMEM_BYTES = OFF_BAR + (2 * SLOTS + 2) * 8 + 16 + 1024;
 constexpr int STAGES = 7;
-constexpr long long TIMEOUT_NS = 10000000000LL;
 
 struct AlbertMaps {
   CUtensorMap a_hi[4], a_lo[4], w[4];
@@ -39,34 +39,6 @@
 
 __device__ __forceinline__ int gemm_of_stage(int s) { return s == 0 ? 0 : s == 2 ? 1 : s == 4 ? 2 : s == 5 ? 3 : -1; }
 
-__device__ __forceinline__ long long globaltimer() {
-  long long t;
-  asm volatile("mov.u64 %0, %globaltimer;" : "=l"(t));
-  return t;
-}
-
-__device__ bool grid_wait(const AlbertParams& p, unsigned target) {
-  long long t0 = 0;
-  for (int it = 0;; it++) {
-    unsigned v;
-    asm volatile("ld.acquire.gpu.global.u32 %0, [%1];" : "=r"(v) : "l"(p.bar) : "memory");
-    if ((int)(v - target) >= 0) return true;
-    if ((it & 63) == 63) {
-      if (*(volatile unsigned*)p.err) return false;
-      const long long now = globaltimer();
-      if (!t0) t0 = now;
-      else if (now - t0 > TIMEOUT_NS) { atomicExch(p.err, 1u); return false; }
-    }
-    __nanosleep(64);
-  }
-}
-
-__device__ __forceinline__ void grid_arrive(unsigned* bar) {
-  asm volatile("red.release.gpu.global.add.u32 [%0], 1;" ::"l"(bar) : "memory");
-}
-
-__device__ __forceinline__ void fence_proxy_async_global() { asm volatile("fence.proxy.async.global;" ::: "memory"); }
-
 template <bool TL>
 __global__ void __launch_bounds__(THREADS, 1) albert_kernel(const __grid_constant__ AlbertMaps maps, const AlbertParams p) {
   extern __shared__ __align__(1024) uint8_t smem_raw[];
@@ -99,8 +71,8 @@
       if (stage == 1) {
         const int units = p.H * p.mb;
         if (bid >= units) continue;
-        grid_wait(p, (unsigned)k * grid);
-        fence_proxy_async_global();
+        gridbar::wait(p.bar, p.err, (unsigned)k * grid);
+        gridbar::fence_proxy_async_global();
         for (int u = bid; u < units; u += grid) {
           const int head = u / p.mb, q0 = (u % p.mb) * 64;
           mbar_wait(q_empty, (qn & 1) ^ 1);
@@ -137,8 +109,8 @@
             mbar_expect_tx(full + s, bytes);
             tma_load_2d(smem + (size_t)s * SLOT_BYTES + 2 * PLANE, &maps.w[gi], full + s, c * 64, n0);
           }
-          grid_wait(p, (unsigned)k * grid);
-          fence_proxy_async_global();
+          gridbar::wait(p.bar, p.err, (unsigned)k * grid);
+          gridbar::fence_proxy_async_global();
           waited = true;
           for (int c = 0; c < pre; c++) {
             const int s = (g + c) % SLOTS;
@@ -169,10 +141,10 @@
   for (int k = 0; k < total; k++) {
     const int stage = k % STAGES, gi = gemm_of_stage(stage);
     if (k > 0) {
-      if (ct == 0) grid_wait(p, (unsigned)k * grid);
+      if (ct == 0) gridbar::wait(p.bar, p.err, (unsigned)k * grid);
       bar_sync(1, 256);
     }
-    if constexpr (TL) { if (ct == 0) p.tl[((int64_t)k * grid + bid) * 2] = globaltimer(); }
+    if constexpr (TL) { if (ct == 0) p.tl[((int64_t)k * grid + bid) * 2] = gridbar::globaltimer(); }
     if (gi >= 0) {
       const int units = p.mb * (p.N[gi] / 64), kc = p.K[gi] / 64, N = p.N[gi];
       const float* bias = p.bias[gi];
@@ -283,11 +255,11 @@
                              el ? el + o : nullptr, lane);
       }
     }
-    if constexpr (TL) { if (ct == 0) p.tl[((int64_t)k * grid + bid) * 2 + 1] = globaltimer(); }
+    if constexpr (TL) { if (ct == 0) p.tl[((int64_t)k * grid + bid) * 2 + 1] = gridbar::globaltimer(); }
     if (k + 1 < total) {
-      fence_proxy_async_global();
+      gridbar::fence_proxy_async_global();
       bar_sync(1, 256);
-      if (ct == 0) { __threadfence(); grid_arrive(p.bar); }
+      if (ct == 0) { __threadfence(); gridbar::arrive(p.bar); }
     }
   }
 }
diff --git a/mlx_audio_b200/csrc/conv_fused.cu b/mlx_audio_b200/csrc/conv_fused.cu
--- a/mlx_audio_b200/csrc/conv_fused.cu
+++ b/mlx_audio_b200/csrc/conv_fused.cu
@@ -1,6 +1,8 @@
 #include "common.cuh"
 #include "tc_common.cuh"
+#include "grid_barrier.cuh"
 #include <stdlib.h>
+#include <string.h>
 
 using namespace tc;
 
@@ -10,6 +12,7 @@
 constexpr int TK = 64;
 
 constexpr int MAXG = B2A_CONVF_MAX_PROBLEMS;
+constexpr int MAXS = B2A_CONVF_MAX_STAGES;
 constexpr int NWORK = 8;
 constexpr int NSUB = NWORK / 4;
 constexpr int WG_PROD = 2;
@@ -48,6 +51,7 @@
   int tile_begin;
 };
 
+
 struct FParams {
   int G, ntiles, planes, f16, wst, w_stage, a_plane, acc_ld;
   unsigned long long* dbg;
@@ -55,6 +59,16 @@
   FProb pr[MAXG];
 };
 constexpr size_t DYN_SMEM_MAX = (size_t)227 * 1024 - ((sizeof(FParams) + 1023) & ~(size_t)1023);
+
+template <int NS>
+struct FChain {
+  CUtensorMap mw[NS][MAXG], ml[NS][MAXG];
+  FParams st[NS];
+  int nst;
+  unsigned* bar;
+  unsigned* err;
+};
+static_assert(sizeof(FChain<MAXS>) <= 32764, "the chain must fit the kernel parameter space");
 
 struct TileRef { int g, b, mt, nt, ks; };
 
@@ -120,8 +134,14 @@
   }
 }
 
+__device__ __forceinline__ float4 ld_stage4(const float* p) {
+  float4 v;
+  asm volatile("ld.global.v4.f32 {%0, %1, %2, %3}, [%4];" : "=f"(v.x), "=f"(v.y), "=f"(v.z), "=f"(v.w) : "l"(p));
+  return v;
+}
+
 template <typename T16, int ACT, int NADD, int U>
-__device__ __forceinline__ void convert_chunk(const float* __restrict__ xb, const float* __restrict__ xb1, const float* __restrict__ xb2, int64_t x_ld,
+__device__ __forceinline__ void convert_chunk(const float* xb, const float* xb1, const float* xb2, int64_t x_ld,
                                               int L, int lbase, int ch, int c4, int r0, int R, bool anych, const float sc[4], const float sh[4],
                                               const float aa[4], const float bb[4], const bool chok[4], int act, float p0, uint8_t* hi, uint8_t* lo,
                                               int flags = 0) {
@@ -135,9 +155,9 @@
       ok[u] = rr < R && l >= 0 && l < L && anych;
       const int64_t off = ok[u] ? (int64_t)l * x_ld + ch : 0;
       if (flags & 1) v[u] = make_float4((float)rr, 1.f, 2.f, 3.f); else
-      v[u] = __ldg(reinterpret_cast<const float4*>(xb + off));
-      if constexpr (NADD > 0) w1[u] = __ldg(reinterpret_cast<const float4*>(xb1 + off));
-      if constexpr (NADD > 1) w2[u] = __ldg(reinterpret_cast<const float4*>(xb2 + off));
+      v[u] = ld_stage4(xb + off);
+      if constexpr (NADD > 0) w1[u] = ld_stage4(xb1 + off);
+      if constexpr (NADD > 1) w2[u] = ld_stage4(xb2 + off);
     }
 #pragma unroll
     for (int u = 0; u < U; u++) {
@@ -250,25 +270,36 @@
   }
 };
 
-template <bool DBG>
-__global__ void __launch_bounds__(THREADS, 1)
-conv_fused_kernel(const __grid_constant__ FParams gp, const __grid_constant__ CUtensorMap mw0, const __grid_constant__ CUtensorMap mw1,
-                  const __grid_constant__ CUtensorMap mw2, const __grid_constant__ CUtensorMap mw3,
-                  const __grid_constant__ CUtensorMap ml0, const __grid_constant__ CUtensorMap ml1,
-                  const __grid_constant__ CUtensorMap ml2, const __grid_constant__ CUtensorMap ml3) {
+template <bool DBG, int NS>
+__device__ __forceinline__ void conv_fused_body(const FChain<NS>& gc) {
+  const int nst = NS == 1 ? 1 : gc.nst;
   extern __shared__ __align__(1024) uint8_t smem_raw[];
   uint8_t* smem = (uint8_t*)(((uintptr_t)smem_raw + 1023) & ~(uintptr_t)1023);
   const int warp = threadIdx.x >> 5, lane = threadIdx.x & 31;
   __shared__ __align__(16) FParams sparams;
   __shared__ unsigned long long mwait_all[DBG ? 2 * MW_N : 1];
-  {
-    const uint32_t* src = reinterpret_cast<const uint32_t*>(&gp);
+  __shared__ unsigned long long wcyc[2];
+  auto load_stage = [&](const int st, const int t0, const int nt) {
+    const uint32_t* src = reinterpret_cast<const uint32_t*>(&gc.st[st]);
     uint32_t* dst = reinterpret_cast<uint32_t*>(&sparams);
-    for (int i = threadIdx.x; i < (int)(sizeof(FParams) / 4); i += THREADS) dst[i] = src[i];
-    if (DBG && threadIdx.x < 2 * MW_N) mwait_all[threadIdx.x] = 0;
-  }
+    for (int i = threadIdx.x - t0; i < (int)(sizeof(FParams) / 4); i += nt) dst[i] = src[i];
+  };
+  load_stage(0, 0, THREADS);
+  if (DBG && threadIdx.x < 2 * MW_N) mwait_all[threadIdx.x] = 0;
+  if (DBG && threadIdx.x < 2) wcyc[threadIdx.x] = 0;
   __syncthreads();
   const FParams& p = sparams;
+  auto next_stage = [&](const int st, const bool copy) {
+    bar_sync(4, THREADS);
+    if (threadIdx.x == 0) {
+      __threadfence();
+      gridbar::arrive(gc.bar);
+      gridbar::wait(gc.bar, gc.err, (unsigned)st * gridDim.x);
+      gridbar::fence_proxy_async_global();
+    }
+    if (copy) load_stage(st, (W_PROD + 1) * 32, 3 * 32);
+    bar_sync(4, THREADS);
+  };
   if (threadIdx.x == 0) if (DBG) stamp(p, 0);
 
   if (warp == W_PROD && lane == 0) {
@@ -286,40 +317,58 @@
   const int wgi = __shfl_sync(0xffffffffu, (int)(threadIdx.x >> 7), 0);
   if (wgi == WG_PROD) {
     set_regs<REG_PROD>();
-    if (warp == W_PROD && lane == 0) {
-      const SmemLayout sl(smem, p);
-      uint8_t* const wbase = sl.wbase;
-      uint64_t* const full = sl.full;
-      uint64_t* const empty = sl.empty;
-      const CUtensorMap* mws[MAXG] = {&mw0, &mw1, &mw2, &mw3};
-      const CUtensorMap* mls[MAXG] = {&ml0, &ml1, &ml2, &ml3};
-      for (int g = 0; g < p.G; g++) {
-        asm volatile("prefetch.tensormap [%0];" ::"l"(mws[g]) : "memory");
-        if (p.pr[g].wplanes == 2) asm volatile("prefetch.tensormap [%0];" ::"l"(mls[g]) : "memory");
-      }
-      int s = 0; uint32_t ph = 0;
-      unsigned long long w_pempty = 0;
-      const long long pt0 = DBG ? clock64() : 0;
-      for (int tile = blockIdx.x; tile < p.ntiles; tile += gridDim.x) {
-        const TileRef t = decode_tile(p, tile);
-        const FProb& P = p.pr[t.g];
+    const bool issuer = warp == W_PROD && lane == 0;
+    const SmemLayout sl(smem, p);
+    uint8_t* const wbase = sl.wbase;
+    uint64_t* const full = sl.full;
+    uint64_t* const empty = sl.empty;
+    int s = 0; uint32_t ph = 0;
+    unsigned long long w_pempty = 0;
+    const long long pt0 = DBG ? clock64() : 0;
+    auto prefetch_maps = [&](const FParams& q, const int st) {
+      for (int g = 0; g < q.G; g++) {
+        asm volatile("prefetch.tensormap [%0];" ::"l"(&gc.mw[st][g]) : "memory");
+        if (q.pr[g].wplanes == 2) asm volatile("prefetch.tensormap [%0];" ::"l"(&gc.ml[st][g]) : "memory");
+      }
+    };
+    auto issue = [&](const FParams& q, const int st, const int from, const int to) {
+      int n = 0;
+      for (int tile = blockIdx.x; tile < q.ntiles; tile += gridDim.x) {
+        const TileRef t = decode_tile(q, tile);
+        const FProb& P = q.pr[t.g];
         const int n0 = t.nt * P.BN;
         const int kchunks = P.cin_pad / TK;
         const int kc0 = t.ks * P.kper, kc1 = min(kchunks, kc0 + P.kper);
         const uint32_t wb = (uint32_t)P.BN * 128u;
         for (int kc = kc0; kc < kc1; kc++) {
-          for (int tap = 0; tap < P.taps; tap++) {
+          for (int tap = 0; tap < P.taps; tap++, n++) {
+            if (n == to) return n;
+            if (n < from) continue;
             TIMED_WAIT(p, w_pempty, mbar_wait(empty + s, ph ^ 1));
-            uint8_t* st = wbase + (size_t)s * p.w_stage;
+            uint8_t* sp = wbase + (size_t)s * p.w_stage;
             mbar_expect_tx(full + s, wb * (uint32_t)P.wplanes);
-            tma_load_2d(st, mws[t.g], full + s, kc * TK, tap * P.Ntot + n0);
-            if (P.wplanes == 2) tma_load_2d(st + wb, mls[t.g], full + s, kc * TK, tap * P.Ntot + n0);
+            tma_load_2d(sp, &gc.mw[st][t.g], full + s, kc * TK, tap * P.Ntot + n0);
+            if (P.wplanes == 2) tma_load_2d(sp + wb, &gc.ml[st][t.g], full + s, kc * TK, tap * P.Ntot + n0);
             if (++s == p.wst) { s = 0; ph ^= 1; }
           }
         }
       }
-      if (DBG && p.dbg) { p.dbg[(size_t)blockIdx.x * 32 + 21] = (unsigned long long)(clock64() - pt0); p.dbg[(size_t)blockIdx.x * 32 + 22] = w_pempty; }
-    }
+      return n;
+    };
+    if (issuer) prefetch_maps(p, 0);
+    int early = 0;
+    for (int st = 0; st < nst; st++) {
+      if (st) next_stage(st, warp != W_PROD);
+      if (issuer) {
+        issue(p, st, early, 0x7fffffff);
+        if (st + 1 < nst) {
+          prefetch_maps(gc.st[st + 1], st + 1);
+          early = issue(gc.st[st + 1], st + 1, 0, p.wst);
+        }
+      }
+      __syncwarp();
+    }
+    if (DBG && issuer && p.dbg) { p.dbg[(size_t)blockIdx.x * 32 + 21] = (unsigned long long)(clock64() - pt0); p.dbg[(size_t)blockIdx.x * 32 + 22] = w_pempty; }
   } else if (wgi < WG_PROD) {
     set_regs<REG_MMA>();
     const SmemLayout sl(smem, p);
@@ -327,13 +376,16 @@
     uint64_t *const tfull = sl.tfull, *const tempty = sl.tempty;
     float* const acct = sl.acct;
     const uint32_t a0 = smem_u32(smem), w0 = smem_u32(sl.wbase);
-    const bool f16 = gp.f16 != 0, two_a = gp.planes == 2;
+    const bool f16 = gc.st[0].f16 != 0, two_a = gc.st[0].planes == 2;
     uint32_t s = 0, ph = 0, lt = 0, cg = 0;
     float acc[4 * 16];
 #pragma unroll
     for (int i = 0; i < 4 * 16; i++) acc[i] = 0.f;
     unsigned long long* const mwait = mwait_all + (DBG ? wgi * MW_N : 0);
-    for (int tile = blockIdx.x; tile < gp.ntiles; tile += gridDim.x, lt++) {
+    for (int st = 0; st < nst; st++) {
+    if (st) next_stage(st, false);
+    const int ntiles = __shfl_sync(0xffffffffu, p.ntiles, 0);
+    for (int tile = blockIdx.x; tile < ntiles; tile += gridDim.x, lt++) {
       const TileRef t = decode_tile(p, tile);
       const FProb& P = p.pr[t.g];
       const MmaCtl c = mma_ctl(P, t);
@@ -346,6 +398,7 @@
         default: B2A_MMA_TILE(4); break;
       }
 #undef B2A_MMA_TILE
+    }
     }
   } else {
     set_regs<REG_WORK>();
@@ -533,7 +586,7 @@
               okr[i] = ti >= i_lo && ti < i_hi;
               rr[i] = make_float4(0.f, 0.f, 0.f, 0.f);
               if (okr[i]) {
-                if (rcol) rr[i] = __ldg(reinterpret_cast<const float4*>(rcol + (int64_t)(half_res ? (row >> 1) : row) * P.res_ld));
+                if (rcol) rr[i] = ld_stage4(rcol + (int64_t)(half_res ? (row >> 1) : row) * P.res_ld);
               }
             }
             if (P.accumulate) {
@@ -598,19 +651,23 @@
       }
     };
 
-    int prev = -1;
     uint32_t nt_done = 0;
-    long long cyc_c = 0, cyc_e = 0;
-    for (int tile = blockIdx.x; tile < p.ntiles; tile += gridDim.x) {
-      const long long c0_ = DBG ? clock64() : 0;
-      convert_tile(tile);
-      const long long c1_ = DBG ? clock64() : 0;
-      if (prev >= 0) { epilogue_tile(prev, nt_done); nt_done++; }
-      if (DBG) { cyc_c += c1_ - c0_; cyc_e += clock64() - c1_; }
-      prev = tile;
-    }
-    { const long long c1_ = DBG ? clock64() : 0; if (prev >= 0) epilogue_tile(prev, nt_done); if (DBG) cyc_e += clock64() - c1_; }
-    if (DBG && p.dbg && warp == W_WORK0 && lane == 0) { p.dbg[(size_t)blockIdx.x * 32 + 24] = (unsigned long long)cyc_c; p.dbg[(size_t)blockIdx.x * 32 + 25] = (unsigned long long)cyc_e; }
+    for (int st = 0; st < nst; st++) {
+      if (st) next_stage(st, false);
+      cur_key = -1;
+      int prev = -1;
+      for (int tile = blockIdx.x; tile < p.ntiles; tile += gridDim.x) {
+        const long long c0_ = DBG ? clock64() : 0;
+        convert_tile(tile);
+        const long long c1_ = DBG ? clock64() : 0;
+        if (prev >= 0) { epilogue_tile(prev, nt_done); nt_done++; }
+        if (DBG && et == 0) { wcyc[0] += c1_ - c0_; wcyc[1] += clock64() - c1_; }
+        prev = tile;
+      }
+      { const long long c1_ = DBG ? clock64() : 0; if (prev >= 0) { epilogue_tile(prev, nt_done); nt_done++; } if (DBG && et == 0) wcyc[1] += clock64() - c1_; }
+      if (st + 1 < nst) gridbar::fence_proxy_async_global();
+    }
+    if (DBG && p.dbg && warp == W_WORK0 && lane == 0) { p.dbg[(size_t)blockIdx.x * 32 + 24] = wcyc[0]; p.dbg[(size_t)blockIdx.x * 32 + 25] = wcyc[1]; }
     if (DBG && p.dbg && warp == W_WORK0 && lane == 0) { p.dbg[(size_t)blockIdx.x * 32 + 19] = w_aempty; p.dbg[(size_t)blockIdx.x * 32 + 20] = w_tfull; }
   }
   if (threadIdx.x == 0) if (DBG) stamp(p, 12);
@@ -619,6 +676,11 @@
   if (DBG && p.dbg && threadIdx.x < MW_N)
     p.dbg[(size_t)blockIdx.x * 32 + 26 + threadIdx.x] = mwait_all[threadIdx.x] + mwait_all[MW_N + threadIdx.x];
 }
+
+template <bool DBG>
+__global__ void __launch_bounds__(THREADS, 1) conv_fused_kernel(const __grid_constant__ FChain<1> gc) { conv_fused_body<DBG, 1>(gc); }
+
+__global__ void __launch_bounds__(THREADS, 1) conv_fused_chain_kernel(const __grid_constant__ FChain<MAXS> gc) { conv_fused_body<false, MAXS>(gc); }
 
 unsigned long long* g_fdbg = nullptr;
 thread_local int32_t g_last_cfg[2 + 2 * MAXG] = {};
@@ -642,33 +704,16 @@
   return wst;
 }
 
-}
-
-extern "C" int32_t b2a_conv1d_fused_debug(void* buf) { g_fdbg = (unsigned long long*)buf; return B2A_OK; }
-
-extern "C" int32_t b2a_conv1d_fused_last_config(int32_t* out10) {
-  B2A_CHECK_ARG(out10, "null pointer");
-  for (int i = 0; i < 2 + 2 * MAXG; i++) out10[i] = g_last_cfg[i];
-  return B2A_OK;
-}
-
-extern "C" int32_t b2a_conv1d_fused_fits(int32_t span, int32_t N, int32_t C, int32_t wplanes, int32_t planes) {
-  if (span < 0 || span > 64 || N <= 0 || C <= 0 || N % C || (wplanes != 1 && wplanes != 2) || (planes != 1 && planes != 2)) return 0;
-  const int bn = n_tile(N, C);
-  return bn && weight_stages(a_rows(span) * 128, planes, acc_tile_ld(bn), bn * 128 * wplanes, nullptr) >= 2;
-}
-
-extern "C" int32_t b2a_conv1d_fused(const b2a_convf_t* pr, int32_t n, int32_t planes, int32_t f16, void* ws, int64_t ws_bytes, void* stream) {
-  B2A_CHECK_ARG(pr && n >= 1 && n <= MAXG && (planes == 1 || planes == 2), "1..4 problems, planes 1 or 2");
-  static const int nsm = [] { const int n = b2a_device_sm_count(); return n > 0 ? n : 132; }();
-  FParams p;
+int32_t fill_stage(FParams& p, CUtensorMap* mw, CUtensorMap* ml, const b2a_convf_t* pr, int n, int planes, int f16, void* ws, int64_t ws_bytes,
+                   int nsm, int& maxR, int& maxBN, int& maxWst) {
+  B2A_CHECK_ARG(pr && n >= 1 && n <= MAXG, "1..4 problems per stage");
   p.G = n; p.planes = planes; p.f16 = f16 ? 1 : 0; p.dbg = g_fdbg;
   { static int flags = -1; if (flags < 0) { const char* e = getenv("B2A_FUSED_DBGFLAGS"); flags = e ? atoi(e) : 0; } p.dbg_flags = flags; }
   int order[MAXG];
   double cost[MAXG];
   for (int i = 0; i < n; i++) { order[i] = i; cost[i] = (double)pr[i].taps * pr[i].cin_pad; }
   for (int i = 0; i < n; i++) for (int j = i + 1; j < n; j++) if (cost[order[j]] > cost[order[i]]) { int t = order[i]; order[i] = order[j]; order[j] = t; }
-  int maxR = 0, maxBN = 0, maxWst = 0, tiles_total = 0;
+  int tiles_total = 0;
   int64_t base_tiles = 0, sum_base = 0, cnt_used = 0, ws_used = 0;
   for (int gi = 0; gi < n; gi++) {
     const b2a_convf_t& q = pr[gi];
@@ -732,34 +777,86 @@
     maxWst = wsz > maxWst ? wsz : maxWst;
   }
   p.ntiles = tiles_total;
-  p.a_plane = maxR * 128;
-  p.w_stage = maxWst;
-  p.acc_ld = acc_tile_ld(maxBN);
-  size_t smem = 0;
-  const int wst = weight_stages(p.a_plane, planes, p.acc_ld, p.w_stage, &smem);
-  if (wst < 2) { b2a_set_error("b2a_conv1d_fused: shared memory cannot hold two weight stages (R %d, BN %d)", maxR, maxBN); return B2A_E_UNSUPPORTED; }
-  p.wst = wst;
-
-  CUtensorMap mw[MAXG], ml[MAXG];
-  for (int gi = 0; gi < MAXG; gi++) {
-    const b2a_convf_t& q = pr[order[gi < n ? gi : 0]];
-    const FProb& P = p.pr[gi < n ? gi : 0];
+  for (int gi = 0; gi < n; gi++) {
+    const b2a_convf_t& q = pr[order[gi]];
+    const FProb& P = p.pr[gi];
     const uint64_t wdims[2] = {(uint64_t)q.cin_pad, (uint64_t)q.taps * q.N}, wstr[1] = {(uint64_t)q.cin_pad * 2};
     const uint32_t wbox[2] = {TK, (uint32_t)P.BN};
     int e = b2a_tmap16(&mw[gi], q.w_hi, 2, wdims, wstr, wbox, p.f16);
     if (!e) e = b2a_tmap16(&ml[gi], q.w_lo ? q.w_lo : q.w_hi, 2, wdims, wstr, wbox, p.f16);
     if (e) { b2a_set_error("b2a_conv1d_fused: cuTensorMapEncodeTiled failed (%d)", e); return B2A_E_CUDA; }
   }
-  const bool dbg = p.dbg != nullptr || p.dbg_flags != 0;
-  const auto kern = dbg ? conv_fused_kernel<true> : conv_fused_kernel<false>;
-  B2A_SMEM_OPTIN(kern, DYN_SMEM_MAX);
-  const int grid = tiles_total < nsm ? tiles_total : nsm;
-  cudaError_t err = b2a_launch_pdl(kern, dim3(grid), dim3(THREADS), smem, (cudaStream_t)stream, p, mw[0], mw[1], mw[2], mw[3], ml[0], ml[1],
-                                   ml[2], ml[3]);
-  if (err != cudaSuccess) { b2a_set_error("b2a_conv1d_fused: launch failed: %s", cudaGetErrorString(err)); return B2A_E_CUDA; }
-  B2A_CHECK_LAUNCH();
   for (int i = 0; i < 2 + 2 * MAXG; i++) g_last_cfg[i] = 0;
-  g_last_cfg[0] = n; g_last_cfg[1] = grid;
+  g_last_cfg[0] = n;
   for (int gi = 0; gi < n; gi++) { g_last_cfg[2 + 2 * order[gi]] = p.pr[gi].BN; g_last_cfg[3 + 2 * order[gi]] = p.pr[gi].ksplit; }
   return B2A_OK;
 }
+
+}
+
+extern "C" int32_t b2a_conv1d_fused_debug(void* buf) { g_fdbg = (unsigned long long*)buf; return B2A_OK; }
+
+extern "C" int32_t b2a_conv1d_fused_last_config(int32_t* out10) {
+  B2A_CHECK_ARG(out10, "null pointer");
+  for (int i = 0; i < 2 + 2 * MAXG; i++) out10[i] = g_last_cfg[i];
+  return B2A_OK;
+}
+
+extern "C" int32_t b2a_conv1d_fused_fits(int32_t span, int32_t N, int32_t C, int32_t wplanes, int32_t planes) {
+  if (span < 0 || span > 64 || N <= 0 || C <= 0 || N % C || (wplanes != 1 && wplanes != 2) || (planes != 1 && planes != 2)) return 0;
+  const int bn = n_tile(N, C);
+  return bn && weight_stages(a_rows(span) * 128, planes, acc_tile_ld(bn), bn * 128 * wplanes, nullptr) >= 2;
+}
+
+extern "C" int32_t b2a_conv1d_fused(const b2a_convf_t* pr, const int32_t* counts, int32_t nst, int32_t planes, int32_t f16, void* ws,
+                                    int64_t ws_bytes, uint32_t* bar, uint32_t* err, int32_t grid, void* stream) {
+  B2A_CHECK_ARG(pr && counts && nst >= 1 && nst <= MAXS && (planes == 1 || planes == 2), "1..4 stages, planes 1 or 2");
+  B2A_CHECK_ARG(nst == 1 || (bar && err), "a chain needs a grid barrier word and an error word");
+  B2A_CHECK_ARG(grid >= 0, "grid >= 0");
+  static const int nsm = [] { const int n = b2a_device_sm_count(); return n > 0 ? n : 132; }();
+  static thread_local FChain<MAXS> c;
+  memset(&c, 0, sizeof(c));
+  c.nst = nst;
+  int maxR = 0, maxBN = 0, maxWst = 0, most_tiles = 0;
+  const b2a_convf_t* q = pr;
+  for (int s = 0; s < nst; s++) {
+    const int32_t e = fill_stage(c.st[s], c.mw[s], c.ml[s], q, counts[s], planes, f16, ws, ws_bytes, nsm, maxR, maxBN, maxWst);
+    if (e != B2A_OK) return e;
+    q += counts[s];
+    most_tiles = c.st[s].ntiles > most_tiles ? c.st[s].ntiles : most_tiles;
+  }
+  size_t smem = 0;
+  const int wst = weight_stages(maxR * 128, planes, acc_tile_ld(maxBN), maxWst, &smem);
+  if (wst < 2) { b2a_set_error("b2a_conv1d_fused: shared memory cannot hold two weight stages (R %d, BN %d)", maxR, maxBN); return B2A_E_UNSUPPORTED; }
+  for (int s = 0; s < nst; s++) { c.st[s].a_plane = maxR * 128; c.st[s].w_stage = maxWst; c.st[s].acc_ld = acc_tile_ld(maxBN); c.st[s].wst = wst; }
+  if (grid == 0 || grid > most_tiles) grid = most_tiles < nsm ? most_tiles : nsm;
+  cudaError_t e;
+  if (nst == 1) {
+    static thread_local FChain<1> c1;
+    memset(&c1, 0, sizeof(c1));
+    c1.nst = 1; c1.st[0] = c.st[0];
+    memcpy(c1.mw[0], c.mw[0], sizeof(c1.mw[0])); memcpy(c1.ml[0], c.ml[0], sizeof(c1.ml[0]));
+    const bool dbg = c1.st[0].dbg != nullptr || c1.st[0].dbg_flags != 0;
+    const auto kern = dbg ? conv_fused_kernel<true> : conv_fused_kernel<false>;
+    B2A_SMEM_OPTIN(kern, DYN_SMEM_MAX);
+    e = b2a_launch_pdl(kern, dim3(grid), dim3(THREADS), smem, (cudaStream_t)stream, c1);
+  } else {
+    B2A_SMEM_OPTIN(conv_fused_chain_kernel, DYN_SMEM_MAX);
+    B2A_CHECK_ARG(grid <= nsm, "a chain runs at most one CTA per SM");
+    c.bar = bar; c.err = err;
+    e = cudaMemsetAsync(c.bar, 0, 4, (cudaStream_t)stream);
+    if (e == cudaSuccess) {
+      cudaLaunchConfig_t cfg = {};
+      cfg.gridDim = dim3(grid); cfg.blockDim = dim3(THREADS); cfg.dynamicSmemBytes = smem; cfg.stream = (cudaStream_t)stream;
+      cudaLaunchAttribute at[1];
+      at[0].id = cudaLaunchAttributeCooperative;
+      at[0].val.cooperative = 1;
+      cfg.attrs = at; cfg.numAttrs = 1;
+      e = cudaLaunchKernelEx(&cfg, conv_fused_chain_kernel, c);
+    }
+  }
+  if (e != cudaSuccess) { b2a_set_error("b2a_conv1d_fused: launch failed: %s", cudaGetErrorString(e)); return B2A_E_CUDA; }
+  B2A_CHECK_LAUNCH();
+  g_last_cfg[1] = grid;
+  return B2A_OK;
+}
diff --git a/mlx_audio_b200/csrc/grid_barrier.cuh b/mlx_audio_b200/csrc/grid_barrier.cuh
--- /dev/null
+++ b/mlx_audio_b200/csrc/grid_barrier.cuh
@@ -0,0 +1,36 @@
+#pragma once
+#include <stdint.h>
+
+namespace gridbar {
+
+constexpr long long TIMEOUT_NS = 10000000000LL;
+
+__device__ __forceinline__ long long globaltimer() {
+  long long t;
+  asm volatile("mov.u64 %0, %globaltimer;" : "=l"(t));
+  return t;
+}
+
+__device__ inline bool wait(unsigned* bar, unsigned* err, unsigned target) {
+  long long t0 = 0;
+  for (int it = 0;; it++) {
+    unsigned v;
+    asm volatile("ld.acquire.gpu.global.u32 %0, [%1];" : "=r"(v) : "l"(bar) : "memory");
+    if ((int)(v - target) >= 0) return true;
+    if ((it & 63) == 63) {
+      if (*(volatile unsigned*)err) return false;
+      const long long now = globaltimer();
+      if (!t0) t0 = now;
+      else if (now - t0 > TIMEOUT_NS) { atomicExch(err, 1u); return false; }
+    }
+    __nanosleep(64);
+  }
+}
+
+__device__ __forceinline__ void arrive(unsigned* bar) {
+  asm volatile("red.release.gpu.global.add.u32 [%0], 1;" ::"l"(bar) : "memory");
+}
+
+__device__ __forceinline__ void fence_proxy_async_global() { asm volatile("fence.proxy.async.global;" ::: "memory"); }
+
+}
diff --git a/mlx_audio_b200/ops.py b/mlx_audio_b200/ops.py
--- a/mlx_audio_b200/ops.py
+++ b/mlx_audio_b200/ops.py
@@ -483,25 +483,57 @@
         self.p, self.out, self.keep, self.f16 = p, out, keep, cw.f16
 
 
-def conv_fused(problems) -> list:
-    if isinstance(problems, FusedProblem):
-        problems = [problems]
-    n = len(problems)
-    if not 1 <= n <= 4:
-        raise ValueError("conv_fused: 1..4 problems per launch")
+_FUSED_ERR = {}
+_FUSED_BAR = {}
+FUSED_MAX_STAGES = 4
+
+
+def conv_fused_error_word(device) -> torch.Tensor:
+    device = torch.device(device)
+    w = _FUSED_ERR.get(device)
+    if w is None:
+        if torch.cuda.is_current_stream_capturing():
+            raise RuntimeError("conv_fused_chain: run one chain outside graph capture first (its error word is allocated then)")
+        w = _FUSED_ERR[device] = torch.zeros(1, device=device, dtype=torch.int32)
+    return w
+
+
+def conv_fused_chain(stages, grid: int = 0) -> list:
+    stages = [[s] if isinstance(s, FusedProblem) else list(s) for s in stages]
+    if not 1 <= len(stages) <= FUSED_MAX_STAGES or not all(1 <= len(s) <= 4 for s in stages):
+        raise ValueError(f"conv_fused_chain: 1..{FUSED_MAX_STAGES} stages of 1..4 problems each")
+    problems = [pr for s in stages for pr in s]
     f16 = problems[0].f16
     if any(pr.f16 != f16 for pr in problems):
         raise ValueError("conv_fused: all problems of a launch must use the same 16-bit operand type")
-    arr = (ConvFParams * n)(*[pr.p for pr in problems])
+    arr = (ConvFParams * len(problems))(*[pr.p for pr in problems])
+    counts = (C.c_int32 * len(stages))(*[len(s) for s in stages])
     dev = problems[0].out.device
     key = (dev, torch.cuda.current_stream().cuda_stream)
     ws = _FUSED_WS.get(key)
     if ws is None:
         ws = _FUSED_WS[key] = torch.zeros(FUSED_WS_BYTES, device=dev, dtype=torch.uint8)
+    err = bar = None
+    if len(stages) > 1:
+        err = conv_fused_error_word(dev)
+        bar = _FUSED_BAR.get(key)
+        if bar is None:
+            bar = _FUSED_BAR[key] = torch.zeros(1, device=dev, dtype=torch.int32)
     if PROFILE_TAGS is not None:
-        TAG[0] = "fused " + " + ".join(f"[{q.B}x{q.L}x{q.Cin}->{q.N} k{q.taps}{' up' + str(q.up_stride) if q.up_stride else ''}]" for q in (pr.p for pr in problems))
-    _call("conv_tc", _lib.lib().b2a_conv1d_fused, 1, arr, n, 2 if TC_MODE[0] == "x2" else 1, int(f16), ws.data_ptr(), ws.numel(), _stream())
-    return [pr.out for pr in problems]
+        TAG[0] = ("fused " if len(stages) == 1 else f"fused chain {len(stages)}: ") + " | ".join(
+            " + ".join(f"[{q.B}x{q.L}x{q.Cin}->{q.N} k{q.taps}{' up' + str(q.up_stride) if q.up_stride else ''}]" for q in (pr.p for pr in s))
+            for s in stages)
+    _call("conv_tc", _lib.lib().b2a_conv1d_fused, 1, arr, counts, len(stages), 2 if TC_MODE[0] == "x2" else 1, int(f16), ws.data_ptr(),
+          ws.numel(), _p(bar), _p(err), int(grid), _stream())
+    return [[pr.out for pr in s] for s in stages]
+
+
+def conv_fused(problems) -> list:
+    if isinstance(problems, FusedProblem):
+        problems = [problems]
+    if not 1 <= len(problems) <= 4:
+        raise ValueError("conv_fused: 1..4 problems per launch")
+    return conv_fused_chain([problems])[0]
 
 
 def linear(x, cw: ConvW, *, planes=False, qkv_heads=0, qkv_scale=0.0, **kw):
diff --git a/mlx_audio_b200/tts/models/kokoro/kokoro.py b/mlx_audio_b200/tts/models/kokoro/kokoro.py
--- a/mlx_audio_b200/tts/models/kokoro/kokoro.py
+++ b/mlx_audio_b200/tts/models/kokoro/kokoro.py
@@ -322,32 +322,44 @@
             first = [ops.FusedProblem(x, b["conv1"], pad_left=1, pre=ops.PreStats(sx, self._gb(b["name"] + ".norm1"), 1e-5, lrelu, 0.2), stats_out=st)
                      for x, sx, b, st in zip(xs, sxs, blks, s1)]
         shortcut = [ops.FusedProblem(x, b["sc"]) for x, b in zip(xs, blks) if "sc" in b]
-        res = ops.conv_fused(first + shortcut) if len(first) + len(shortcut) <= 4 else ops.conv_fused(first) + ops.conv_fused(shortcut)
-        r1 = res[:n]
-        scs = res[n:] if shortcut else xs
+        stages = [first + shortcut] if len(first) + len(shortcut) <= 4 else [first, shortcut]
+        r1 = [pr.out for pr in first]
+        scs = [pr.out for pr in shortcut] if shortcut else xs
         second = [ops.FusedProblem(r, b["conv2"], pad_left=1, pre=ops.PreStats(st, self._gb(b["name"] + ".norm2"), 1e-5, lrelu, 0.2), res=sc,
                                    res_div=2 if up else 1, out_scale=1.0 / math.sqrt(2.0), out=o, stats_out=so)
                   for r, b, st, sc, o, so in zip(r1, blks, s1, scs, outs, sos)]
-        return ops.conv_fused(second)
+        return stages + [second], [pr.out for pr in second]
 
     def _resblock1_group(self, xs, sxs, blks, outs=None):
         n = len(blks)
         outs = outs or [None] * n
         cur, scur = list(xs), list(sxs)
+        stages = []
         for j in range(3):
             last = j == 2
             st1 = [self._stats(b["c1"][j].cout) for b in blks]
             c1 = [ops.FusedProblem(x, b["c1"][j], dilation=b["dils"][j], pad_left=(b["k"] * b["dils"][j] - b["dils"][j]) // 2,
                                    pre=ops.PreStats(sx, self._gb(f"{b['name']}.adain1.{j}"), 1e-5, ACT["snake"], 0.0, *b["a1"][j]), stats_out=st)
                   for x, sx, b, st in zip(cur, scur, blks, st1)]
-            xt = ops.conv_fused(c1)
+            xt = [pr.out for pr in c1]
             snew = [None if last else self._stats(b["c2"][j].cout) for b in blks]
             c2 = [ops.FusedProblem(t, b["c2"][j], pad_left=(b["k"] - 1) // 2,
                                    pre=ops.PreStats(st, self._gb(f"{b['name']}.adain2.{j}"), 1e-5, ACT["snake"], 0.0, *b["a2"][j]), res=x,
                                    out=outs[i] if last else None, stats_out=sn)
                   for i, (t, st, x, b, sn) in enumerate(zip(xt, st1, cur, blks, snew))]
-            cur, scur = ops.conv_fused(c2), snew
-        return cur
+            stages += [c1, c2]
+            cur, scur = [pr.out for pr in c2], snew
+        return stages, cur
+
+    @staticmethod
+    def _chain(stages):
+        for i in range(0, len(stages), ops.FUSED_MAX_STAGES):
+            ops.conv_fused_chain(stages[i:i + ops.FUSED_MAX_STAGES])
+
+    @staticmethod
+    def _launch(stages):
+        for st in stages:
+            ops.conv_fused(st)
 
     @torch.no_grad()
     def _acoustic_side_fused(self, st, F: int, noise=None, f0n_override=None):
@@ -365,11 +377,17 @@
         ops.channel_stats(xs, sxs)
         F0N = torch.empty(2, 2 * F, 1, device=dev, dtype=torch.float32)
         hcur, scur = [xs, xs], [sxs, sxs]
+        chain = []
         for bi in range(3):
             blks = [W["F0"][bi], W["N"][bi]]
             sos = [self._stats(b["conv2"].cout) for b in blks] if bi < 2 else None
-            hcur = self._resblk1d_group(hcur, scur, blks, sos=sos)
+            if blks[0]["up"]:
+                self._chain(chain)
+                chain = []
+            stages, hcur = self._resblk1d_group(hcur, scur, blks, sos=sos)
+            chain += stages
             scur = sos
+        self._chain(chain)
         ops.conv1d(hcur[0], W["F0_proj"], out=F0N[0:1])
         ops.conv1d(hcur[1], W["N_proj"], out=F0N[1:2])
         if f0n_override is not None:
@@ -405,9 +423,10 @@
                 ts.append(t)
             pool, self._stats_pool = self._stats_pool, [s for group in zip(*src_arena) for s in group]
             try:
-                self._resblock1_group(ts, src_stats, W["noise_res"], outs=xsrcs)
+                stages, _ = self._resblock1_group(ts, src_stats, W["noise_res"], outs=xsrcs)
             finally:
                 self._stats_pool = pool
+            self._launch(stages)
 
         if par:
             side_src = ops.fork(dev, 1)
@@ -426,16 +445,17 @@
         nblk = len(W["decode"])
         sbuf = [self._stats(1024 + 64 + 2) for _ in range(nblk)]
         ops.channel_stats(bufs[0][:, :, 1024:], [sb[:, 1024:] for sb in sbuf])
-        self._resblk1d_group([b514], [s514], [W["encode"]], outs=[bufs[0][:, :, :1024]], sos=[sbuf[0][:, :1024]])
+        self._launch(self._resblk1d_group([b514], [s514], [W["encode"]], outs=[bufs[0][:, :, :1024]], sos=[sbuf[0][:, :1024]])[0])
         self._tap("dec_encode", bufs[0][:, :, :1024])
         cur = 0
         x = None
         for i, blk in enumerate(W["decode"]):
             if blk["up"]:
-                x = self._resblk1d_group([bufs[cur]], [sbuf[i]], [blk])[0]
+                stages, (x,) = self._resblk1d_group([bufs[cur]], [sbuf[i]], [blk])
             else:
-                self._resblk1d_group([bufs[cur]], [sbuf[i]], [blk], outs=[bufs[1 - cur][:, :, :1024]], sos=[sbuf[i + 1][:, :1024]])
+                stages, _ = self._resblk1d_group([bufs[cur]], [sbuf[i]], [blk], outs=[bufs[1 - cur][:, :, :1024]], sos=[sbuf[i + 1][:, :1024]])
                 cur = 1 - cur
+            self._launch(stages)
         self._tap("dec_out", x)
         if par:
             ops.join(dev, side_src)
@@ -460,7 +480,8 @@
                 y = ops.conv_fused(ops.FusedProblem(x, W["ups"][i], stride=u, pad_left=(kk - u) // 2, pre=pre, transpose=True, res=xsrc,
                                                     x_add=x_add, in_scale=in_scale, stats_out=sy))[0]
             blks = [W["resblocks"][i * nk + j] for j in range(nk)]
-            outs = self._resblock1_group([y] * nk, [sy] * nk, blks)
+            stages, outs = self._resblock1_group([y] * nk, [sy] * nk, blks)
+            self._launch(stages)
             x, x_add, in_scale = outs[0], tuple(outs[1:]), 1.0 / nk
             if self.tap is not None:
                 self._tap(f"gen_stage{i}", sum(outs) / nk)
```
